# lostinc0de/sparsemat

Measured on AMD Instinct MI355X. Metric: csr_spmv_effective_hbm_GBps, higher is better.
Workload: dtype f32

## Files before the change

include/sparsemat_hip.h:

```cpp
#ifndef SPARSEMAT_HIP_H
#define SPARSEMAT_HIP_H

#include <stddef.h>
#include <stdint.h>

#ifdef __cplusplus
extern "C" {
#endif

#define SMH_ABI_VERSION 3

enum {
    SMH_OK = 0,
    SMH_ERR_DIM_MISMATCH = 1,
    SMH_ERR_NOT_SQUARE = 2,
    SMH_ERR_INDEX_RANGE = 3,
    SMH_ERR_INVALID = 4,
    SMH_ERR_HIP = 5,
    SMH_ERR_OOM = 6,
    SMH_ERR_NO_DEVICE = 7,
    SMH_ERR_CAPACITY = 8,
    SMH_ERR_COMM = 9
};

typedef enum { SMH_F32 = 0, SMH_F64 = 1 } smh_dtype;

typedef enum {
    SMH_SPMV_AUTO = 0,
    SMH_SPMV_VECTOR = 1,
    SMH_SPMV_MERGE = 2,
    SMH_SPMV_SEQ = 3,
    SMH_SPMV_STREAM = 4,
    SMH_SPMV_COLBLOCK = 5,
    SMH_SPMV_COLFUSED = 6,
    SMH_SPMV_COLSPLIT = 7,
    SMH_SPMV_TILED = 8
} smh_spmv_variant;

typedef enum { SMH_TRI_LOWER = 0, SMH_TRI_UPPER = 1 } smh_tri_uplo;
typedef enum { SMH_DIAG_NON_UNIT = 0, SMH_DIAG_UNIT = 1 } smh_tri_diag;

typedef struct smh_crs smh_crs;
typedef struct smh_vec smh_vec;
typedef struct smh_mvec smh_mvec;

int smh_abi_version(void);
const char *smh_last_error(void);
const char *smh_status_string(int status);
int smh_device_count(int *count_out);
int smh_set_device(int device);
int smh_device_synchronize(void);

int smh_crs_create(smh_dtype dtype, size_t n_rows, size_t n_cols, size_t nnz,
                   const uint32_t *offset_rows, const uint32_t *columns, const void *values,
                   int validate, smh_crs **out);
int smh_crs_create_dev(smh_dtype dtype, size_t n_rows, size_t n_cols, size_t nnz,
                       const uint32_t *offset_rows_dev, const uint32_t *columns_dev,
                       const void *values_dev, int validate, smh_crs **out);
int smh_crs_assemble(smh_dtype dtype, size_t n_ops, const uint32_t *rows, const uint32_t *cols,
                     const void *values, const uint8_t *ops, smh_crs **out);
int smh_crs_assemble_dev(smh_dtype dtype, size_t n_ops, const uint32_t *rows_dev,
                         const uint32_t *cols_dev, const void *values_dev, const uint8_t *ops_dev,
                         smh_crs **out);
int smh_crs_replay(smh_dtype dtype, size_t n_ops, const uint32_t *rows, const uint32_t *cols,
                   const void *values, const uint8_t *ops, smh_crs **out);
int smh_crs_replay_dev(smh_dtype dtype, size_t n_ops, const uint32_t *rows_dev,
                       const uint32_t *cols_dev, const void *values_dev, const uint8_t *ops_dev,
                       smh_crs **out);
int smh_crs_transpose(const smh_crs *a, smh_crs **out);
int smh_last_transpose_route(void);
int smh_crs_column_info(const smh_crs *m, uint32_t *rows, uint32_t *col_ptr, uint32_t *entries);
int smh_crs_column_info_dev(const smh_crs *m, uint32_t *rows_dev, uint32_t *col_ptr_dev,
                            uint32_t *entries_dev);
int smh_crs_prod(const smh_crs *a, const smh_crs *b, smh_crs **out);
int smh_crs_permute(const smh_crs *a, const uint32_t *row_perm, size_t n_row_perm, const uint32_t *col_perm, size_t n_col_perm, smh_crs **out);
int smh_crs_permute_dev(const smh_crs *a, const uint32_t *row_perm_dev, size_t n_row_perm, const uint32_t *col_perm_dev, size_t n_col_perm,
                        smh_crs **out);
int smh_crs_permute_symmetric(const smh_crs *a, const uint32_t *perm, size_t n_perm, smh_crs **out);
int smh_crs_permute_symmetric_dev(const smh_crs *a, const uint32_t *perm_dev, size_t n_perm, smh_crs **out);
int smh_crs_bandwidth(const smh_crs *m, uint32_t *lower_out, uint32_t *upper_out);
int smh_crs_span_fraction(smh_crs *m, double *out);
int smh_crs_rcm(const smh_crs *m, uint32_t *perm_out, size_t *n_components_out, size_t *n_levels_out);
int smh_crs_rcm_dev(const smh_crs *m, uint32_t *perm_out_dev, size_t *n_components_out, size_t *n_levels_out);
int smh_crs_color(const smh_crs *m, uint32_t seed, uint32_t *colors_out, uint32_t *perm_out, size_t *n_colors_out, size_t *n_rounds_out);
int smh_crs_color_dev(const smh_crs *m, uint32_t seed, uint32_t *colors_out_dev, uint32_t *perm_out_dev, size_t *n_colors_out, size_t *n_rounds_out);
int smh_crs_clone(const smh_crs *a, smh_crs **out);
int smh_crs_add(const smh_crs *a, const smh_crs *b, smh_crs **out);
int smh_crs_sub(const smh_crs *a, const smh_crs *b, smh_crs **out);
int smh_crs_add_assign(smh_crs *a, const smh_crs *b);
int smh_crs_sub_assign(smh_crs *a, const smh_crs *b);
int smh_last_add_route(void);
int smh_crs_get(const smh_crs *m, size_t i, size_t j, void *value_out);
int smh_crs_get_many(const smh_crs *m, size_t n, const uint32_t *rows, const uint32_t *cols, void *values_out);
int smh_crs_get_many_dev(const smh_crs *m, size_t n, const uint32_t *rows_dev, const uint32_t *cols_dev, void *values_out_dev);
int smh_crs_apply(smh_crs *m, size_t n_ops, const uint32_t *rows, const uint32_t *cols, const void *values, const uint8_t *ops);
int smh_crs_apply_dev(smh_crs *m, size_t n_ops, const uint32_t *rows_dev, const uint32_t *cols_dev, const void *values_dev,
                      const uint8_t *ops_dev);
int smh_last_apply_route(void);
typedef struct smh_update_plan smh_update_plan;
int smh_update_plan_create(const smh_crs *m, size_t n_ops, const uint32_t *rows, const uint32_t *cols, const uint8_t *ops,
                           smh_update_plan **out);
int smh_update_plan_create_dev(const smh_crs *m, size_t n_ops, const uint32_t *rows_dev, const uint32_t *cols_dev,
                               const uint8_t *ops_dev, smh_update_plan **out);
int smh_update_plan_execute(smh_update_plan *p, smh_crs *m, const void *values, int from_zero);
int smh_update_plan_execute_dev(smh_update_plan *p, smh_crs *m, const void *values_dev, int from_zero);
int smh_update_plan_stats(const smh_update_plan *p, size_t *n_ops, size_t *n_targets, size_t *n_live_ops, size_t *longest_run,
                          size_t *long_run_threshold, size_t *device_bytes);
int smh_update_plan_destroy(smh_update_plan *p);
int smh_crs_eye(smh_dtype dtype, size_t dim, smh_crs **out);
int smh_crs_is_symmetric(const smh_crs *m, int *out);
int smh_crs_is_sorted(const smh_crs *m, int *out);
int smh_crs_sort_rows(smh_crs *m);
int smh_crs_destroy(smh_crs *m);
int smh_crs_update_values(smh_crs *m, const void *values_host);
int smh_crs_download(const smh_crs *m, uint32_t *offset_rows, uint32_t *columns, void *values);
size_t smh_crs_n_rows(const smh_crs *m);
size_t smh_crs_n_cols(const smh_crs *m);
size_t smh_crs_nnz(const smh_crs *m);
size_t smh_crs_orphans(const smh_crs *m);
int smh_crs_dtype(const smh_crs *m);
int smh_crs_max_row_len(const smh_crs *m, uint32_t *out);
int smh_crs_col_range(const smh_crs *m, uint32_t *min_out, uint32_t *max_out);
int smh_crs_scale(smh_crs *m, double a);
int smh_crs_resolved_variant(const smh_crs *m, int *variant_out, int *lanes_out);
int smh_crs_set_vector_lanes(smh_crs *m, int lanes);
int smh_crs_set_stream_xs(smh_crs *m, int mode);
int smh_crs_stream_layout(smh_crs *m, int *coded_out, int *byte_lengths_out, int *small_tiles_out, int *xs_chunks_out);
int smh_crs_stream_value_dict(smh_crs *m, int *n_values_out, void *values_out);
int smh_crs_set_stream_value_dict(smh_crs *m, int mode);
int smh_crs_set_stream_direct(smh_crs *m, int mode);
int smh_crs_stream_direct(smh_crs *m, int *direct_out);
int smh_crs_set_vector_chunks(smh_crs *m, int chunks);
int smh_crs_set_ring(smh_crs *m, int mode);
int smh_crs_ring_entries(smh_crs *m, uint32_t *out);
int smh_crs_ring_column_form(smh_crs *m, int *form_out);
int smh_crs_ring_bands(smh_crs *m, uint32_t *bands_out, uint32_t *intervals_out);
int smh_crs_ring_plan(smh_crs *m, uint32_t *n_blocks_out, size_t *n_phases_out,
                      double *ring_fraction_out, int *active_out, uint32_t *phase_ptr_out,
                      uint32_t *phases_out);

int smh_crs_set_colblock_shift(smh_crs *m, uint32_t shift);
int smh_crs_colblock(smh_crs *m, uint32_t *shift_out, size_t *n_blocks_out, int *rows_per_thread_out,
                     double *span_fraction_out, uint32_t *offsets_out, uint32_t *columns_out,
                     void *values_out);

int smh_crs_colfused(smh_crs *m, int *fits_out, uint32_t *shift_out, size_t *n_blocks_out, uint32_t *rows_per_lane_out,
                     size_t *n_tiles_out, uint32_t *tile_rows_out, uint32_t *segments_out, uint8_t *counts_out,
                     uint32_t *columns_out, void *values_out);

int smh_crs_tiled_layout(smh_crs *m, uint32_t *n_slices_out, uint32_t *slice_columns_out, uint32_t *rows_per_block_out,
                         uint32_t *n_row_blocks_out, size_t *copy_entries_out);
int smh_crs_tiled_products(smh_crs *m, size_t *n_products_out);

int smh_crs_tiled_array(smh_crs *m, int which, void *out, size_t capacity_bytes, size_t *bytes_out);

int smh_crs_colsplit(smh_crs *m, int *split_out, uint32_t *min_long_out, size_t *n_long_out, uint32_t *long_rows_out,
                     smh_crs **long_out, smh_crs **short_out);

int smh_crs_spmv(smh_crs *m, const void *x_host, size_t x_len, void *y_host, int variant);
int smh_crs_prepare(smh_crs *m, int variant);
int smh_crs_prepare_stats(smh_crs *m, int variant, double *prepare_ms_out, size_t *derived_bytes_out);
int smh_crs_spmv_dev(smh_crs *m, const void *x_dev, size_t x_len, void *y_dev, int variant,
                     void *stream);
int smh_crs_inner_prod(smh_crs *m, const void *lhs_host, size_t lhs_len, const void *rhs_host,
                       size_t rhs_len, int variant, double *out);
size_t smh_crs_merge_tiles(const smh_crs *m);
size_t smh_crs_merge_tile_items(const smh_crs *m);
int smh_crs_merge_table(smh_crs *m, uint32_t *row_out, uint32_t *nnz_out);

int smh_vec_create(smh_dtype dtype, size_t n, smh_vec **out);
int smh_vec_from_host(smh_dtype dtype, size_t n, const void *host, smh_vec **out);
int smh_vec_wrap_dev(smh_dtype dtype, size_t n, void *dev_ptr, smh_vec **out);
int smh_vec_destroy(smh_vec *v);
int smh_vec_upload(smh_vec *v, const void *host);
int smh_vec_download(const smh_vec *v, void *host);
size_t smh_vec_dim(const smh_vec *v);
int smh_vec_dtype(const smh_vec *v);
void *smh_vec_data(const smh_vec *v);
int smh_vec_copy(smh_vec *dst, const smh_vec *src);
int smh_vec_permute(smh_vec *dst, const smh_vec *src, const uint32_t *perm, size_t n_perm, int inverse);
int smh_vec_permute_dev(smh_vec *dst, const smh_vec *src, const uint32_t *perm_dev, size_t n_perm, int inverse);
int smh_vec_add(smh_vec *x, const smh_vec *y);
int smh_vec_sub(smh_vec *x, const smh_vec *y);
int smh_vec_scale(smh_vec *x, double a);
int smh_vec_axpy(smh_vec *y, double a, const smh_vec *x);
int smh_vec_xpby(smh_vec *p, double b, const smh_vec *r);
int smh_vec_dot(const smh_vec *x, const smh_vec *y, double *out);
int smh_vec_norm_squared(const smh_vec *x, double *out);
int smh_vec_norm(const smh_vec *x, double *out);
int smh_blas_dot_dev(smh_dtype dtype, const void *x_dev, const void *y_dev, size_t n, void *result_dev,
                     void *scratch_dev, void *stream);
size_t smh_blas_dot_scratch_bytes(void);
int smh_blas_axpy_dev(smh_dtype dtype, void *y_dev, const void *a_dev, const void *x_dev, size_t n, void *stream);
int smh_blas_xpby_dev(smh_dtype dtype, void *p_dev, const void *b_dev, const void *r_dev, size_t n, void *stream);
int smh_crs_spmv_vec(smh_crs *m, const smh_vec *x, smh_vec *y, int variant);
int smh_crs_inner_prod_vec(smh_crs *m, const smh_vec *lhs, const smh_vec *rhs, int variant, double *out);

int smh_mvec_create(smh_dtype dtype, size_t n, size_t k, smh_mvec **out);
int smh_mvec_from_host(smh_dtype dtype, size_t n, size_t k, const void *host, smh_mvec **out);
int smh_mvec_upload(smh_mvec *mv, const void *host);
int smh_mvec_download(const smh_mvec *mv, void *host);
int smh_mvec_destroy(smh_mvec *mv);
size_t smh_mvec_dim(const smh_mvec *mv);
size_t smh_mvec_count(const smh_mvec *mv);
size_t smh_mvec_ld(const smh_mvec *mv);
int smh_mvec_dtype(const smh_mvec *mv);
void *smh_mvec_data(const smh_mvec *mv);
int smh_mvec_set_column(smh_mvec *mv, size_t c, const smh_vec *v);
int smh_mvec_get_column(const smh_mvec *mv, size_t c, smh_vec *v);
int smh_mvec_copy(smh_mvec *dst, const smh_mvec *src);
int smh_mvec_add(smh_mvec *x, const smh_mvec *y);
int smh_mvec_sub(smh_mvec *x, const smh_mvec *y);
int smh_mvec_scale(smh_mvec *x, const double *a);
int smh_mvec_dot(const smh_mvec *x, const smh_mvec *y, double *out);
int smh_mvec_norm_squared(const smh_mvec *x, double *out);

int smh_crs_spmv_many(smh_crs *m, const smh_mvec *x, smh_mvec *y);
int smh_crs_spmv_many_dev(smh_crs *m, const void *x_dev, size_t x_len, void *y_dev, size_t k, size_t ld, void *stream);
int smh_crs_spmv_many_host(smh_crs *m, const void *x_host, size_t x_len, size_t k, void *y_host);

int smh_cg_solve(smh_crs *m, const void *b_host, size_t b_len, void *x_host_inout, size_t x_len,
                 double tol, size_t iter_max, int variant, size_t *iters_out, double *rr_out);
int smh_cg_solve_vec(smh_crs *m, const smh_vec *b, smh_vec *x, double tol, size_t iter_max,
                     int variant, size_t check_every, size_t *iters_out, double *rr_out);
int smh_cg_solve_many(smh_crs *m, const smh_mvec *b, smh_mvec *x, double tol, size_t iter_max, size_t check_every,
                      size_t *iters_out, double *rr_out);
int smh_cg_solve_many_host(smh_crs *m, const void *b_host, size_t n, size_t k, void *x_host_inout, double tol,
                           size_t iter_max, size_t *iters_out, double *rr_out);

int smh_pcg_jacobi_solve(smh_crs *m, const void *b_host, size_t b_len, void *x_host_inout,
                         size_t x_len, double tol, size_t iter_max, int variant, size_t *iters_out,
                         double *rr_out);

int smh_crs_trisolve_levels(smh_crs *m, int uplo, size_t *n_levels_out, uint32_t *level_of_row_out, size_t *n_launches_out,
                            size_t *small_level_rows_out);
int smh_crs_trisolve(smh_crs *m, int uplo, int diag, const void *b_host, size_t b_len, void *x_host, size_t x_len);
int smh_crs_trisolve_vec(smh_crs *m, int uplo, int diag, const smh_vec *b, smh_vec *x);
int smh_crs_sgs_apply_vec(smh_crs *m, const smh_vec *r, smh_vec *z);
int smh_pcg_sgs_solve(smh_crs *m, const void *b_host, size_t b_len, void *x_host_inout, size_t x_len,
                      double tol, size_t iter_max, int variant, size_t *iters_out, double *rr_out);
int smh_pcg_sgs_solve_vec(smh_crs *m, const smh_vec *b, smh_vec *x, double tol, size_t iter_max,
                          int variant, size_t check_every, size_t *iters_out, double *rr_out);

int smh_crs_ilu0(const smh_crs *a, smh_crs **f_out, size_t *zero_pivot_out);
int smh_crs_ilu0_refactor(smh_crs *f, const smh_crs *a, size_t *zero_pivot_out);
int smh_crs_ilu_apply_vec(smh_crs *f, const smh_vec *r, smh_vec *z);
int smh_pcg_ilu_solve(smh_crs *a, smh_crs *f, const void *b_host, size_t b_len, void *x_host_inout, size_t x_len,
                      double tol, size_t iter_max, int variant, size_t *iters_out, double *rr_out);
int smh_pcg_ilu_solve_vec(smh_crs *a, smh_crs *f, const smh_vec *b, smh_vec *x, double tol, size_t iter_max,
                          int variant, size_t check_every, size_t *iters_out, double *rr_out);

int smh_bicgstab_solve(smh_crs *m, const void *b_host, size_t b_len, void *x_host_inout, size_t x_len,
                       double tol, size_t iter_max, int variant,
                       size_t *iters_out, double *rr_out, int *breakdown_out);
int smh_bicgstab_solve_vec(smh_crs *m, const smh_vec *b, smh_vec *x, double tol, size_t iter_max,
                           int variant, size_t check_every,
                           size_t *iters_out, double *rr_out, int *breakdown_out);

typedef struct smh_par smh_par;
typedef struct smh_par_vec smh_par_vec;
typedef struct smh_comm smh_comm;

enum { SMH_EXCHANGE_NONE = 0, SMH_EXCHANGE_ALLGATHER = 1, SMH_EXCHANGE_WINDOW = 2, SMH_EXCHANGE_AUTO = 3 };
enum { SMH_PAR_BACKEND_AUTO = 0, SMH_PAR_BACKEND_PEER = 1, SMH_PAR_BACKEND_RCCL = 2 };
#define SMH_COMM_ID_BYTES 128

int smh_comm_unique_id(void *id_out);
int smh_comm_create(const void *id, int n_ranks, int rank, smh_comm **out);
int smh_comm_destroy(smh_comm *c);
int smh_comm_size(const smh_comm *c);
int smh_comm_rank(const smh_comm *c);
int smh_comm_ranks_seen(const smh_comm *c, int *count_out, int *device_out);
int smh_rccl_version(int *version_out);
int smh_comm_barrier(smh_comm *c);
int smh_comm_max_f64(smh_comm *c, double *value_inout);

int smh_par_create(smh_dtype dtype, size_t n_blocks, const int *device_ids, size_t n_rows,
                   size_t n_cols, const uint32_t *offset_rows, const uint32_t *columns,
                   const void *values, int validate, smh_par **out);
enum { SMH_SPLIT_ROWS = 0, SMH_SPLIT_NNZ = 1 };
int smh_par_create_split(smh_dtype dtype, size_t n_blocks, const int *device_ids, size_t n_rows,
                         size_t n_cols, const uint32_t *offset_rows, const uint32_t *columns,
                         const void *values, int validate, int split_mode, smh_par **out);
int smh_par_adopt_split(size_t n_blocks, smh_crs *const *blocks, size_t n_rows, const size_t *split_rows, smh_par **out);
int smh_par_create_rank_split(smh_comm *comm, size_t n_rows, smh_crs *block, size_t row_begin, smh_par **out);
int smh_par_split(const smh_par *p, size_t *rows_out);
int smh_par_adopt(size_t n_blocks, smh_crs *const *blocks, size_t n_rows, smh_par **out);
int smh_par_create_rank(smh_comm *comm, size_t n_rows, smh_crs *block, smh_par **out);
int smh_par_destroy(smh_par *p);
size_t smh_par_n_blocks(const smh_par *p);
size_t smh_par_n_local_blocks(const smh_par *p);
size_t smh_par_n_rows(const smh_par *p);
// ... 72 lines not shown
```

rust/src/ffi.rs:

```rust
#![allow(non_camel_case_types)]
use std::os::raw::{c_char, c_double, c_int, c_void};

#[repr(C)] pub struct smh_crs { _private: [u8; 0] }
#[repr(C)] pub struct smh_vec { _private: [u8; 0] }
#[repr(C)] pub struct smh_update_plan { _private: [u8; 0] }
#[repr(C)] pub struct smh_par { _private: [u8; 0] }
#[repr(C)] pub struct smh_par_vec { _private: [u8; 0] }
#[repr(C)] pub struct smh_comm { _private: [u8; 0] }

pub const SMH_OK: c_int = 0;
pub const SMH_ERR_DIM_MISMATCH: c_int = 1;
pub const SMH_F32: c_int = 0;
pub const SMH_F64: c_int = 1;
pub const SMH_SPMV_AUTO: c_int = 0;
pub const SMH_TRI_LOWER: c_int = 0;
pub const SMH_TRI_UPPER: c_int = 1;
pub const SMH_DIAG_NON_UNIT: c_int = 0;
pub const SMH_DIAG_UNIT: c_int = 1;
pub const SMH_EXCHANGE_NONE: c_int = 0;
pub const SMH_EXCHANGE_ALLGATHER: c_int = 1;
pub const SMH_EXCHANGE_WINDOW: c_int = 2;
pub const SMH_EXCHANGE_AUTO: c_int = 3;
pub const SMH_COMM_ID_BYTES: usize = 128;
pub const SMH_SPLIT_ROWS: c_int = 0;
pub const SMH_SPLIT_NNZ: c_int = 1;

extern "C" {
    pub fn smh_abi_version() -> c_int;
    pub fn smh_last_error() -> *const c_char;
    pub fn smh_device_count(count_out: *mut c_int) -> c_int;
    pub fn smh_pool_trim() -> c_int;
    pub fn smh_pool_stats(kept_bytes_out: *mut usize, live_bytes_out: *mut usize) -> c_int;
    pub fn smh_crs_create(dtype: c_int, n_rows: usize, n_cols: usize, nnz: usize,
                          offset_rows: *const u32, columns: *const u32, values: *const c_void,
                          validate: c_int, out: *mut *mut smh_crs) -> c_int;
    pub fn smh_crs_destroy(m: *mut smh_crs) -> c_int;
    pub fn smh_crs_update_values(m: *mut smh_crs, values_host: *const c_void) -> c_int;
    pub fn smh_crs_spmv(m: *mut smh_crs, x_host: *const c_void, x_len: usize, y_host: *mut c_void,
                        variant: c_int) -> c_int;
    pub fn smh_cg_solve(m: *mut smh_crs, b_host: *const c_void, b_len: usize, x_host_inout: *mut c_void,
                        x_len: usize, tol: c_double, iter_max: usize, variant: c_int,
                        iters_out: *mut usize, rr_out: *mut c_double) -> c_int;
    pub fn smh_pcg_jacobi_solve(m: *mut smh_crs, b_host: *const c_void, b_len: usize, x_host_inout: *mut c_void,
                                x_len: usize, tol: c_double, iter_max: usize, variant: c_int,
                                iters_out: *mut usize, rr_out: *mut c_double) -> c_int;
    pub fn smh_bicgstab_solve(m: *mut smh_crs, b_host: *const c_void, b_len: usize, x_host_inout: *mut c_void,
                              x_len: usize, tol: c_double, iter_max: usize, variant: c_int,
                              iters_out: *mut usize, rr_out: *mut c_double, breakdown_out: *mut c_int) -> c_int;
    pub fn smh_bicgstab_solve_vec(m: *mut smh_crs, b: *const smh_vec, x: *mut smh_vec, tol: c_double, iter_max: usize,
                                  variant: c_int, check_every: usize,
                                  iters_out: *mut usize, rr_out: *mut c_double, breakdown_out: *mut c_int) -> c_int;
    pub fn smh_crs_trisolve_levels(m: *mut smh_crs, uplo: c_int, n_levels_out: *mut usize, level_of_row_out: *mut u32,
                                   n_launches_out: *mut usize, small_level_rows_out: *mut usize) -> c_int;
    pub fn smh_crs_trisolve(m: *mut smh_crs, uplo: c_int, diag: c_int, b_host: *const c_void, b_len: usize, x_host: *mut c_void,
                            x_len: usize) -> c_int;
    pub fn smh_crs_trisolve_vec(m: *mut smh_crs, uplo: c_int, diag: c_int, b: *const smh_vec, x: *mut smh_vec) -> c_int;
    pub fn smh_crs_sgs_apply_vec(m: *mut smh_crs, r: *const smh_vec, z: *mut smh_vec) -> c_int;
    pub fn smh_pcg_sgs_solve(m: *mut smh_crs, b_host: *const c_void, b_len: usize, x_host_inout: *mut c_void,
                             x_len: usize, tol: c_double, iter_max: usize, variant: c_int,
                             iters_out: *mut usize, rr_out: *mut c_double) -> c_int;
    pub fn smh_pcg_sgs_solve_vec(m: *mut smh_crs, b: *const smh_vec, x: *mut smh_vec, tol: c_double, iter_max: usize,
                                 variant: c_int, check_every: usize, iters_out: *mut usize, rr_out: *mut c_double) -> c_int;
    pub fn smh_crs_ilu0(a: *const smh_crs, f_out: *mut *mut smh_crs, zero_pivot_out: *mut usize) -> c_int;
    pub fn smh_crs_ilu0_refactor(f: *mut smh_crs, a: *const smh_crs, zero_pivot_out: *mut usize) -> c_int;
    pub fn smh_crs_ilu_apply_vec(f: *mut smh_crs, r: *const smh_vec, z: *mut smh_vec) -> c_int;
    pub fn smh_pcg_ilu_solve(a: *mut smh_crs, f: *mut smh_crs, b_host: *const c_void, b_len: usize, x_host_inout: *mut c_void,
                             x_len: usize, tol: c_double, iter_max: usize, variant: c_int,
                             iters_out: *mut usize, rr_out: *mut c_double) -> c_int;
    pub fn smh_pcg_ilu_solve_vec(a: *mut smh_crs, f: *mut smh_crs, b: *const smh_vec, x: *mut smh_vec, tol: c_double, iter_max: usize,
                                 variant: c_int, check_every: usize, iters_out: *mut usize, rr_out: *mut c_double) -> c_int;
    pub fn smh_crs_inner_prod(m: *mut smh_crs, lhs_host: *const c_void, lhs_len: usize, rhs_host: *const c_void,
                              rhs_len: usize, variant: c_int, out: *mut c_double) -> c_int;
    pub fn smh_crs_assemble(dtype: c_int, n_ops: usize, rows: *const u32, cols: *const u32, values: *const c_void,
                            ops: *const u8, out: *mut *mut smh_crs) -> c_int;
    pub fn smh_crs_replay(dtype: c_int, n_ops: usize, rows: *const u32, cols: *const u32, values: *const c_void,
                          ops: *const u8, out: *mut *mut smh_crs) -> c_int;
    pub fn smh_crs_transpose(a: *const smh_crs, out: *mut *mut smh_crs) -> c_int;
    pub fn smh_crs_set_stream_xs(m: *mut smh_crs, mode: c_int) -> c_int;
    pub fn smh_crs_set_stream_direct(m: *mut smh_crs, mode: c_int) -> c_int;
    pub fn smh_crs_stream_direct(m: *mut smh_crs, direct_out: *mut c_int) -> c_int;
    pub fn smh_crs_stream_layout(m: *mut smh_crs, coded_out: *mut c_int, byte_lengths_out: *mut c_int, small_tiles_out: *mut c_int, xs_chunks_out: *mut c_int) -> c_int;
    pub fn smh_last_transpose_route() -> c_int;
    pub fn smh_crs_orphans(m: *const smh_crs) -> usize;
    pub fn smh_crs_prod(a: *const smh_crs, b: *const smh_crs, out: *mut *mut smh_crs) -> c_int;
    pub fn smh_crs_clone(a: *const smh_crs, out: *mut *mut smh_crs) -> c_int;
    pub fn smh_crs_permute(a: *const smh_crs, row_perm: *const u32, n_row_perm: usize, col_perm: *const u32, n_col_perm: usize,
                           out: *mut *mut smh_crs) -> c_int;
    pub fn smh_crs_permute_dev(a: *const smh_crs, row_perm_dev: *const u32, n_row_perm: usize, col_perm_dev: *const u32,
                               n_col_perm: usize, out: *mut *mut smh_crs) -> c_int;
    pub fn smh_crs_permute_symmetric(a: *const smh_crs, perm: *const u32, n_perm: usize, out: *mut *mut smh_crs) -> c_int;
    pub fn smh_crs_permute_symmetric_dev(a: *const smh_crs, perm_dev: *const u32, n_perm: usize, out: *mut *mut smh_crs) -> c_int;
    pub fn smh_crs_bandwidth(m: *const smh_crs, lower_out: *mut u32, upper_out: *mut u32) -> c_int;
    pub fn smh_crs_span_fraction(m: *mut smh_crs, out: *mut f64) -> c_int;
    pub fn smh_crs_rcm(m: *const smh_crs, perm_out: *mut u32, n_components_out: *mut usize, n_levels_out: *mut usize) -> c_int;
    pub fn smh_crs_rcm_dev(m: *const smh_crs, perm_out_dev: *mut u32, n_components_out: *mut usize, n_levels_out: *mut usize) -> c_int;
    pub fn smh_crs_color(m: *const smh_crs, seed: u32, colors_out: *mut u32, perm_out: *mut u32, n_colors_out: *mut usize, n_rounds_out: *mut usize) -> c_int;
    pub fn smh_crs_color_dev(m: *const smh_crs, seed: u32, colors_out_dev: *mut u32, perm_out_dev: *mut u32, n_colors_out: *mut usize, n_rounds_out: *mut usize) -> c_int;
    pub fn smh_vec_permute(dst: *mut smh_vec, src: *const smh_vec, perm: *const u32, n_perm: usize, inverse: c_int) -> c_int;
    pub fn smh_vec_permute_dev(dst: *mut smh_vec, src: *const smh_vec, perm_dev: *const u32, n_perm: usize, inverse: c_int) -> c_int;
    pub fn smh_crs_add(a: *const smh_crs, b: *const smh_crs, out: *mut *mut smh_crs) -> c_int;
    pub fn smh_crs_sub(a: *const smh_crs, b: *const smh_crs, out: *mut *mut smh_crs) -> c_int;
    pub fn smh_crs_add_assign(a: *mut smh_crs, b: *const smh_crs) -> c_int;
    pub fn smh_crs_sub_assign(a: *mut smh_crs, b: *const smh_crs) -> c_int;
    pub fn smh_last_add_route() -> c_int;
    pub fn smh_crs_get(m: *const smh_crs, i: usize, j: usize, value_out: *mut c_void) -> c_int;
    pub fn smh_crs_get_many(m: *const smh_crs, n: usize, rows: *const u32, cols: *const u32, values_out: *mut c_void) -> c_int;
    pub fn smh_crs_get_many_dev(m: *const smh_crs, n: usize, rows_dev: *const u32, cols_dev: *const u32,
                                values_out_dev: *mut c_void) -> c_int;
    pub fn smh_crs_apply(m: *mut smh_crs, n_ops: usize, rows: *const u32, cols: *const u32, values: *const c_void,
                         ops: *const u8) -> c_int;
    pub fn smh_crs_apply_dev(m: *mut smh_crs, n_ops: usize, rows_dev: *const u32, cols_dev: *const u32,
                             values_dev: *const c_void, ops_dev: *const u8) -> c_int;
    pub fn smh_last_apply_route() -> c_int;
    pub fn smh_update_plan_create(m: *const smh_crs, n_ops: usize, rows: *const u32, cols: *const u32, ops: *const u8,
                                  out: *mut *mut smh_update_plan) -> c_int;
    pub fn smh_update_plan_create_dev(m: *const smh_crs, n_ops: usize, rows_dev: *const u32, cols_dev: *const u32,
                                      ops_dev: *const u8, out: *mut *mut smh_update_plan) -> c_int;
    pub fn smh_update_plan_execute(p: *mut smh_update_plan, m: *mut smh_crs, values: *const c_void, from_zero: c_int) -> c_int;
    pub fn smh_update_plan_execute_dev(p: *mut smh_update_plan, m: *mut smh_crs, values_dev: *const c_void, from_zero: c_int) -> c_int;
    pub fn smh_update_plan_stats(p: *const smh_update_plan, n_ops: *mut usize, n_targets: *mut usize, n_live_ops: *mut usize,
                                 longest_run: *mut usize, long_run_threshold: *mut usize, device_bytes: *mut usize) -> c_int;
    pub fn smh_update_plan_destroy(p: *mut smh_update_plan) -> c_int;
    pub fn smh_crs_eye(dtype: c_int, dim: usize, out: *mut *mut smh_crs) -> c_int;
    pub fn smh_crs_is_symmetric(m: *const smh_crs, out: *mut c_int) -> c_int;
    pub fn smh_crs_is_sorted(m: *const smh_crs, out: *mut c_int) -> c_int;
    pub fn smh_crs_column_info(m: *const smh_crs, rows: *mut u32, col_ptr: *mut u32, entries: *mut u32) -> c_int;
    pub fn smh_crs_sort_rows(m: *mut smh_crs) -> c_int;
    pub fn smh_par_create(dtype: c_int, n_blocks: usize, device_ids: *const c_int, n_rows: usize, n_cols: usize,
                          offset_rows: *const u32, columns: *const u32, values: *const c_void, validate: c_int,
                          out: *mut *mut smh_par) -> c_int;
    pub fn smh_par_create_split(dtype: c_int, n_blocks: usize, device_ids: *const c_int, n_rows: usize, n_cols: usize,
                                offset_rows: *const u32, columns: *const u32, values: *const c_void, validate: c_int,
                                split_mode: c_int, out: *mut *mut smh_par) -> c_int;
    pub fn smh_par_split(p: *const smh_par, rows_out: *mut usize) -> c_int;
    pub fn smh_par_set_overlap(p: *mut smh_par, on: c_int) -> c_int;
    pub fn smh_par_interior(p: *const smh_par, local_block: usize, variant: c_int, row_begin: *mut usize, row_end: *mut usize) -> c_int;
    pub fn smh_par_destroy(p: *mut smh_par) -> c_int;
    pub fn smh_par_spmv(p: *mut smh_par, x_host: *const c_void, x_len: usize, y_host: *mut c_void, variant: c_int) -> c_int;
    pub fn smh_par_cg_solve(p: *mut smh_par, b_host: *const c_void, b_len: usize, x_host_inout: *mut c_void, x_len: usize,
                            tol: c_double, iter_max: usize, variant: c_int, iters_out: *mut usize,
                            rr_out: *mut c_double) -> c_int;
    pub fn smh_par_vec_create(p: *mut smh_par, n: usize, out: *mut *mut smh_par_vec) -> c_int;
    pub fn smh_par_vec_destroy(v: *mut smh_par_vec) -> c_int;
    pub fn smh_par_vec_upload(v: *mut smh_par_vec, host: *const c_void) -> c_int;
    pub fn smh_par_vec_download(v: *const smh_par_vec, host: *mut c_void) -> c_int;
    pub fn smh_par_spmv_dev(p: *mut smh_par, x: *const smh_par_vec, y: *mut smh_par_vec, variant: c_int, exchange: c_int) -> c_int;
    pub fn smh_par_exchange(p: *mut smh_par, v: *mut smh_par_vec, mode: c_int) -> c_int;
    pub fn smh_par_synchronize(p: *mut smh_par) -> c_int;
    pub fn smh_par_cg_solve_vec(p: *mut smh_par, b: *const smh_par_vec, x: *mut smh_par_vec, tol: c_double, iter_max: usize,
                                variant: c_int, check_every: usize, iters_out: *mut usize, rr_out: *mut c_double) -> c_int;
    pub fn smh_comm_unique_id(id_out: *mut c_void) -> c_int;
    pub fn smh_comm_create(id: *const c_void, n_ranks: c_int, rank: c_int, out: *mut *mut smh_comm) -> c_int;
    pub fn smh_comm_destroy(c: *mut smh_comm) -> c_int;
    pub fn smh_par_create_rank(comm: *mut smh_comm, n_rows: usize, block: *mut smh_crs, out: *mut *mut smh_par) -> c_int;
    pub fn smh_par_create_rank_split(comm: *mut smh_comm, n_rows: usize, block: *mut smh_crs, row_begin: usize, out: *mut *mut smh_par) -> c_int;
    pub fn smh_crs_n_rows(m: *const smh_crs) -> usize;
    pub fn smh_crs_n_cols(m: *const smh_crs) -> usize;
    pub fn smh_crs_dtype(m: *const smh_crs) -> c_int;
    pub fn smh_crs_nnz(m: *const smh_crs) -> usize;
    pub fn smh_crs_download(m: *const smh_crs, offset_rows: *mut u32, columns: *mut u32, values: *mut c_void) -> c_int;
}
```

sparsemat_amd/_lib.py:

```python
import ctypes as C
import os

_HERE = os.path.dirname(os.path.abspath(__file__))
LIB_PATH = os.environ.get("SPARSEMAT_HIP_LIB") or os.path.join(_HERE, "libsparsemat_hip.so")

SMH_OK = 0
SMH_ERR_DIM_MISMATCH, SMH_ERR_NOT_SQUARE, SMH_ERR_INDEX_RANGE, SMH_ERR_INVALID = 1, 2, 3, 4
SMH_ERR_HIP, SMH_ERR_OOM, SMH_ERR_NO_DEVICE, SMH_ERR_CAPACITY, SMH_ERR_COMM = 5, 6, 7, 8, 9
SMH_F32, SMH_F64 = 0, 1
SMH_TRI_LOWER, SMH_TRI_UPPER = 0, 1
SMH_DIAG_NON_UNIT, SMH_DIAG_UNIT = 0, 1
UPLO = {"lower": SMH_TRI_LOWER, "upper": SMH_TRI_UPPER}
EXCHANGE_NONE, EXCHANGE_ALLGATHER, EXCHANGE_WINDOW, EXCHANGE_AUTO = 0, 1, 2, 3
EXCHANGES = {"none": EXCHANGE_NONE, "allgather": EXCHANGE_ALLGATHER, "window": EXCHANGE_WINDOW, "halo": EXCHANGE_WINDOW, "auto": EXCHANGE_AUTO}
EXCHANGE_NAMES = {EXCHANGE_NONE: "none", EXCHANGE_ALLGATHER: "allgather", EXCHANGE_WINDOW: "window", EXCHANGE_AUTO: "auto"}
PAR_BACKEND_AUTO, PAR_BACKEND_PEER, PAR_BACKEND_RCCL = 0, 1, 2
PAR_BACKENDS = {"auto": PAR_BACKEND_AUTO, "peer": PAR_BACKEND_PEER, "rccl": PAR_BACKEND_RCCL}
COMM_ID_BYTES = 128
SPMV_AUTO, SPMV_VECTOR, SPMV_MERGE, SPMV_SEQ, SPMV_STREAM, SPMV_COLBLOCK, SPMV_COLFUSED, SPMV_COLSPLIT, SPMV_TILED = 0, 1, 2, 3, 4, 5, 6, 7, 8
VARIANTS = {"auto": SPMV_AUTO, "vector": SPMV_VECTOR, "merge": SPMV_MERGE, "seq": SPMV_SEQ, "stream": SPMV_STREAM,
            "colblock": SPMV_COLBLOCK, "colfused": SPMV_COLFUSED, "colsplit": SPMV_COLSPLIT, "tiled": SPMV_TILED}

_sz = C.c_size_t
_vp = C.c_void_p
_u32p = C.POINTER(C.c_uint32)
_int = C.c_int

SIGNATURES = {
    "smh_abi_version": (_int, []),
    "smh_last_error": (C.c_char_p, []),
    "smh_status_string": (C.c_char_p, [_int]),
    "smh_device_count": (_int, [C.POINTER(_int)]),
    "smh_set_device": (_int, [_int]),
    "smh_device_synchronize": (_int, []),
    "smh_crs_create": (_int, [_int, _sz, _sz, _sz, _vp, _vp, _vp, _int, C.POINTER(_vp)]),
    "smh_crs_create_dev": (_int, [_int, _sz, _sz, _sz, _vp, _vp, _vp, _int, C.POINTER(_vp)]),
    "smh_crs_assemble": (_int, [_int, _sz, _vp, _vp, _vp, _vp, C.POINTER(_vp)]),
    "smh_crs_assemble_dev": (_int, [_int, _sz, _vp, _vp, _vp, _vp, C.POINTER(_vp)]),
    "smh_crs_replay": (_int, [_int, _sz, _vp, _vp, _vp, _vp, C.POINTER(_vp)]),
    "smh_crs_replay_dev": (_int, [_int, _sz, _vp, _vp, _vp, _vp, C.POINTER(_vp)]),
    "smh_crs_transpose": (_int, [_vp, C.POINTER(_vp)]),
    "smh_crs_column_info": (_int, [_vp, _vp, _vp, _vp]),
    "smh_crs_column_info_dev": (_int, [_vp, _vp, _vp, _vp]),
    "smh_crs_prod": (_int, [_vp, _vp, C.POINTER(_vp)]),
    "smh_crs_permute": (_int, [_vp, _vp, _sz, _vp, _sz, C.POINTER(_vp)]),
    "smh_crs_permute_dev": (_int, [_vp, _vp, _sz, _vp, _sz, C.POINTER(_vp)]),
    "smh_crs_permute_symmetric": (_int, [_vp, _vp, _sz, C.POINTER(_vp)]),
    "smh_crs_permute_symmetric_dev": (_int, [_vp, _vp, _sz, C.POINTER(_vp)]),
    "smh_crs_bandwidth": (_int, [_vp, _u32p, _u32p]),
    "smh_crs_span_fraction": (_int, [_vp, C.POINTER(C.c_double)]),
    "smh_crs_rcm": (_int, [_vp, _vp, C.POINTER(_sz), C.POINTER(_sz)]),
    "smh_crs_rcm_dev": (_int, [_vp, _vp, C.POINTER(_sz), C.POINTER(_sz)]),
    "smh_crs_color": (_int, [_vp, C.c_uint32, _vp, _vp, C.POINTER(_sz), C.POINTER(_sz)]),
    "smh_crs_color_dev": (_int, [_vp, C.c_uint32, _vp, _vp, C.POINTER(_sz), C.POINTER(_sz)]),
    "smh_vec_permute": (_int, [_vp, _vp, _vp, _sz, _int]),
    "smh_vec_permute_dev": (_int, [_vp, _vp, _vp, _sz, _int]),
    "smh_crs_clone": (_int, [_vp, C.POINTER(_vp)]),
    "smh_crs_add": (_int, [_vp, _vp, C.POINTER(_vp)]),
    "smh_crs_sub": (_int, [_vp, _vp, C.POINTER(_vp)]),
    "smh_crs_add_assign": (_int, [_vp, _vp]),
    "smh_crs_sub_assign": (_int, [_vp, _vp]),
    "smh_last_add_route": (_int, []),
    "smh_crs_get": (_int, [_vp, _sz, _sz, _vp]),
    "smh_crs_get_many": (_int, [_vp, _sz, _vp, _vp, _vp]),
    "smh_crs_get_many_dev": (_int, [_vp, _sz, _vp, _vp, _vp]),
    "smh_crs_apply": (_int, [_vp, _sz, _vp, _vp, _vp, _vp]),
    "smh_crs_apply_dev": (_int, [_vp, _sz, _vp, _vp, _vp, _vp]),
    "smh_last_apply_route": (_int, []),
    "smh_update_plan_create": (_int, [_vp, _sz, _vp, _vp, _vp, _vp]),
    "smh_update_plan_create_dev": (_int, [_vp, _sz, _vp, _vp, _vp, _vp]),
    "smh_update_plan_execute": (_int, [_vp, _vp, _vp, _int]),
    "smh_update_plan_execute_dev": (_int, [_vp, _vp, _vp, _int]),
    "smh_update_plan_stats": (_int, [_vp, _vp, _vp, _vp, _vp, _vp, _vp]),
    "smh_update_plan_destroy": (_int, [_vp]),
    "smh_crs_eye": (_int, [_int, _sz, C.POINTER(_vp)]),
    "smh_crs_is_symmetric": (_int, [_vp, C.POINTER(_int)]),
    "smh_crs_is_sorted": (_int, [_vp, C.POINTER(_int)]),
    "smh_crs_sort_rows": (_int, [_vp]),
    "smh_crs_destroy": (_int, [_vp]),
    "smh_crs_update_values": (_int, [_vp, _vp]),
    "smh_crs_download": (_int, [_vp, _vp, _vp, _vp]),
    "smh_crs_n_rows": (_sz, [_vp]),
    "smh_crs_n_cols": (_sz, [_vp]),
    "smh_crs_nnz": (_sz, [_vp]),
    "smh_crs_orphans": (_sz, [_vp]),
    "smh_crs_dtype": (_int, [_vp]),
    "smh_crs_max_row_len": (_int, [_vp, _u32p]),
    "smh_crs_col_range": (_int, [_vp, _u32p, _u32p]),
    "smh_crs_scale": (_int, [_vp, C.c_double]),
    "smh_crs_resolved_variant": (_int, [_vp, C.POINTER(_int), C.POINTER(_int)]),
    "smh_crs_set_vector_lanes": (_int, [_vp, _int]),
    "smh_crs_set_vector_chunks": (_int, [_vp, _int]),
    "smh_crs_set_ring": (_int, [_vp, _int]),
    "smh_crs_ring_entries": (_int, [_vp, _u32p]),
    "smh_crs_ring_column_form": (_int, [_vp, C.POINTER(_int)]),
    "smh_crs_ring_bands": (_int, [_vp, _u32p, _vp]),
    "smh_crs_ring_plan": (_int, [_vp, _u32p, C.POINTER(_sz), C.POINTER(C.c_double), C.POINTER(_int), _vp, _vp]),
    "smh_crs_set_colblock_shift": (_int, [_vp, C.c_uint32]),
    "smh_crs_tiled_layout": (_int, [_vp, _u32p, _u32p, _u32p, _u32p, C.POINTER(_sz)]),
    "smh_crs_tiled_products": (_int, [_vp, C.POINTER(_sz)]),
    "smh_crs_prepare_stats": (_int, [_vp, _int, C.POINTER(C.c_double), C.POINTER(_sz)]),
    "smh_crs_tiled_array": (_int, [_vp, _int, _vp, _sz, C.POINTER(_sz)]),
    "smh_crs_colblock": (_int, [_vp, _u32p, C.POINTER(_sz), C.POINTER(_int), C.POINTER(C.c_double), _vp, _vp, _vp]),
    "smh_crs_colfused": (_int, [_vp, C.POINTER(_int), _u32p, C.POINTER(_sz), _u32p, C.POINTER(_sz), _vp, _vp, _vp, _vp, _vp]),
    "smh_crs_colsplit": (_int, [_vp, C.POINTER(_int), _u32p, C.POINTER(_sz), _vp, C.POINTER(_vp), C.POINTER(_vp)]),
    "smh_crs_spmv": (_int, [_vp, _vp, _sz, _vp, _int]),
    "smh_crs_spmv_dev": (_int, [_vp, _vp, _sz, _vp, _int, _vp]),
    "smh_crs_prepare": (_int, [_vp, _int]),
    "smh_crs_merge_tiles": (_sz, [_vp]),
    "smh_crs_merge_tile_items": (_sz, [_vp]),
    "smh_crs_merge_table": (_int, [_vp, _vp, _vp]),
    "smh_vec_create": (_int, [_int, _sz, C.POINTER(_vp)]),
    "smh_vec_from_host": (_int, [_int, _sz, _vp, C.POINTER(_vp)]),
    "smh_vec_wrap_dev": (_int, [_int, _sz, _vp, C.POINTER(_vp)]),
    "smh_vec_destroy": (_int, [_vp]),
    "smh_vec_upload": (_int, [_vp, _vp]),
    "smh_vec_download": (_int, [_vp, _vp]),
    "smh_vec_dim": (_sz, [_vp]),
    "smh_vec_dtype": (_int, [_vp]),
    "smh_vec_data": (_vp, [_vp]),
    "smh_vec_copy": (_int, [_vp, _vp]),
    "smh_vec_add": (_int, [_vp, _vp]),
    "smh_vec_sub": (_int, [_vp, _vp]),
    "smh_vec_scale": (_int, [_vp, C.c_double]),
    "smh_vec_axpy": (_int, [_vp, C.c_double, _vp]),
    "smh_vec_xpby": (_int, [_vp, C.c_double, _vp]),
    "smh_vec_dot": (_int, [_vp, _vp, C.POINTER(C.c_double)]),
    "smh_vec_norm_squared": (_int, [_vp, C.POINTER(C.c_double)]),
    "smh_vec_norm": (_int, [_vp, C.POINTER(C.c_double)]),
    "smh_blas_dot_dev": (_int, [_int, _vp, _vp, _sz, _vp, _vp, _vp]),
    "smh_blas_dot_scratch_bytes": (_sz, []),
    "smh_blas_axpy_dev": (_int, [_int, _vp, _vp, _vp, _sz, _vp]),
    "smh_blas_xpby_dev": (_int, [_int, _vp, _vp, _vp, _sz, _vp]),
    "smh_crs_spmv_vec": (_int, [_vp, _vp, _vp, _int]),
    "smh_crs_inner_prod": (_int, [_vp, _vp, _sz, _vp, _sz, _int, C.POINTER(C.c_double)]),
    "smh_crs_inner_prod_vec": (_int, [_vp, _vp, _vp, _int, C.POINTER(C.c_double)]),
    "smh_mvec_create": (_int, [_int, _sz, _sz, C.POINTER(_vp)]),
    "smh_mvec_from_host": (_int, [_int, _sz, _sz, _vp, C.POINTER(_vp)]),
    "smh_mvec_upload": (_int, [_vp, _vp]),
    "smh_mvec_download": (_int, [_vp, _vp]),
    "smh_mvec_destroy": (_int, [_vp]),
    "smh_mvec_dim": (_sz, [_vp]),
    "smh_mvec_count": (_sz, [_vp]),
    "smh_mvec_ld": (_sz, [_vp]),
    "smh_mvec_dtype": (_int, [_vp]),
    "smh_mvec_data": (_vp, [_vp]),
    "smh_mvec_set_column": (_int, [_vp, _sz, _vp]),
    "smh_mvec_get_column": (_int, [_vp, _sz, _vp]),
    "smh_mvec_copy": (_int, [_vp, _vp]),
    "smh_mvec_add": (_int, [_vp, _vp]),
    "smh_mvec_sub": (_int, [_vp, _vp]),
    "smh_mvec_scale": (_int, [_vp, C.POINTER(C.c_double)]),
    "smh_mvec_dot": (_int, [_vp, _vp, C.POINTER(C.c_double)]),
    "smh_mvec_norm_squared": (_int, [_vp, C.POINTER(C.c_double)]),
    "smh_crs_spmv_many": (_int, [_vp, _vp, _vp]),
    "smh_crs_spmv_many_dev": (_int, [_vp, _vp, _sz, _vp, _sz, _sz, _vp]),
    "smh_crs_spmv_many_host": (_int, [_vp, _vp, _sz, _sz, _vp]),
    "smh_cg_solve": (_int, [_vp, _vp, _sz, _vp, _sz, C.c_double, _sz, _int, C.POINTER(_sz),
                            C.POINTER(C.c_double)]),
    "smh_cg_solve_vec": (_int, [_vp, _vp, _vp, C.c_double, _sz, _int, _sz, C.POINTER(_sz),
                                C.POINTER(C.c_double)]),
    "smh_cg_solve_many": (_int, [_vp, _vp, _vp, C.c_double, _sz, _sz, C.POINTER(_sz), C.POINTER(C.c_double)]),
    "smh_cg_solve_many_host": (_int, [_vp, _vp, _sz, _sz, _vp, C.c_double, _sz, C.POINTER(_sz), C.POINTER(C.c_double)]),
    "smh_pcg_jacobi_solve": (_int, [_vp, _vp, _sz, _vp, _sz, C.c_double, _sz, _int, C.POINTER(_sz),
                                    C.POINTER(C.c_double)]),
    "smh_crs_trisolve_levels": (_int, [_vp, _int, C.POINTER(_sz), _vp, C.POINTER(_sz), C.POINTER(_sz)]),
    "smh_crs_trisolve": (_int, [_vp, _int, _int, _vp, _sz, _vp, _sz]),
    "smh_crs_trisolve_vec": (_int, [_vp, _int, _int, _vp, _vp]),
    "smh_crs_sgs_apply_vec": (_int, [_vp, _vp, _vp]),
    "smh_pcg_sgs_solve": (_int, [_vp, _vp, _sz, _vp, _sz, C.c_double, _sz, _int, C.POINTER(_sz),
                                 C.POINTER(C.c_double)]),
    "smh_pcg_sgs_solve_vec": (_int, [_vp, _vp, _vp, C.c_double, _sz, _int, _sz, C.POINTER(_sz),
                                     C.POINTER(C.c_double)]),
    "smh_crs_ilu0": (_int, [_vp, C.POINTER(_vp), C.POINTER(_sz)]),
    "smh_crs_ilu0_refactor": (_int, [_vp, _vp, C.POINTER(_sz)]),
    "smh_crs_ilu_apply_vec": (_int, [_vp, _vp, _vp]),
    "smh_pcg_ilu_solve": (_int, [_vp, _vp, _vp, _sz, _vp, _sz, C.c_double, _sz, _int, C.POINTER(_sz),
                                 C.POINTER(C.c_double)]),
    "smh_pcg_ilu_solve_vec": (_int, [_vp, _vp, _vp, _vp, C.c_double, _sz, _int, _sz, C.POINTER(_sz),
                                     C.POINTER(C.c_double)]),
    "smh_bicgstab_solve": (_int, [_vp, _vp, _sz, _vp, _sz, C.c_double, _sz, _int, C.POINTER(_sz),
                                  C.POINTER(C.c_double), C.POINTER(_int)]),
    "smh_bicgstab_solve_vec": (_int, [_vp, _vp, _vp, C.c_double, _sz, _int, _sz, C.POINTER(_sz),
                                      C.POINTER(C.c_double), C.POINTER(_int)]),
    "smh_comm_unique_id": (_int, [_vp]),
    "smh_comm_create": (_int, [_vp, _int, _int, C.POINTER(_vp)]),
    "smh_comm_destroy": (_int, [_vp]),
    "smh_comm_size": (_int, [_vp]),
    "smh_comm_rank": (_int, [_vp]),
    "smh_comm_ranks_seen": (_int, [_vp, C.POINTER(C.c_int), C.POINTER(C.c_int)]),
    "smh_rccl_version": (_int, [C.POINTER(C.c_int)]),
    "smh_comm_barrier": (_int, [_vp]),
    "smh_comm_max_f64": (_int, [_vp, C.POINTER(C.c_double)]),
    "smh_par_create": (_int, [_int, _sz, _vp, _sz, _sz, _vp, _vp, _vp, _int, C.POINTER(_vp)]),
    "smh_par_create_split": (_int, [_int, _sz, _vp, _sz, _sz, _vp, _vp, _vp, _int, _int, C.POINTER(_vp)]),
    "smh_par_adopt_split": (_int, [_sz, C.POINTER(_vp), _sz, _vp, C.POINTER(_vp)]),
    "smh_par_create_rank_split": (_int, [_vp, _sz, _vp, _sz, C.POINTER(_vp)]),
    "smh_par_split": (_int, [_vp, _vp]),
    "smh_par_plan_split": (_int, [_sz, _sz, _vp, _vp, _vp, _vp, _sz, _vp, _vp, _vp, _vp, C.POINTER(_int), C.POINTER(_sz)]),
    "smh_par_adopt": (_int, [_sz, C.POINTER(_vp), _sz, C.POINTER(_vp)]),
    "smh_par_create_rank": (_int, [_vp, _sz, _vp, C.POINTER(_vp)]),
    "smh_par_n_local_blocks": (_sz, [_vp]),
    "smh_par_set_backend": (_int, [_vp, _int]),
    "smh_par_backend": (_int, [_vp]),
    "smh_par_set_overlap": (_int, [_vp, _int]),
    "smh_par_set_threads": (_int, [_vp, _int]),
    "smh_par_interior": (_int, [_vp, _sz, _int, C.POINTER(_sz), C.POINTER(_sz)]),
    "smh_par_exchange_mode": (_int, [_vp, _int, C.POINTER(_int), C.POINTER(_sz)]),
    "smh_par_plan": (_int, [_sz, _sz, _vp, _vp, _vp, _sz, _vp, _vp, _vp, _vp, C.POINTER(_int), C.POINTER(_sz)]),
    "smh_par_vec_create": (_int, [_vp, _sz, C.POINTER(_vp)]),
    "smh_par_vec_destroy": (_int, [_vp]),
    "smh_par_vec_dim": (_sz, [_vp]),
    "smh_par_vec_upload": (_int, [_vp, _vp]),
    "smh_par_vec_download": (_int, [_vp, _vp]),
    "smh_par_vec_download_block": (_int, [_vp, _sz, _vp]),
    "smh_par_vec_ptr": (_int, [_vp, _sz, C.POINTER(_vp)]),
    "smh_par_spmv_dev": (_int, [_vp, _vp, _vp, _int, _int]),
    "smh_par_exchange": (_int, [_vp, _vp, _int]),
    "smh_par_synchronize": (_int, [_vp]),
    "smh_par_cg_solve_vec": (_int, [_vp, _vp, _vp, C.c_double, _sz, _int, _sz, C.POINTER(_sz), C.POINTER(C.c_double)]),
    "smh_par_destroy": (_int, [_vp]),
    "smh_par_n_blocks": (_sz, [_vp]),
    "smh_par_n_rows": (_sz, [_vp]),
    "smh_par_n_cols": (_sz, [_vp]),
    "smh_par_nnz": (_sz, [_vp]),
    "smh_par_rows_per_block": (_sz, [_vp]),
    "smh_par_block": (_int, [_vp, _sz, C.POINTER(_vp), C.POINTER(_sz), C.POINTER(_sz), C.POINTER(_int)]),
    "smh_par_block_stream": (_int, [_vp, _sz, C.POINTER(_vp)]),
    "smh_par_get_block_and_row_id": (_int, [_vp, _sz, C.POINTER(_sz), C.POINTER(_sz)]),
    "smh_par_scale": (_int, [_vp, C.c_double]),
    "smh_par_spmv": (_int, [_vp, _vp, _sz, _vp, _int]),
    "smh_par_cg_solve": (_int, [_vp, _vp, _sz, _vp, _sz, C.c_double, _sz, _int, C.POINTER(_sz),
                                C.POINTER(C.c_double)]),
    "smh_synth_x": (_int, [_int, C.c_uint64, _sz, _sz, _vp, _vp]),
    "smh_synth_fixed": (_int, [_int, C.c_uint64, _int, _sz, C.c_uint32, _sz, _sz, _vp, _vp, _vp, _vp]),
    "smh_synth_powerlaw_cdf": (_int, [C.c_uint32, C.c_double, _vp]),
    "smh_synth_powerlaw_lengths": (_int, [C.c_uint64, _sz, _sz, C.c_uint32, _vp, _vp]),
    "smh_synth_fill": (_int, [_int, C.c_uint64, _sz, _sz, _sz, _vp, _vp, _vp, _vp]),
    "smh_synth_laplace3d": (_int, [_int, _sz, _sz, _sz, _sz, _sz, _vp, _vp, _vp, C.POINTER(_sz), _vp]),
    "smh_crs_set_stream_xs": (_int, [_vp, _int]),
    "smh_crs_set_stream_direct": (_int, [_vp, _int]),
    "smh_crs_stream_direct": (_int, [_vp, C.POINTER(_int)]),
    "smh_crs_stream_layout": (_int, [_vp, C.POINTER(_int), C.POINTER(_int), C.POINTER(_int), C.POINTER(_int)]),
    "smh_crs_stream_value_dict": (_int, [_vp, C.POINTER(C.c_int), _vp]),
    "smh_crs_set_stream_value_dict": (_int, [_vp, _int]),
    "smh_last_transpose_route": (_int, []),
    "smh_pool_trim": (_int, []),
    "smh_pool_stats": (_int, [C.POINTER(_sz), C.POINTER(_sz)]),
    "smh_dev_alloc": (_int, [_sz, C.POINTER(_vp)]),
# ... 68 lines not shown
```

sparsemat_amd/csrc/capi.hip:

```cpp
#include <atomic>
#include <chrono>
#include <cmath>
#include <cstdarg>
#include <cstdlib>
#include <cstring>
#include <new>
#include <vector>

#include "crs_forms.hpp"

namespace smh {

static thread_local char g_err[512] = "";

void set_error(const char *fmt, ...) {
    va_list ap;
    va_start(ap, fmt);
    vsnprintf(g_err, sizeof g_err, fmt, ap);
    va_end(ap);
}

void clear_error() { g_err[0] = 0; }

int fail(int status, const char *fmt, ...) {
// ... 1049 lines not shown
    return tiled_array(m, which, out, capacity_bytes, bytes_out);
}

int smh_crs_set_colblock_shift(smh_crs *m, uint32_t shift) {
    if (!m) return fail(SMH_ERR_INVALID, "NULL handle");
    if (shift > 31) return fail(SMH_ERR_INVALID, "column block shift must be 0 (automatic) or 1..31");
    if (shift != m->knobs.cb_forced_shift) invalidate(m, Changed::BlockWidth);
    m->knobs.cb_forced_shift = shift;
    return SMH_OK;
}

int smh_crs_colblock(smh_crs *m, uint32_t *shift_out, size_t *n_blocks_out, int *rows_per_thread_out,
                     double *span_fraction_out, uint32_t *offsets_out, uint32_t *columns_out, void *values_out) {
    if (!m) return fail(SMH_ERR_INVALID, "NULL handle");
    SMH_TRY(ensure_ring_plan(m, false));
    SMH_TRY(ensure_colblock(m));
    if (shift_out) *shift_out = m->cb.shift;
    if (n_blocks_out) *n_blocks_out = m->cb.blocks;
    if (rows_per_thread_out) *rows_per_thread_out = m->cb.rpt;
    if (span_fraction_out) *span_fraction_out = m->span_fraction;
    if (offsets_out)
        SMH_HIP(hipMemcpy(offsets_out, m->cb.off.get(), m->cb.blocks * (m->n_rows + 1) * sizeof(uint32_t), hipMemcpyDeviceToHost));
    if (columns_out && m->nnz) SMH_HIP(hipMemcpy(columns_out, m->cb.col.get(), m->nnz * sizeof(uint32_t), hipMemcpyDeviceToHost));
    if (values_out && m->nnz) SMH_HIP(hipMemcpy(values_out, m->cb.val.get(), m->nnz * dtype_size(m->dtype), hipMemcpyDeviceToHost));
    return SMH_OK;
}

int smh_crs_colfused(smh_crs *m, int *fits_out, uint32_t *shift_out, size_t *n_blocks_out, uint32_t *rows_per_lane_out,
                     size_t *n_tiles_out, uint32_t *tile_rows_out, uint32_t *segments_out, uint8_t *counts_out, uint32_t *columns_out,
                     void *values_out) {
    if (!m) return fail(SMH_ERR_INVALID, "NULL handle");
    SMH_TRY(ensure_colfused(m));
    const size_t tile_rows = (size_t)64 * m->cf.rt, n_tiles = (m->cf.state == Form::Ready) ? m->cf.tiles : 0;
    if (fits_out) *fits_out = (m->cf.state == Form::Ready) ? 1 : 0;
    if (shift_out) *shift_out = m->cf.shift;
    if (n_blocks_out) *n_blocks_out = m->cf.blocks;
    if (rows_per_lane_out) *rows_per_lane_out = m->cf.rt;
    if (n_tiles_out) *n_tiles_out = n_tiles;
    if (m->cf.state != Form::Ready) return SMH_OK;
    SMH_HIP(hipStreamSynchronize(m->stream));
    if (tile_rows_out) SMH_HIP(hipMemcpy(tile_rows_out, m->cf.tile_row.get(), (n_tiles + 1) * sizeof(uint32_t), hipMemcpyDeviceToHost));
    if (segments_out) SMH_HIP(hipMemcpy(segments_out, m->cf.seg.get(), (n_tiles * m->cf.blocks + 1) * sizeof(uint32_t), hipMemcpyDeviceToHost));
    if (counts_out && n_tiles) SMH_HIP(hipMemcpy(counts_out, m->cf.cnt.get(), n_tiles * m->cf.blocks * tile_rows, hipMemcpyDeviceToHost));
    if (columns_out && m->nnz) SMH_HIP(hipMemcpy(columns_out, m->cf.col.get(), m->nnz * sizeof(uint32_t), hipMemcpyDeviceToHost));
    if (values_out && m->nnz) SMH_HIP(hipMemcpy(values_out, m->cf.val.get(), m->nnz * dtype_size(m->dtype), hipMemcpyDeviceToHost));
    return SMH_OK;
}

int smh_crs_colsplit(smh_crs *m, int *split_out, uint32_t *min_long_out, size_t *n_long_out, uint32_t *long_rows_out, smh_crs **long_out,
                     smh_crs **short_out) {
    if (!m) return fail(SMH_ERR_INVALID, "NULL handle");
    SMH_TRY(ensure_split(m));
    const bool split = m->split.state == Form::Ready;
    if (split_out) *split_out = split ? 1 : 0;
    if (min_long_out) *min_long_out = kSplitMinLong;
    if (n_long_out) *n_long_out = split ? m->split.n_long : 0;
    if (long_out) *long_out = split ? m->split.long_part : nullptr;
    if (short_out) *short_out = split ? m->split.short_part : nullptr;
    if (long_rows_out && split && m->split.n_long)
        SMH_HIP(hipMemcpy(long_rows_out, m->split.rows.get(), m->split.n_long * sizeof(uint32_t), hipMemcpyDeviceToHost));
    return SMH_OK;
}

int smh_crs_resolved_variant(const smh_crs *m, int *variant_out, int *lanes_out) {
    if (!m) return fail(SMH_ERR_INVALID, "NULL handle");
    if (variant_out) *variant_out = resolve_variant(m, SMH_SPMV_AUTO);
    if (lanes_out) *lanes_out = auto_lanes(m);
    return SMH_OK;
}

int smh_crs_set_stream_xs(smh_crs *m, int mode) {
    if (!m) return fail(SMH_ERR_INVALID, "NULL handle");
    if (mode < -1 || mode > 1) return fail(SMH_ERR_INVALID, "mode must be -1 (automatic), 0 (never) or 1 (whenever the tiles allow)");
    m->knobs.use_stream_xs = mode;
    return recode_stream(m);
}

int smh_crs_set_stream_direct(smh_crs *m, int mode) {
    if (!m) return fail(SMH_ERR_INVALID, "NULL handle");
    if (mode < -1 || mode > 1) return fail(SMH_ERR_INVALID, "mode must be -1 (automatic), 0 (never) or 1 (whenever x is staged)");
    m->knobs.use_stream_direct = mode;
    return recode_stream(m);
}

int smh_crs_stream_direct(smh_crs *m, int *direct_out) {
    if (!m || !direct_out) return fail(SMH_ERR_INVALID, "NULL argument");
    StreamCfg c;
    SMH_TRY(stream_cfg(m, &c));
    *direct_out = c.direct && c.xs != 0;
    return SMH_OK;
}

int smh_crs_stream_value_dict(smh_crs *m, int *n_values_out, void *values_out) {
    if (!m || !n_values_out) return fail(SMH_ERR_INVALID, "NULL argument");
    StreamCfg c;
    SMH_TRY(stream_cfg(m, &c));
    *n_values_out = c.dict ? (int)m->dict.n : 0;
    if (c.dict && values_out) {
        SMH_HIP(hipMemcpyAsync(values_out, m->dict.values.get(), (size_t)m->dict.n * dtype_size(m->dtype), hipMemcpyDeviceToHost, m->stream));
        SMH_HIP(hipStreamSynchronize(m->stream));
    }
    return SMH_OK;
}

int smh_crs_set_stream_value_dict(smh_crs *m, int mode) {
    if (!m) return fail(SMH_ERR_INVALID, "NULL handle");
    if (mode < -1 || mode > 0) return fail(SMH_ERR_INVALID, "mode must be -1 (automatic: whenever the values allow) or 0 (never)");
    m->knobs.use_stream_vdict = mode;
    return recode_stream(m);
}

int smh_crs_stream_layout(smh_crs *m, int *coded_out, int *byte_lengths_out, int *small_tiles_out, int *xs_chunks_out) {
    if (!m) return fail(SMH_ERR_INVALID, "NULL handle");
    StreamCfg c;
    SMH_TRY(stream_cfg(m, &c));
    if (coded_out) *coded_out = c.code && c.cwin;
    if (byte_lengths_out) *byte_lengths_out = c.len8 && c.tbase;
    if (small_tiles_out) *small_tiles_out = c.small;
    if (xs_chunks_out) *xs_chunks_out = c.xs;
    return SMH_OK;
}

int smh_crs_set_vector_chunks(smh_crs *m, int chunks) {
    if (!m) return fail(SMH_ERR_INVALID, "NULL handle");
    if (chunks < 0 || chunks > 3) return fail(SMH_ERR_INVALID, "chunks per lane must be 0 (automatic), 1, 2 or 3");
    m->knobs.forced_chunks = chunks;
    return SMH_OK;
}

int smh_crs_set_ring(smh_crs *m, int mode) {
    if (!m) return fail(SMH_ERR_INVALID, "NULL handle");
    if (mode < -1 || mode > 1) return fail(SMH_ERR_INVALID, "ring mode must be -1 (auto), 0 (plain K1) or 1 (K1r)");
    m->knobs.use_ring = mode;
    return SMH_OK;
}

int smh_crs_ring_plan(smh_crs *m, uint32_t *n_blocks_out, size_t *n_phases_out, double *ring_fraction_out,
                      int *active_out, uint32_t *phase_ptr_out, uint32_t *phases_out) {
    if (!m) return fail(SMH_ERR_INVALID, "NULL handle");
    SMH_TRY(ensure_ring_plan(m));
    bool ring = false;
    SMH_TRY(vector_uses_ring(m, &ring));
    if (n_blocks_out) *n_blocks_out = m->ring.blocks;
    if (n_phases_out) *n_phases_out = m->ring.n_phases;
    if (ring_fraction_out) *ring_fraction_out = m->ring.fraction;
    if (active_out) *active_out = ring ? 1 : 0;
    if (phase_ptr_out)
        SMH_HIP(hipMemcpy(phase_ptr_out, m->ring.phase_ptr.get(), (m->ring.blocks + 1) * sizeof(uint32_t), hipMemcpyDeviceToHost));
    if (phases_out && m->ring.n_phases)
        SMH_HIP(hipMemcpy(phases_out, m->ring.phases.get(), m->ring.n_phases * sizeof(RingPhase), hipMemcpyDeviceToHost));
    return SMH_OK;
}

int smh_crs_ring_column_form(smh_crs *m, int *form_out) {
    if (!m || !form_out) return fail(SMH_ERR_INVALID, "NULL argument");
    bool ring = false;
    SMH_TRY(vector_uses_ring(m, &ring));
    *form_out = !ring ? 0 : m->ring.lo8.get() ? 2 : m->ring.col16.get() ? 1 : 0;
    return SMH_OK;
}

int smh_crs_ring_entries(smh_crs *m, uint32_t *out) {
    if (!m || !out) return fail(SMH_ERR_INVALID, "NULL argument");
    SMH_TRY(ensure_ring_plan(m));
    *out = m->ring.entries;
    return SMH_OK;
}

int smh_crs_ring_bands(smh_crs *m, uint32_t *bands_out, uint32_t *intervals_out) {
    if (!m || !bands_out) return fail(SMH_ERR_INVALID, "NULL argument");
    SMH_TRY(ensure_ring_plan(m));
    *bands_out = m->ring.bands;
    if (intervals_out && m->ring.bands == 4 && m->ring.win.get())
        SMH_HIP(hipMemcpy(intervals_out, m->ring.win.get(), ((m->n_rows + 63) / 64) * 8 * sizeof(uint32_t), hipMemcpyDeviceToHost));
    return SMH_OK;
}

int smh_crs_set_vector_lanes(smh_crs *m, int lanes) {
    if (!m) return fail(SMH_ERR_INVALID, "NULL handle");
    if (lanes != 0 && (lanes < 1 || lanes > 64 || (lanes & (lanes - 1))))
        return fail(SMH_ERR_INVALID, "lanes per row must be 0 or a power of two in 1..64");
    m->knobs.forced_lanes = lanes;
    return SMH_OK;
}

int smh_crs_prepare(smh_crs *m, int variant) {
    if (!m) return fail(SMH_ERR_INVALID, "NULL handle");
    const auto t0 = std::chrono::steady_clock::now();
    const long long b0 = pool_thread_net_bytes();
    int rc = prepare_forms(m, variant);
    if (rc == SMH_OK && m->stream) {
        const hipError_t e = hipStreamSynchronize(m->stream);
        if (e != hipSuccess) rc = hip_fail(e, "hipStreamSynchronize", __FILE__, __LINE__);
    }
    m->prepare_ms += std::chrono::duration<double, std::milli>(std::chrono::steady_clock::now() - t0).count();
    m->prepare_bytes += pool_thread_net_bytes() - b0;
    return rc;
}

int smh_crs_prepare_stats(smh_crs *m, int variant, double *prepare_ms_out, size_t *derived_bytes_out) {
    if (!m) return fail(SMH_ERR_INVALID, "NULL handle");
    SMH_TRY(smh_crs_prepare(m, variant));
    if (prepare_ms_out) *prepare_ms_out = m->create_ms + m->prepare_ms;
    if (derived_bytes_out) *derived_bytes_out = (size_t)(m->prepare_bytes + m->create_bytes > 0 ? m->prepare_bytes + m->create_bytes : 0);
    return SMH_OK;
}

int smh_crs_spmv_dev(smh_crs *m, const void *x_dev, size_t x_len, void *y_dev, int variant, void *stream) {
    if (!m) return fail(SMH_ERR_INVALID, "NULL handle");
    if (m->n_rows && (!y_dev || (m->nnz && !x_dev))) return fail(SMH_ERR_INVALID, "NULL device vector");
    return spmv_enqueue(m, x_dev, x_len, y_dev, variant, (hipStream_t)stream);
}

int smh_crs_spmv(smh_crs *m, const void *x_host, size_t x_len, void *y_host, int variant) {
    if (!m) return fail(SMH_ERR_INVALID, "NULL handle");
    if (m->n_rows == 0) return SMH_OK;
    if (!y_host || (x_len && !x_host)) return fail(SMH_ERR_INVALID, "NULL host vector");
    const size_t vs = dtype_size(m->dtype);
    SMH_TRY(m->stage_x.ensure_cap(x_len * vs));
    SMH_TRY(m->stage_y.ensure_cap(m->n_rows * vs));
    if (x_len) SMH_HIP(hipMemcpyAsync(m->stage_x.d.get(), x_host, x_len * vs, hipMemcpyHostToDevice, m->stream));
    SMH_TRY(spmv_enqueue(m, m->stage_x.d.get(), x_len, m->stage_y.d.get(), variant, m->stream));
    SMH_HIP(hipMemcpyAsync(y_host, m->stage_y.d.get(), m->n_rows * vs, hipMemcpyDeviceToHost, m->stream));
    SMH_HIP(hipStreamSynchronize(m->stream));
    return SMH_OK;
}

size_t smh_crs_merge_tiles(const smh_crs *m) {
    if (!m) return 0;
    return (size_t)(((uint64_t)m->n_rows + m->nnz + kMergeTile - 1) / kMergeTile);
}

size_t smh_crs_merge_tile_items(const smh_crs *) { return kMergeTile; }

int smh_crs_merge_table(smh_crs *m, uint32_t *row_out, uint32_t *nnz_out) {
    if (!m || !row_out || !nnz_out) return fail(SMH_ERR_INVALID, "NULL argument");
    SMH_TRY(ensure_merge_ws(m));
    if (m->merge.n_tiles == 0) { row_out[0] = 0; nnz_out[0] = 0; return SMH_OK; }
    SMH_HIP(hipMemcpy(row_out, m->merge.tile_row.get(), (m->merge.n_tiles + 1) * sizeof(uint32_t), hipMemcpyDeviceToHost));
    SMH_HIP(hipMemcpy(nnz_out, m->merge.tile_nz.get(), (m->merge.n_tiles + 1) * sizeof(uint32_t), hipMemcpyDeviceToHost));
    return SMH_OK;
}

int smh_vec_create(smh_dtype dtype, size_t n, smh_vec **out) {
    if (!out) return fail(SMH_ERR_INVALID, "out is NULL");
    *out = nullptr;
    if (!valid_dtype(dtype)) return fail(SMH_ERR_INVALID, "dtype must be SMH_F32 or SMH_F64");
    SMH_TRY(require_device());
    smh_vec *v = new (std::nothrow) smh_vec();
    if (!v) return fail(SMH_ERR_OOM, "host allocation failed");
    v->dtype = dtype; v->n = n; v->owns = true; v->device = current_device();
    const size_t bytes = (n ? n : 1) * dtype_size(dtype);
    hipError_t e = hipMalloc(&v->d, bytes);
    if (e == hipSuccess) e = hipMemset(v->d, 0, bytes);
    if (e != hipSuccess) { delete v; return hip_fail(e, "smh_vec_create", __FILE__, __LINE__); }
    *out = v;
    return SMH_OK;
}

int smh_vec_from_host(smh_dtype dtype, size_t n, const void *host, smh_vec **out) {
    SMH_TRY(smh_vec_create(dtype, n, out));
    if (n) {
        int rc = smh_vec_upload(*out, host);
        if (rc != SMH_OK) { smh_vec_destroy(*out); *out = nullptr; return rc; }
    }
    return SMH_OK;
}

int smh_vec_wrap_dev(smh_dtype dtype, size_t n, void *dev_ptr, smh_vec **out) {
    if (!out) return fail(SMH_ERR_INVALID, "out is NULL");
    *out = nullptr;
    if (!valid_dtype(dtype)) return fail(SMH_ERR_INVALID, "dtype must be SMH_F32 or SMH_F64");
    if (n && !dev_ptr) return fail(SMH_ERR_INVALID, "dev_ptr is NULL");
    SMH_TRY(require_device());
    smh_vec *v = new (std::nothrow) smh_vec();
    if (!v) return fail(SMH_ERR_OOM, "host allocation failed");
    v->dtype = dtype; v->n = n; v->d = dev_ptr; v->owns = false; v->device = current_device();
    *out = v;
    return SMH_OK;
}

int smh_vec_destroy(smh_vec *v) {
    if (!v) return SMH_OK;
    if (v->owns) { (void)hipFree(v->d); (void)hipGetLastError(); }
    delete v;
    return SMH_OK;
}

int smh_vec_upload(smh_vec *v, const void *host) {
    if (!v || (v->n && !host)) return fail(SMH_ERR_INVALID, "NULL argument");
    if (v->n) SMH_HIP(hipMemcpy(v->d, host, v->n * dtype_size(v->dtype), hipMemcpyHostToDevice));
    return SMH_OK;
}

int smh_vec_download(const smh_vec *v, void *host) {
    if (!v || (v->n && !host)) return fail(SMH_ERR_INVALID, "NULL argument");
    if (v->n) SMH_HIP(hipMemcpy(host, v->d, v->n * dtype_size(v->dtype), hipMemcpyDeviceToHost));
    return SMH_OK;
}

size_t smh_vec_dim(const smh_vec *v) { return v ? v->n : 0; }
int smh_vec_dtype(const smh_vec *v) { return v ? v->dtype : -1; }
void *smh_vec_data(const smh_vec *v) { return v ? v->d : nullptr; }

int smh_vec_copy(smh_vec *dst, const smh_vec *src) {
    SMH_TRY(vec_check_pair(dst, src));
// ... 310 lines not shown
```

sparsemat_amd/csrc/crs_forms.hip:

```cpp
#include <cstdlib>
#include <cstring>
#include <vector>

#include "crs_forms.hpp"

namespace smh {

void build_ring_plan(size_t n_rows, size_t ring_entries, const uint32_t *cmin, const uint32_t *cmax, size_t n_blocks,
                     uint32_t noring_mode, std::vector<uint32_t> &phase_ptr, std::vector<RingPhase> &phases,
                     double *ring_row_fraction);
void build_ring_plan_banded(size_t n_rows, size_t ring_entries, const uint32_t *win, size_t n_blocks, uint32_t noring_mode,
                            std::vector<uint32_t> &phase_ptr, std::vector<RingPhase> &phases, double *ring_row_fraction);

int ensure_merge_ws(smh_crs *m) {
    if (m->merge.state == Form::Ready) return SMH_OK;
    MergeTable t;
    const uint64_t items = (uint64_t)m->n_rows + (uint64_t)m->nnz;
    t.n_tiles = (size_t)((items + kMergeTile - 1) / kMergeTile);
    if (t.n_tiles) {
        SMH_TRY(t.tile_row.alloc(t.n_tiles + 1));
        SMH_TRY(t.tile_nz.alloc(t.n_tiles + 1));
        SMH_TRY(t.carry_row.alloc(t.n_tiles));
        SMH_TRY(t.carry_val.alloc(t.n_tiles * dtype_size(m->dtype)));
        SMH_TRY(launch_merge_table(m->d_off, m->n_rows, m->nnz, t.n_tiles, t.tile_row.get(), t.tile_nz.get(), m->stream));
        SMH_HIP(hipStreamSynchronize(m->stream));
    }
    t.state = Form::Ready;
    m->merge = std::move(t);
    return SMH_OK;
}

int ensure_ring_plan(smh_crs *m, bool with_bands) {
    if (m->ring.state == Form::Ready && (!with_bands || m->ring.bands_tried)) return SMH_OK;
    m->ring = RingPlan();
    RingPlan p;
    p.bands_tried = with_bands;
    const size_t n_tiles = (m->n_rows + 63) / 64;
    int cus = 256;
    hipDeviceProp_t prop;
    if (hipGetDeviceProperties(&prop, m->device) == hipSuccess && prop.multiProcessorCount > 0) cus = prop.multiProcessorCount;
    unsigned per_cu = 6;
    if (const char *e = getenv("SMH_RING_BLOCKS_PER_CU")) {
        const int v = atoi(e);
        if (v >= 1 && v <= 64) per_cu = (unsigned)v;
    }
    unsigned blocks = per_cu * (unsigned)cus;
    blocks = (blocks + 7u) & ~7u;
    std::vector<uint32_t> cmin(n_tiles), cmax(n_tiles);
    if (n_tiles) {
        Scratch scr;
        uint32_t *d_min = nullptr, *d_max = nullptr;
        SMH_TRY(scr.alloc(&d_min, n_tiles));
        SMH_TRY(scr.alloc(&d_max, n_tiles));
        SMH_TRY(read_back(d_min, cmin.data(), n_tiles, m->stream, [&](uint32_t *) -> int {
            SMH_TRY(launch_tile_span(m->d_off, m->d_col, m->n_rows, n_tiles, d_min, d_max, m->stream));
            SMH_HIP(hipMemcpyAsync(cmax.data(), d_max, n_tiles * sizeof(uint32_t), hipMemcpyDeviceToHost, m->stream));
            return SMH_OK;
        }));
    }
    double span_fraction = 0.0;
    {
        double acc = 0.0;
        size_t used = 0;
        for (size_t t = 0; t < n_tiles; ++t)
            if (cmin[t] <= cmax[t]) { acc += (double)(cmax[t] - cmin[t]) + 1.0; ++used; }
        span_fraction = used && m->n_cols ? acc / (double)used / (double)m->n_cols : 0.0;
    }
    std::vector<uint32_t> phase_ptr;
    std::vector<RingPhase> phases;
    uint32_t noring_mode = 0;
    if (const char *e = getenv("SMH_GATHER_NT")) noring_mode = atoi(e) ? 2u : 0u;
    build_ring_plan(m->n_rows, kRingEntries, cmin.data(), cmax.data(), blocks, noring_mode, phase_ptr, phases,
                    &p.fraction);
    p.entries = kRingEntries;
    const char *wide_env = getenv("SMH_RING_WIDE");
    if (m->dtype == SMH_F32 && p.fraction < 0.5 && !(wide_env && atoi(wide_env) == 0)) {
        std::vector<uint32_t> phase_ptr_w;
        std::vector<RingPhase> phases_w;
        double frac_w = 0.0;
        const unsigned blocks_w = ((blocks / 2) + 7u) & ~7u;
        build_ring_plan(m->n_rows, kRingEntriesWide, cmin.data(), cmax.data(), blocks_w, noring_mode, phase_ptr_w, phases_w, &frac_w);
        if (frac_w >= 0.5) {
            phase_ptr.swap(phase_ptr_w);
            phases.swap(phases_w);
            p.fraction = frac_w;
            p.entries = kRingEntriesWide;
            blocks = blocks_w;
        }
    }
    const char *band_env = getenv("SMH_RING_BANDS");
    if (with_bands && p.fraction < 0.5 && n_tiles && m->nnz && !(band_env && atoi(band_env) == 0)) {
        const unsigned sizes[2] = {(unsigned)kRingEntries, (unsigned)kRingEntriesWide};
        const int n_sizes = m->dtype == SMH_F32 && !(wide_env && atoi(wide_env) == 0) ? 2 : 1;
        std::vector<uint32_t> h_win(n_tiles * 8);
        Scratch scr;
        uint32_t *d_count = nullptr;
        SMH_TRY(p.win.alloc(n_tiles * 8));
        SMH_TRY(scr.alloc(&d_count, 1));
        for (int si = 0; si < n_sizes && p.bands == 1; ++si) {
            const unsigned ring = sizes[si];
            SMH_TRY(read_back(p.win.get(), h_win.data(), n_tiles * 8, m->stream, [&](uint32_t *d_win) {
                return launch_tile_intervals(m->d_off, m->d_col, m->n_rows, 64, ring / 4, d_win, d_count, m->stream);
            }));
            std::vector<uint32_t> phase_ptr_b;
            std::vector<RingPhase> phases_b;
            double frac_b = 0.0;
            const unsigned blocks_b = ring == (unsigned)kRingEntries || m->dtype == SMH_F64 ? blocks : ((blocks / 2) + 7u) & ~7u;
            build_ring_plan_banded(m->n_rows, ring, h_win.data(), blocks_b, noring_mode, phase_ptr_b, phases_b, &frac_b);
            if (frac_b >= 0.5 && frac_b > p.fraction) {
                phase_ptr.swap(phase_ptr_b);
                phases.swap(phases_b);
                p.fraction = frac_b;
                p.entries = ring;
                p.bands = 4;
                blocks = blocks_b;
            }
        }
        if (p.bands != 4) p.win.reset();
    }
    SMH_TRY(p.phase_ptr.alloc(phase_ptr.size()));
    SMH_TRY(p.phases.alloc(phases.size() + 1));
    SMH_HIP(hipMemcpy(p.phase_ptr.get(), phase_ptr.data(), phase_ptr.size() * sizeof(uint32_t), hipMemcpyHostToDevice));
    if (!phases.empty())
        SMH_HIP(hipMemcpy(p.phases.get(), phases.data(), phases.size() * sizeof(RingPhase), hipMemcpyHostToDevice));
    p.blocks = blocks;
    p.n_phases = phases.size();
    p.state = Form::Ready;
    m->ring = std::move(p);
    m->span_fraction = span_fraction;
    return SMH_OK;
}

int columns_within_n_cols(const smh_crs *m, const char *what) {
    if (m->nnz && (size_t)m->max_col >= m->n_cols)
        return fail(SMH_ERR_INDEX_RANGE, "%s: column index %u >= n_cols %zu", what, m->max_col, m->n_cols);
    return SMH_OK;
}

int ensure_colblock(smh_crs *m) {
    if (m->cb.state == Form::Ready) return SMH_OK;
    SMH_TRY(columns_within_n_cols(m, "column-blocked variant"));
    const size_t blocks = blocks_for(m->n_cols, cb_shift_for(m));
    if (blocks == 0 || blocks > 128)
        return fail(SMH_ERR_INVALID, "column-blocked variant: %zu column blocks (supported: 1..128)", blocks);
    if ((uint64_t)blocks * (m->n_rows + 1) >= (1ull << 34)) return fail(SMH_ERR_OOM, "column-blocked offsets too large");
    ColBlock c;
    c.shift = cb_shift_for(m);
    uint32_t *off2 = nullptr, *col2 = nullptr;
    void *val2 = nullptr;
    SMH_TRY(build_colblock(m->dtype, m->d_off, m->d_col, m->d_val, m->n_rows, m->nnz, c.shift, blocks, &off2, &col2, &val2, m->stream));
    c.off.reset(off2);
    c.col.reset(col2);
    c.val.reset((char *)val2);
    c.blocks = blocks;
    Scratch scr;
    uint32_t *d_max = nullptr;
    SMH_TRY(scr.alloc(&d_max, 1));
    int rpt = 8;
    uint32_t worst = 0;
    for (; rpt >= 1; rpt >>= 1) {
        worst = 0;
        for (size_t b = 0; b < blocks; ++b) {
            uint32_t h = 0;
            SMH_TRY(read_back(d_max, &h, 1, m->stream, [&](uint32_t *d) {
                return launch_stream_max_tile(c.off.get() + b * (m->n_rows + 1), m->n_rows, (size_t)kStreamRows * rpt, d, m->stream);
            }));
            worst = h > worst ? h : worst;
        }
        if (worst <= (uint32_t)kStreamCap || rpt == 1) break;
    }
    c.rpt = rpt < 1 ? 1 : rpt;
    c.single_pass = worst <= (uint32_t)kStreamCap;
    c.state = Form::Ready;
    m->cb = std::move(c);
    return SMH_OK;
}

int ensure_colfused(smh_crs *m) {
    if (m->cf.state != Form::NotTried) return SMH_OK;
    SMH_TRY(columns_within_n_cols(m, "fused column-blocked variant"));
    const size_t blocks = blocks_for(m->n_cols, cf_shift_for(m));
    if (blocks > 255) return fail(SMH_ERR_INVALID, "fused column-blocked variant: %zu column blocks (supported: 1..255)", blocks);
    uint32_t rt = 16;
    if (const char *e = getenv("SMH_COLFUSED_RT")) {
        if (atoi(e) == 8) rt = 8;
    }
    ColFused c;
    bool fits = false;
    uint32_t *tile_row = nullptr, *seg = nullptr, *col2 = nullptr;
    uint8_t *cnt = nullptr;
    void *val2 = nullptr;
    SMH_TRY(build_colfused(m->dtype, m->d_off, m->d_col, m->d_val, m->n_rows, m->nnz, cf_shift_for(m), blocks, rt, &c.tiles,
                           &tile_row, &seg, &cnt, &col2, &val2, &fits, m->stream));
    c.tile_row.reset(tile_row);
    c.seg.reset(seg);
    c.cnt.reset(cnt);
    c.col.reset(col2);
    c.val.reset((char *)val2);
    c.shift = cf_shift_for(m);
    c.blocks = blocks;
    c.rt = rt;
    c.state = fits ? Form::Ready : Form::Refused;
    m->cf = std::move(c);
    return SMH_OK;
}

const uint32_t kSplitMinLong = 64;
int ensure_split(smh_crs *m) {
    if (m->split.state != Form::NotTried) return SMH_OK;
    SMH_TRY(columns_within_n_cols(m, "row-length split"));
    m->split.state = Form::Refused;
    if (m->no_split || m->n_rows == 0 || m->nnz == 0) return SMH_OK;
    RowSplit sp;
    size_t nnz_long = 0;
    uint32_t *rows = nullptr;
    CrsArrays long_part, short_part;
    SMH_TRY(build_colsplit(m->dtype, m->d_off, m->d_col, m->d_val, m->n_rows, m->nnz, kSplitMinLong, &sp.n_long, &nnz_long, &rows, &long_part.off,
                           &long_part.col, &long_part.val, &short_part.off, &short_part.col, &short_part.val, m->stream));
    sp.rows.reset(rows);
    const bool worth = sp.n_long > 0 && sp.n_long * 4 <= m->n_rows && nnz_long * 4 >= m->nnz;
    if (!worth) return SMH_OK;
    auto part = [&](size_t n_rows, size_t nnz, CrsArrays &arrays, uint32_t shift, smh_crs **out) -> int {
        SMH_TRY(wrap_arrays(m->dtype, nullptr, n_rows, m->n_cols, nnz, arrays, 0, out));
        (*out)->no_split = true;
        (*out)->knobs.cb_forced_shift = shift;
        return SMH_OK;
    };
    SMH_TRY(part(sp.n_long, nnz_long, long_part, 18u, &sp.long_part));
    SMH_TRY(part(m->n_rows, m->nnz - nnz_long, short_part, 19u, &sp.short_part));
    SMH_TRY(sp.y.alloc(sp.n_long * dtype_size(m->dtype)));
    SMH_HIP(hipStreamCreateWithFlags(&sp.side, hipStreamNonBlocking));
    SMH_HIP(hipEventCreateWithFlags(&sp.fork, hipEventDisableTiming));
    SMH_HIP(hipEventCreateWithFlags(&sp.join, hipEventDisableTiming));
    sp.state = Form::Ready;
    m->split = std::move(sp);
    return SMH_OK;
}
RowSplit::~RowSplit() {
    (void)smh_crs_destroy(long_part);
    (void)smh_crs_destroy(short_part);
    rows.reset();
    y.reset();
    if (side) { (void)hipStreamSynchronize(side); (void)hipStreamDestroy(side); }
    if (fork) (void)hipEventDestroy(fork);
    if (join) (void)hipEventDestroy(join);
}

static int ensure_stream_codes(smh_crs *m) {
    if (m->codes.state != Form::NotTried) return SMH_OK;
    StreamCodes c;
    c.state = Form::Refused;
    const size_t n_tiles = (m->n_rows + kStreamRows - 1) / kStreamRows;
    if (n_tiles && m->nnz) {
        uint32_t h_count = 0;
        SMH_TRY(c.cwin.alloc(n_tiles * 8));
        SMH_TRY(read_back(&h_count, 1, m->stream, [&](uint32_t *d_count) {
            return launch_stream_windows(m->d_off, m->d_col, m->n_rows, c.cwin.get(), d_count, m->stream);
        }));
        if ((size_t)h_count == n_tiles) c.state = Form::Ready;
        else c.cwin.reset();
    }
    if (c.state == Form::Ready) {
        const size_t n_out = ((m->nnz + 3) & ~size_t(3)) + 4;
        SMH_TRY(c.code.alloc(n_out));
        SMH_HIP(hipMemsetAsync(c.code.get(), 0, n_out * sizeof(uint16_t), m->stream));
        SMH_TRY(launch_stream_codes(m->d_off, m->d_col, c.cwin.get(), m->n_rows, c.code.get(), m->stream));
        if (m->max_row_len <= 255u) {
            SMH_TRY(c.len8.alloc(n_tiles * kStreamRows));
            SMH_TRY(c.tbase.alloc(n_tiles + 1));
            SMH_TRY(launch_stream_len8(m->d_off, m->n_rows, c.len8.get(), c.tbase.get(), m->stream));
            uint32_t h_xs[2] = {0xFFFFFFFFu, 0};
            SMH_TRY(read_back(h_xs, 2, m->stream, [&](uint32_t *d_xs) { return launch_stream_xs_stats(c.cwin.get(), n_tiles, d_xs, m->stream); }));
            c.xs_chunks = h_xs[0];
            c.xs_end = h_xs[1];
            unsigned long long h_odd = 0;
            SMH_TRY(read_back(&h_odd, 1, m->stream, [&](unsigned long long *d_odd) {
                return launch_stream_odd_rows(c.len8.get(), n_tiles * kStreamRows, d_odd, m->stream);
// ... 168 lines not shown
```

sparsemat_amd/csrc/internal.hpp:

```cpp
#pragma once
#include <hip/hip_runtime.h>

#include <cstddef>
#include <cstdint>
#include <cstdio>
#include <cstring>
#include <string>
#include <utility>
#include <vector>

#include "../../include/sparsemat_hip.h"

namespace smh {

void set_error(const char *fmt, ...);
int fail(int status, const char *fmt, ...);
int hip_fail(hipError_t e, const char *what, const char *file, int line);

#define SMH_HIP(call)                                                     \
    do {                                                                  \
        hipError_t e__ = (call);                                          \
        if (e__ != hipSuccess) return ::smh::hip_fail(e__, #call, __FILE__, __LINE__); \
    } while (0)

// ... 269 lines not shown
constexpr int kRingEntriesWide = 32768;
constexpr int kStreamRows = kBlock;
constexpr int kStreamCap = 4096;
constexpr int kStreamCapSmall = 2045;
constexpr int kStreamCodeWidth = 16384;
constexpr int kManyCap = 2048;

int device_exclusive_scan_u32(uint32_t *data, uint64_t n, hipStream_t s, uint64_t *total_out);
int launch_spmv_vector(int dtype, int lanes, const uint32_t *off, const uint32_t *col, const void *val,
                       const void *x, void *y, size_t n_rows, size_t nnz, hipStream_t s);
int launch_spmv_seq(int dtype, const uint32_t *off, const uint32_t *col, const void *val, const void *x,
                    void *y, size_t n_rows, hipStream_t s);
int launch_merge_table(const uint32_t *off, size_t n_rows, size_t nnz, size_t n_tiles, uint32_t *tile_row,
                       uint32_t *tile_nz, hipStream_t s);
int launch_spmv_merge(int dtype, const uint32_t *off, const uint32_t *col, const void *val, const void *x,
                      void *y, size_t n_rows, size_t nnz, size_t n_tiles, const uint32_t *tile_row,
                      const uint32_t *tile_nz, uint32_t *carry_row, void *carry_val, hipStream_t s);
int launch_spmv_stream(int dtype, const uint32_t *off, const uint32_t *col, const void *val, const void *x, void *y,
                       size_t n_rows, size_t nnz, bool padded, int rows_per_thread,
                       bool single_pass ,
                       void *dot_partials ,
                       const uint16_t *code, const uint32_t *cwin ,
                       const uint8_t *len8, const uint32_t *tbase ,
                       const void *dot_lhs ,
                       hipStream_t s, bool small_tiles = false ,
                       int xs = 0 ,
                       uint64_t tile_begin = 0, uint64_t tile_end = ~uint64_t(0) );
int launch_stream_xs_stats(const uint32_t *win, size_t n_tiles, uint32_t *d_out2, hipStream_t s);
int launch_stream_len8(const uint32_t *off, size_t n_rows, uint8_t *len8, uint32_t *tbase, hipStream_t s);
size_t stream_tiles(size_t n_rows, int rows_per_thread);
int launch_stream_windows(const uint32_t *off, const uint32_t *col, size_t n_rows, uint32_t *win,
                          uint32_t *d_count, hipStream_t s);
int launch_stream_codes(const uint32_t *off, const uint32_t *col, const uint32_t *win, size_t n_rows, uint16_t *code,
                        hipStream_t s);
int launch_spmv_many(int dtype, const uint32_t *off, const uint32_t *col, const void *val, const void *x, void *y, size_t n_rows, size_t nnz,
                     bool padded, size_t k, size_t ld, hipStream_t s);
int launch_spmv_stream_xd(int dtype, const void *val, const void *x, void *y, size_t n_rows, void *dot_partials, const uint16_t *scode,
                          const uint32_t *cwin, const uint8_t *len8, const uint32_t *tbase, const void *dot_lhs, hipStream_t s, int xs,
                          uint64_t tile_begin = 0, uint64_t tile_end = ~uint64_t(0), const void *dict = nullptr ,
                          bool dict_high = false );
bool stream_value_dict_high(int dtype, uint32_t n, int xs);
int stream_value_dict(int dtype, const void *val, size_t nnz, void *dict_out, uint32_t *count_out, hipStream_t s);
int launch_stream_value_codes(int dtype, const void *val, size_t nnz, const void *dict, uint32_t n, int xs, uint16_t *code, hipStream_t s);
uint32_t stream_value_dict_capacity(int xs);
int launch_stream_stage_codes(const uint32_t *off, const uint32_t *col, const uint32_t *win, size_t n_rows, uint32_t elem_bytes,
                              uint16_t *code, hipStream_t s);
int launch_stream_odd_rows(const uint8_t *len8, size_t n_padded, unsigned long long *d_out, hipStream_t s);
int launch_stream_max_tile(const uint32_t *off, size_t n_rows, size_t tile_rows, uint32_t *d_out, hipStream_t s);
int launch_spmv_stream_block(int dtype, const uint32_t *off, const uint32_t *col, const void *val, const void *x, void *y,
                             size_t n_rows, size_t nnz_total, int rows_per_thread, bool single_pass, bool accumulate,
                             hipStream_t s);
int build_colblock(int dtype, const uint32_t *off, const uint32_t *col, const void *val, size_t n_rows, size_t nnz,
                   uint32_t shift, size_t n_blocks, uint32_t **off2_out, uint32_t **col2_out, void **val2_out,
                   hipStream_t s);
int build_colfused(int dtype, const uint32_t *off, const uint32_t *col, const void *val, size_t n_rows, size_t nnz, uint32_t shift,
                   size_t n_blocks, uint32_t rt, size_t *n_tiles_out, uint32_t **tile_row_out, uint32_t **seg_out, uint8_t **cnt_out,
                   uint32_t **col2_out, void **val2_out, bool *fits_out, hipStream_t s);
int launch_spmv_colfused(int dtype, uint32_t rt, const uint32_t *tile_row, size_t n_tiles, const uint32_t *seg, const uint8_t *cnt,
                         const uint32_t *col, const void *val, const void *x, void *y, size_t n_rows, size_t nnz, uint32_t n_blocks,
                         int device, hipStream_t s);
int build_colsplit(int dtype, const uint32_t *off, const uint32_t *col, const void *val, size_t n_rows, size_t nnz, uint32_t min_long,
                   size_t *n_long_out, size_t *nnz_long_out, uint32_t **long_rows_out, uint32_t **off_l_out, uint32_t **col_l_out, void **val_l_out,
                   uint32_t **off_s_out, uint32_t **col_s_out, void **val_s_out, hipStream_t s);
int launch_split_scatter(int dtype, const uint32_t *long_rows, const void *y_long, size_t n_long, void *y, hipStream_t s);
int assemble_triplets(int dtype, size_t n, const uint32_t *rows, const uint32_t *cols, const void *vals, const uint8_t *ops,
                      bool reverse_rows, bool all_set, bool repeats_adjacent, size_t *n_rows_out, size_t *n_cols_out, size_t *nnz_out,
                      uint32_t **off_out, uint32_t **col_out, void **val_out, hipStream_t s);
int expand_rows(const uint32_t *off, size_t n_rows, uint32_t *rows_out, hipStream_t s);
int column_lists_bucketed(const uint32_t *off, const uint32_t *col, size_t n_rows, size_t n_cols, size_t nnz, uint32_t max_col, uint32_t *col_ptr,
                          uint32_t *entries, bool *done, hipStream_t s);
int transpose_bucketed(int dtype, const uint32_t *off, const uint32_t *col, const void *val, size_t n_rows, size_t nnz, uint32_t max_col,
                       uint32_t **off_out, uint32_t **col_out, void **val_out, size_t *n_rows_out, size_t *n_cols_out, bool *done, hipStream_t s);
int append_to_row(int dtype, uint32_t *off, uint32_t **col, void **val, size_t n_rows, size_t *nnz, size_t row, uint32_t column,
                  const void *value_host, hipStream_t s);
int column_info(const uint32_t *off, const uint32_t *col, size_t n_rows, size_t n_cols, size_t nnz, uint32_t max_col, uint32_t *rows,
                uint32_t *col_ptr, uint32_t *entries, hipStream_t s);
int sort_rows(int dtype, const uint32_t *off, uint32_t *col, void *val, size_t n_rows, size_t nnz, uint32_t max_col,
              hipStream_t s);
int crs_is_sorted(const uint32_t *off, const uint32_t *col, size_t n_rows, int *out, hipStream_t s);
int crs_is_symmetric(int dtype, const uint32_t *off, const uint32_t *col, const void *val, size_t n_rows, int *out, hipStream_t s);
int prod_crs(int dtype, const uint32_t *a_off, const uint32_t *a_col, const void *a_val, size_t a_rows, size_t a_nnz, uint32_t a_max_col,
             const uint32_t *b_off, const uint32_t *b_col, const void *b_val, size_t b_rows, size_t *n_rows_out, size_t *n_cols_out,
             size_t *nnz_out, uint32_t **off_out, uint32_t **col_out, void **val_out, hipStream_t s);
struct AddOperand {
    const uint32_t *off = nullptr, *col = nullptr;
    const void *val = nullptr;
    size_t n_rows = 0, n_cols = 0, nnz = 0, orphans = 0;
    uint32_t max_row_len = 0, max_col = 0;
};
struct AddResult {
    size_t n_rows = 0, n_cols = 0, nnz = 0;
    CrsArrays arrays;
    int route = 0;
    bool values_only = false;
};
int add_crs(int dtype, bool subtract, const AddOperand &a, const AddOperand &b, bool in_place, bool alias, bool force_general, AddResult *res,
            hipStream_t s);
struct UpdMatrix {
    const uint32_t *off = nullptr, *col = nullptr;
    void *val = nullptr;
    size_t n_rows = 0, n_cols = 0, nnz = 0, orphans = 0;
    uint32_t max_row_len = 0;
};
struct UpdResult {
    size_t n_rows = 0, n_cols = 0, nnz = 0;
    CrsArrays arrays;
    int route = 0;
    bool values_only = false;
};
int crs_get_many(int dtype, const UpdMatrix &m, size_t n, const uint32_t *rows, const uint32_t *cols, void *values_out, hipStream_t s);
int crs_apply(int dtype, const UpdMatrix &m, size_t n, const uint32_t *rows, const uint32_t *cols, const void *vals, const uint8_t *ops,
              bool force_general, UpdResult *res, hipStream_t s);
int build_eye(int dtype, size_t dim, uint32_t *off, uint32_t *col, void *val, hipStream_t s);
int validate_permutation(const uint32_t *perm, size_t n, uint32_t *first, const char *what, hipStream_t s);
int permute_crs(int dtype, const uint32_t *a_off, const uint32_t *a_col, const void *a_val, size_t n_rows, size_t nnz, const uint32_t *row_perm,
                const uint32_t *col_inv, CrsArrays *out, hipStream_t s);
int launch_vec_permute(int dtype, void *dst, const void *src, const uint32_t *perm, size_t n, bool inverse, hipStream_t s);
int launch_bandwidth(const uint32_t *off, const uint32_t *col, size_t n_rows, uint32_t *d_out2, hipStream_t s);
int rcm_order(const uint32_t *off, const uint32_t *col, size_t n, size_t nnz, uint32_t *perm_out, size_t *n_components, size_t *n_levels, hipStream_t s);
int symmetrised_pattern(const uint32_t *off, const uint32_t *col, size_t n, size_t nnz, Scratch &scr, uint32_t **adj_off_out, uint32_t **adj_col_out,
                        hipStream_t s);
int color_order(const uint32_t *off, const uint32_t *col, size_t n, size_t nnz, uint32_t seed, uint32_t *colors_out, uint32_t *perm_out, size_t *n_colors,
                size_t *n_rounds, hipStream_t s);
constexpr uint32_t kPlanLongRun = 64;
struct UpdPlan {
    size_t n_ops = 0, n_targets = 0, n_live = 0, longest_run = 0, n_short = 0, device_bytes = 0;
    DevArray<uint32_t> pos;
    DevArray<uint32_t> off;
    DevArray<uint32_t> tgt;
    DevArray<uint32_t> setbits;
};
int crs_plan_targets(const UpdMatrix &m, size_t n, const uint32_t *rows, const uint32_t *cols, uint32_t *key_out, uint32_t *src_out,
                     uint64_t *n_absent_out, hipStream_t s);
int plan_build(size_t n, const uint32_t *key, const uint32_t *src, const uint8_t *ops, UpdPlan *plan, hipStream_t s);
int plan_execute(int dtype, const UpdPlan &plan, const void *values, void *m_val, bool from_zero, hipStream_t s);
struct RingPhase {
    uint32_t row_begin, row_end;
    uint32_t load_lo, load_hi;
    uint32_t use_ring;
    uint32_t band_lo[3], band_hi[3];
};
constexpr int kRingPhaseWords = 11;
int launch_tile_span(const uint32_t *off, const uint32_t *col, size_t n_rows, size_t n_tiles, uint32_t *cmin,
                     uint32_t *cmax, hipStream_t s);
struct RingCol12 {
    const uint8_t *lo8 = nullptr;
    const uint16_t *hdr = nullptr;
    const uint32_t *escapes = nullptr;
};
int launch_spmv_ring2(int dtype, int lanes, int chunks, const uint32_t *off, const uint32_t *col, const uint16_t *col16, const RingCol12 &c12,
                      const void *val, const void *x, void *y, size_t n_rows, size_t nnz, bool padded, unsigned n_blocks,
                      const uint32_t *phase_ptr, const RingPhase *phases, unsigned ring_entries, unsigned bands,
                      hipStream_t s, void *dot_partials = nullptr ,
                      unsigned block_begin = 0, unsigned block_end = ~0u );
int launch_tile_intervals(const uint32_t *off, const uint32_t *col, size_t n_rows, size_t tile_rows, size_t max_width,
                          uint32_t *win, uint32_t *d_count, hipStream_t s);
int launch_ring_band_codes(const uint32_t *off, const uint32_t *col, const uint32_t *win, size_t n_rows, uint32_t S,
                           uint16_t *code, hipStream_t s);
int launch_narrow_columns(const uint32_t *col, size_t nnz, uint16_t *col16, size_t n_out, hipStream_t s);
int launch_col12_count(const uint32_t *off, const uint32_t *col, size_t nnz, const RingPhase *phases, size_t n_phases, uint32_t *jobs,
                       unsigned long long *counts, hipStream_t s);
int launch_col12_encode(const uint32_t *col, size_t nnz, const uint32_t *jobs, size_t n_phases, size_t n_chunks_out, uint8_t *lo8,
                        uint16_t *hdr, uint32_t *escapes, unsigned long long *counts, hipStream_t s);
struct CrsStats {
    uint32_t max_row_len;
    uint32_t max_col;
    uint32_t min_col_inv;
    uint32_t bad;
};
int launch_crs_stats(const uint32_t *off, const uint32_t *col, size_t n_rows, size_t nnz, CrsStats *d_stats,
                     hipStream_t s);
void tiled_geometry(size_t n_rows, size_t n_cols, size_t nnz, int dtype, uint32_t *n_cb, uint32_t *rows_per_block, uint32_t *n_rb);
int tiled_build(::smh_crs *m);
uint32_t tiled_slice_columns(int dtype);
int columns_within_n_cols(const ::smh_crs *m, const char *what);
int tiled_array(::smh_crs *m, int which, void *out, size_t capacity_bytes, size_t *bytes_out);
int launch_spmv_tiled(::smh_crs *m, const void *x, size_t x_len, void *y, hipStream_t s);
size_t spmv_fused_dot_partials(::smh_crs *m, size_t x_len, int variant, bool any_lhs = false);
int spmv_enqueue(::smh_crs *m, const void *x, size_t x_len, void *y, int variant, hipStream_t s, void *dot_partials = nullptr,
                 const void *dot_lhs = nullptr);
int spmv_rows_granularity(::smh_crs *m, int variant, size_t *gran_out);
int spmv_enqueue_rows(::smh_crs *m, const void *x, size_t x_len, void *y, int variant, hipStream_t s, size_t row0, size_t row1,
                      void *dot_partials = nullptr, const void *dot_lhs = nullptr);
int spmv_enqueue_rows_short(::smh_crs *m, const void *x, size_t x_len, void *y, int variant, hipStream_t s, size_t row0, size_t row1);
enum class Ew { Add, Sub, Scale, Axpy, Xpby, RSubInto };
int launch_ew(int dtype, Ew op, void *x, const void *y, size_t n, double a, const void *a_dev, hipStream_t s);
int launch_dot(int dtype, const void *x, const void *y, size_t n, void *partials, void *result_dev,
               hipStream_t s);
int launch_fold2(int dtype, const void *in, size_t count, void *partials, void *result_dev, hipStream_t s);
int launch_scale_values(int dtype, void *v, size_t n, double a, hipStream_t s);
int ensure_tri_schedule(::smh_crs *m, int uplo);
int tri_lanes(const ::smh_crs *m);
int trisolve_enqueue(::smh_crs *m, int uplo, int diag, bool scale_rhs, const void *b, void *x, const uint32_t *active, hipStream_t s);

template <typename T>
struct CgScalars {
    T rr, rr_prev, pap, alpha, beta;
    uint32_t converged;
    uint32_t active;
    uint32_t entered;
    uint32_t pad_;
    uint64_t iters;
    uint64_t iter_max;
    double tol;
};
size_t cg_scalars_bytes(int dtype);
void cg_read_scalars(int dtype, const void *host_copy, int *converged, uint64_t *iters, double *rr);

template <typename Body>
int solve_in_batches(int dtype, hipStream_t s, size_t iter_max, size_t check_every, Body &&body, const void *d_sc, void *h_sc, int *converged,
                     size_t *iters, double *rr, bool capture = true) {
    Graph graph;
    GraphExec exec;
    if (capture && iter_max > check_every && hipStreamBeginCapture(s, hipStreamCaptureModeThreadLocal) == hipSuccess) {
        int crc = SMH_OK;
        for (size_t i = 0; i < check_every && crc == SMH_OK; ++i) crc = body();
        const hipError_t ce = graph.end_capture(s);
        if (crc != SMH_OK || ce != hipSuccess || !graph.get() || exec.instantiate(graph.get()) != hipSuccess)
            (void)hipGetLastError();
    } else {
        (void)hipGetLastError();
    }
    auto poll = [&]() -> int {
        SMH_HIP(hipMemcpyAsync(h_sc, d_sc, cg_scalars_bytes(dtype), hipMemcpyDeviceToHost, s));
        SMH_HIP(hipStreamSynchronize(s));
        uint64_t it64 = 0;
        cg_read_scalars(dtype, h_sc, converged, &it64, rr);
        *iters = (size_t)it64;
        return SMH_OK;
    };
    auto run = [&]() -> int {
        size_t launched = 0;
        while (launched < iter_max) {
            size_t batch = iter_max - launched < check_every ? iter_max - launched : check_every;
            if (exec.get()) {
                SMH_HIP(hipGraphLaunch(exec.get(), s));
                batch = check_every;
            } else {
                for (size_t i = 0; i < batch; ++i) SMH_TRY(body());
            }
            launched += batch;
            SMH_TRY(poll());
            if (*converged) break;
        }
        if (iter_max == 0) SMH_TRY(poll());
        return SMH_OK;
    };
    const int rc = run();
    if (rc != SMH_OK) (void)hipStreamSynchronize(s);
    return rc;
}

enum class Form {
    NotTried,
    Ready,
    Refused,
};
struct MergeTable {
    Form state = Form::NotTried;
    size_t n_tiles = 0;
    DevArray<uint32_t> tile_row, tile_nz, carry_row;
    DevArray<char> carry_val;
};
struct RingPlan {
    Form state = Form::NotTried;
    bool bands_tried = false;
    unsigned blocks = 0;
    double fraction = 0.0;
    unsigned entries = kRingEntries;
    unsigned bands = 1;
    size_t n_phases = 0;
    DevArray<uint32_t> phase_ptr;
    DevArray<RingPhase> phases;
    DevArray<uint32_t> win;
    DevArray<uint16_t> col16;
    Form c12 = Form::NotTried;
    uint64_t c12_chunks = 0, c12_escapes = 0;
    DevArray<uint8_t> lo8;
    DevArray<uint16_t> hdr;
    DevArray<uint32_t> escapes;
};
struct StreamCodes {
    Form state = Form::NotTried;
    DevArray<uint32_t> cwin;
    DevArray<uint16_t> code;
    DevArray<uint8_t> len8;
    DevArray<uint32_t> tbase;
    uint32_t xs_chunks = 0xFFFFFFFFu, xs_end = 0;
    uint64_t odd_rows = 0;
    bool direct = false;
    bool vdict = false;
    int vdict_xs = 0;
};
struct StreamDict {
    Form state = Form::NotTried;
    uint32_t n = 0;
    DevArray<char> values;
};
struct ColBlock {
    Form state = Form::NotTried;
    uint32_t shift = 0;
    size_t blocks = 0;
    int rpt = 1;
    bool single_pass = false;
    DevArray<uint32_t> off, col;
    DevArray<char> val;
};
struct ColFused {
    Form state = Form::NotTried;
    uint32_t shift = 0, rt = 0;
    size_t blocks = 0, tiles = 0;
    DevArray<uint32_t> seg, col, tile_row;
    DevArray<uint8_t> cnt;
    DevArray<char> val;
};
struct RowSplit {
    Form state = Form::NotTried;
    ::smh_crs *long_part = nullptr, *short_part = nullptr;
    DevArray<uint32_t> rows;
    DevArray<char> y;
    size_t n_long = 0;
    hipStream_t side = nullptr;
    hipEvent_t fork = nullptr, join = nullptr;
    RowSplit() = default;
    RowSplit(RowSplit &&o) noexcept { swap(o); }
    RowSplit &operator=(RowSplit &&o) noexcept {
        RowSplit old(std::move(*this));
        swap(o);
        return *this;
    }
    ~RowSplit();
    void swap(RowSplit &o) noexcept {
        std::swap(state, o.state); std::swap(long_part, o.long_part); std::swap(short_part, o.short_part);
        std::swap(rows, o.rows); std::swap(y, o.y); std::swap(n_long, o.n_long);
        std::swap(side, o.side); std::swap(fork, o.fork); std::swap(join, o.join);
    }
};
struct Tiled {
    Form state = Form::NotTried;
    uint32_t n_cb = 0, n_rb = 0, R = 0;
    uint64_t tot = 0;
    DevArray<char> val, prod;
    DevArray<uint16_t> code, row;
    DevArray<uint32_t> tstart;
    DevArray<uint32_t> rbstart;
    DevArray<uint32_t> cptr;
    DevArray<char> chunk;
    uint32_t n_chunks = 0, max_slice_chunks = 0;
    bool dups = false;
    uint64_t n_prod = 0;
};
struct TriSchedule {
    Form state = Form::NotTried;
    size_t n_levels = 0;
    uint64_t first_no_diag = ~0ull;
    DevArray<uint32_t> rows;
    DevArray<uint32_t> level_ptr;
    DevArray<uint32_t> level;
    DevArray<uint32_t> diagpos;
    struct Launch { uint32_t level_begin, level_end, row_begin, row_end; bool small; };
    std::vector<Launch> launches;
};
constexpr uint32_t kTriSmallRows = 128;
constexpr uint32_t kTriSmallBlock = 1024;
struct StageBuf {
    DevArray<char> d;
    size_t cap = 0;
    int ensure_cap(size_t bytes) {
        if (cap >= bytes && d.get()) return SMH_OK;
        cap = 0;
        const size_t want = bytes < 256 ? 256 : bytes;
        SMH_TRY(d.alloc(want));
        cap = want;
        return SMH_OK;
    }
};
struct Knobs {
    int forced_lanes = 0;
    int forced_chunks = 0;
    int stream_rows_per_thread = 0;
    uint32_t cb_forced_shift = 0;
    int use_ring = -1;
    int use_stream_xs = -1;
    int use_stream_direct = -1;
    int use_stream_vdict = -1;
    int use_col16 = -1;
    int use_col12 = -1;
};

}

namespace smh {
uint64_t next_crs_id();
}
struct smh_crs {
    uint64_t id = smh::next_crs_id();
    uint64_t epoch = 0;
    int dtype = SMH_F32;
    int device = 0;
    size_t n_rows = 0, n_cols = 0, nnz = 0;
    size_t orphans = 0;
    bool has_first_op = false;
    uint32_t first_row = 0, first_col = 0;
    uint64_t first_val_bits = 0;
    uint32_t *d_off = nullptr;
    uint32_t *d_col = nullptr;
    void *d_val = nullptr;
    bool owns = true;
    bool no_split = false;
    hipStream_t stream = nullptr;
    uint32_t max_row_len = 0;
    uint32_t max_col = 0;
    uint32_t min_col = 0;
    uint32_t max_tile_entries = 0;
    uint32_t max_tile512_entries = 0;
    bool have_stats = false;
    double span_fraction = 0.0;
    smh::Knobs knobs;
    smh::MergeTable merge;
    smh::RingPlan ring;
    smh::StreamCodes codes;
    smh::StreamDict dict;
    smh::ColBlock cb;
    smh::ColFused cf;
    smh::RowSplit split;
    smh::Tiled tiled;
// ... 31 lines not shown
```

sparsemat_amd/csrc/spmv_dispatch.hip:

```cpp
#include <cstdlib>

#include "crs_forms.hpp"

namespace smh {

static double mean_row(const smh_crs *m) { return m->n_rows ? (double)m->nnz / (double)m->n_rows : 0.0; }

static int mean_lanes(const smh_crs *m) {
    const double mean = mean_row(m);
    const double need = mean < 16.0 ? mean + 3.0 : mean;
    int lanes = 1;
    while (lanes < 64 && 4.0 * lanes < need) lanes <<= 1;
    return lanes;
}

int auto_lanes(const smh_crs *m) {
    if (m->knobs.forced_lanes) return m->knobs.forced_lanes;
    const double mean = mean_row(m);
    int lanes = mean_lanes(m);
    if (m->knobs.use_ring != 0) {
        if (mean >= 128.0) lanes = 16;
        else if (lanes > 32) lanes = 32;
        if (mean > 32.0 && m->ring.state == Form::Ready && m->ring.fraction < 0.5) lanes = 8;
    }
    return lanes;
}

static int auto_chunks(const smh_crs *m) {
    const int lanes = auto_lanes(m);
    if (m->knobs.forced_chunks) {
        if (lanes == 1) return m->knobs.forced_chunks;
        if (lanes == 2) return m->knobs.forced_chunks > 2 ? 2 : m->knobs.forced_chunks;
        return 1;
    }
    return 1;
}

uint32_t cb_shift_for(const smh_crs *m) { return m->knobs.cb_forced_shift ? m->knobs.cb_forced_shift : 19u; }
uint32_t cf_shift_for(const smh_crs *m) { return m->knobs.cb_forced_shift ? m->knobs.cb_forced_shift : 18u; }
size_t blocks_for(size_t n_cols, uint32_t shift) {
    const uint64_t w = 1ull << shift;
    const uint64_t b = ((uint64_t)n_cols + w - 1) / w;
    return (size_t)(b ? b : 1);
}
const size_t kColblockMinXBytes = 4u << 20;
static bool wants_colblock(const smh_crs *m) {
    const size_t b = blocks_for(m->n_cols, cb_shift_for(m));
    return m->n_cols * dtype_size(m->dtype) >= kColblockMinXBytes && m->span_fraction > 0.25 && b >= 2 && b <= 128;
}

static bool tiled_fits(const smh_crs *m, double min_tile = 32.0) {
    static const bool tiled_off = getenv("SMH_TILED") && atoi(getenv("SMH_TILED")) == 0;
    if (tiled_off || m->tiled.state == Form::Refused) return false;
    uint32_t n_cb = 0, R = 0, n_rb = 0;
    tiled_geometry(m->n_rows, m->n_cols, m->nnz, m->dtype, &n_cb, &R, &n_rb);
    const double tile = (double)m->nnz / (double)n_cb / (double)n_rb;
    return tile >= min_tile && (double)(n_rb + 1) * (double)n_cb * 4.0 <= (double)(1u << 30);
}

int resolve_variant(const smh_crs *m, int variant) {
    if (variant != SMH_SPMV_AUTO) return variant;
    if (wants_colblock(m)) {
        static const bool fused_off = getenv("SMH_COLBLOCK_FUSED") && atoi(getenv("SMH_COLBLOCK_FUSED")) == 0;
        if (fused_off || m->cf.state == Form::Refused || blocks_for(m->n_cols, cf_shift_for(m)) > 255) return SMH_SPMV_COLBLOCK;
        const double mean = mean_row(m);
        const double similar = 2.0 * mean + 8.0 > 128.0 ? 2.0 * mean + 8.0 : 128.0;
        if ((double)m->max_row_len <= similar) {
            const size_t blocks = blocks_for(m->n_cols, cf_shift_for(m));
            const bool pays = m->dtype == SMH_F32 ? tiled_fits(m)
                              : m->no_split       ? false
                                                  : tiled_fits(m, blocks >= 24 ? 12.0 : 32.0);
            if (pays) return SMH_SPMV_TILED;
            return SMH_SPMV_COLFUSED;
        }
        if (!m->no_split && tiled_fits(m, m->dtype == SMH_F64 && blocks_for(m->n_cols, cf_shift_for(m)) >= 24 ? 12.0 : 32.0)) return SMH_SPMV_TILED;
        static const bool split_off = getenv("SMH_COLBLOCK_SPLIT") && atoi(getenv("SMH_COLBLOCK_SPLIT")) == 0;
        const double vs = (double)dtype_size(m->dtype);
        const double sweeps = (double)blocks_for(m->n_cols, cb_shift_for(m)) * (double)m->n_rows * (4.0 + 2.0 * vs), entries = (double)m->nnz * (4.0 + vs);
        if (!split_off && !m->no_split && m->split.state != Form::Refused && sweeps >= 0.6 * entries) return SMH_SPMV_COLSPLIT;
        return SMH_SPMV_COLBLOCK;
    }
    const int lanes = mean_lanes(m);
    const double mean = mean_row(m);
    const bool short_ring_rows = mean > 8.0 && m->ring.state == Form::Ready && m->ring.fraction >= 0.5 && m->knobs.use_ring != 0;
    if (mean <= 12.0 && m->max_row_len <= 64 && !short_ring_rows) return SMH_SPMV_STREAM;
    if ((uint64_t)m->max_row_len >= 8ull * 4ull * (uint64_t)lanes && m->max_row_len > 64) return SMH_SPMV_MERGE;
    if (mean > 32.0 && mean <= 128.0 && m->ring.state == Form::Ready && m->ring.fraction < 0.5) return SMH_SPMV_STREAM;
    return SMH_SPMV_VECTOR;
}

static int launch_colblock(const smh_crs *m, const void *x, void *y, hipStream_t s) {
    for (size_t b = 0; b < m->cb.blocks; ++b)
        SMH_TRY(launch_spmv_stream_block(m->dtype, m->cb.off.get() + b * (m->n_rows + 1), m->cb.col.get(), m->cb.val.get(), x, y,
                                         m->n_rows, m->nnz, m->cb.rpt, m->cb.single_pass, b > 0, s));
    return SMH_OK;
}

static int stream_launch(smh_crs *m, const StreamCfg &c, const void *x, size_t x_len, void *y, hipStream_t s, void *dot_partials,
                         const void *dot_lhs, uint64_t t0, uint64_t t1) {
    const bool xs_ok = ((m->dtype == SMH_F64 ? x_len + 1 : ((x_len + 3) & ~(size_t)3)) >= (size_t)m->codes.xs_end) &&
                       (reinterpret_cast<uintptr_t>(x) & 15u) == 0;
    if (c.direct) {
        if (xs_ok && c.xs)
            return launch_spmv_stream_xd(m->dtype, m->d_val, x, y, m->n_rows, dot_partials, c.code, c.cwin, c.len8, c.tbase, dot_lhs, s,
                                         c.xs, t0, t1, c.dict, c.dict_high);
        return launch_spmv_stream(m->dtype, m->d_off, m->d_col, m->d_val, x, y, m->n_rows, m->nnz, m->owns, c.rpt, c.single_pass,
                                  dot_partials, nullptr, nullptr, nullptr, nullptr, dot_lhs, s, false, 0, t0, t1);
    }
    return launch_spmv_stream(m->dtype, m->d_off, m->d_col, m->d_val, x, y, m->n_rows, m->nnz, m->owns, c.rpt, c.single_pass,
                              dot_partials, c.code, c.cwin, c.len8, c.tbase, dot_lhs, s, c.small, xs_ok ? c.xs : 0, t0, t1);
}

static int launch_ring(smh_crs *m, const void *x, void *y, hipStream_t s, void *dot_partials = nullptr, unsigned b0 = 0, unsigned b1 = ~0u) {
    return launch_spmv_ring2(m->dtype, auto_lanes(m), auto_chunks(m), m->d_off, m->d_col, m->ring.col16.get(),
                             RingCol12{m->ring.lo8.get(), m->ring.hdr.get(), m->ring.escapes.get()}, m->d_val, x, y, m->n_rows, m->nnz,
                             m->owns || m->nnz % 4 == 0, m->ring.blocks, m->ring.phase_ptr.get(), m->ring.phases.get(), m->ring.entries,
                             m->ring.bands, s, dot_partials, b0, b1);
}

size_t spmv_fused_dot_partials(smh_crs *m, size_t x_len, int variant, bool any_lhs) {
    if (const char *e = getenv("SMH_CG_FUSED_DOT")) {
        if (atoi(e) == 0) return 0;
    }
    if (resolve_variant(m, variant) != SMH_SPMV_STREAM) return 0;
    if (!any_lhs && (m->n_rows != m->n_cols || x_len < m->n_rows)) return 0;
    StreamCfg c;
    if (stream_cfg(m, &c) != SMH_OK) return 0;
    return stream_tiles(m->n_rows, c.rpt);
}

static int x_covers_columns(const smh_crs *m, size_t x_len) {
    if (m->nnz > 0 && (size_t)m->max_col >= x_len)
        return fail(SMH_ERR_INDEX_RANGE, "index out of bounds: the len is %zu but the index is %u", x_len, m->max_col);
    return SMH_OK;
}

struct Resolved {
    int v = SMH_SPMV_AUTO;
    bool ring = false;
    StreamCfg stream;
};

static int build_forms(smh_crs *m, Resolved *r, bool eager) {
    switch (r->v) {
        case SMH_SPMV_VECTOR: return vector_uses_ring(m, &r->ring);
        case SMH_SPMV_SEQ: return SMH_OK;
        case SMH_SPMV_STREAM: return stream_cfg(m, &r->stream, eager);
        case SMH_SPMV_COLSPLIT:
            SMH_TRY(ensure_split(m));
            if (m->split.state != Form::Ready) return ensure_colblock(m);
            if (eager) {
                SMH_TRY(smh_crs_prepare(m->split.short_part, SMH_SPMV_AUTO));
                return smh_crs_prepare(m->split.long_part, SMH_SPMV_AUTO);
            }
            return SMH_OK;
        case SMH_SPMV_COLFUSED:
            SMH_TRY(ensure_colfused(m));
            return (m->cf.state == Form::Ready) ? SMH_OK : ensure_colblock(m);
        case SMH_SPMV_COLBLOCK: return ensure_colblock(m);
        case SMH_SPMV_TILED: return tiled_build(m);
        case SMH_SPMV_MERGE: return ensure_merge_ws(m);
        default: return fail(SMH_ERR_INVALID, "unknown SpMV variant %d", r->v);
    }
}

static int resolve_and_build(smh_crs *m, int variant, bool eager, Resolved *r) {
    for (;;) {
        r->v = resolve_variant(m, variant);
        const int rc = build_forms(m, r, eager);
        if (rc == SMH_OK || variant != SMH_SPMV_AUTO || rc == SMH_ERR_INDEX_RANGE || resolve_variant(m, variant) == r->v) return rc;
        clear_error();
    }
}

int prepare_forms(smh_crs *m, int variant) {
    Resolved r;
    return resolve_and_build(m, variant, true, &r);
}

int spmv_enqueue(smh_crs *m, const void *x, size_t x_len, void *y, int variant, hipStream_t s, void *dot_partials, const void *dot_lhs) {
    SMH_TRY(x_covers_columns(m, x_len));
    Resolved r;
    SMH_TRY(resolve_and_build(m, variant, false, &r));
    switch (r.v) {
        case SMH_SPMV_VECTOR:
            if (r.ring) return launch_ring(m, x, y, s);
            return launch_spmv_vector(m->dtype, auto_lanes(m), m->d_off, m->d_col, m->d_val, x, y, m->n_rows, m->nnz, s);
        case SMH_SPMV_SEQ:
            return launch_spmv_seq(m->dtype, m->d_off, m->d_col, m->d_val, x, y, m->n_rows, s);
        case SMH_SPMV_STREAM:
            return stream_launch(m, r.stream, x, x_len, y, s, dot_partials, dot_lhs, 0, ~uint64_t(0));
        case SMH_SPMV_COLSPLIT:
            if (m->split.state == Form::Ready) {
                static const bool overlap = getenv("SMH_COLSPLIT_OVERLAP") && atoi(getenv("SMH_COLSPLIT_OVERLAP")) != 0;
                hipStream_t sl = overlap ? m->split.side : s;
                if (overlap) {
                    SMH_HIP(hipEventRecord(m->split.fork, s));
                    SMH_HIP(hipStreamWaitEvent(sl, m->split.fork, 0));
                }
                SMH_TRY(spmv_enqueue(m->split.long_part, x, x_len, m->split.y.get(), SMH_SPMV_AUTO, sl));
                if (overlap) SMH_HIP(hipEventRecord(m->split.join, sl));
                SMH_TRY(spmv_enqueue(m->split.short_part, x, x_len, y, SMH_SPMV_AUTO, s));
                if (overlap) SMH_HIP(hipStreamWaitEvent(s, m->split.join, 0));
                return launch_split_scatter(m->dtype, m->split.rows.get(), m->split.y.get(), m->split.n_long, y, s);
            }
            return launch_colblock(m, x, y, s);
        case SMH_SPMV_COLFUSED:
            if (m->cf.state == Form::Ready)
                return launch_spmv_colfused(m->dtype, m->cf.rt, m->cf.tile_row.get(), m->cf.tiles, m->cf.seg.get(), m->cf.cnt.get(), m->cf.col.get(), m->cf.val.get(),
                                            x, y, m->n_rows, m->nnz, (uint32_t)m->cf.blocks, m->device, s);
            [[fallthrough]];
        case SMH_SPMV_COLBLOCK:
            return launch_colblock(m, x, y, s);
        case SMH_SPMV_TILED:
            return launch_spmv_tiled(m, x, x_len, y, s);
        case SMH_SPMV_MERGE:
            return launch_spmv_merge(m->dtype, m->d_off, m->d_col, m->d_val, x, y, m->n_rows, m->nnz, m->merge.n_tiles,
                                     m->merge.tile_row.get(), m->merge.tile_nz.get(), m->merge.carry_row.get(), m->merge.carry_val.get(), s);
        default:
            return fail(SMH_ERR_INVALID, "unknown SpMV variant %d", variant);
    }
}

static int resolve_rows(smh_crs *m, int variant, Resolved *r, size_t *gran_out) {
    *gran_out = 0;
    if (m->n_rows == 0) return SMH_OK;
    r->v = resolve_variant(m, variant);
    if (r->v == SMH_SPMV_STREAM) {
        SMH_TRY(stream_cfg(m, &r->stream));
        *gran_out = (size_t)kStreamRows * (size_t)r->stream.rpt;
    } else if (r->v == SMH_SPMV_VECTOR) {
        SMH_TRY(vector_uses_ring(m, &r->ring));
        if (r->ring && m->ring.blocks) {
            const size_t n_tiles = (m->n_rows + 63) / 64;
            *gran_out = ((n_tiles + m->ring.blocks - 1) / m->ring.blocks) * 64;
        }
    }
    return SMH_OK;
}
int spmv_rows_granularity(smh_crs *m, int variant, size_t *gran_out) {
    Resolved r;
    return resolve_rows(m, variant, &r, gran_out);
}

int spmv_enqueue_rows(smh_crs *m, const void *x, size_t x_len, void *y, int variant, hipStream_t s, size_t row0, size_t row1,
                      void *dot_partials, const void *dot_lhs) {
    SMH_TRY(x_covers_columns(m, x_len));
    if (row1 > m->n_rows) row1 = m->n_rows;
    if (row0 >= row1) return SMH_OK;
    Resolved r;
    size_t gran = 0;
    SMH_TRY(resolve_rows(m, variant, &r, &gran));
    if (gran == 0 || row0 % gran || (row1 % gran && row1 != m->n_rows))
        return fail(SMH_ERR_INVALID, "rows [%zu, %zu) cannot be launched on their own (granularity %zu)", row0, row1, gran);
    if (r.v == SMH_SPMV_STREAM)
        return stream_launch(m, r.stream, x, x_len, y, s, dot_partials, dot_lhs, row0 / gran, (row1 + gran - 1) / gran);
    if (dot_partials) return fail(SMH_ERR_INVALID, "a product by parts with the dot epilogue needs the CSR-stream kernel");
    return launch_ring(m, x, y, s, nullptr, (unsigned)(row0 / gran), (unsigned)((row1 + gran - 1) / gran));
}

int spmv_enqueue_rows_short(smh_crs *m, const void *x, size_t x_len, void *y, int variant, hipStream_t s, size_t row0, size_t row1) {
    static const bool off = getenv("SMH_PAR_BOUNDARY_K1") && atoi(getenv("SMH_PAR_BOUNDARY_K1")) == 0;
    if (row1 > m->n_rows) row1 = m->n_rows;
    if (row0 >= row1) return SMH_OK;
    if (!off && resolve_variant(m, variant) == SMH_SPMV_VECTOR && auto_lanes(m) >= 4 && row1 - row0 <= (size_t)1 << 20) {
        bool ring = false;
        SMH_TRY(vector_uses_ring(m, &ring));
        if (ring) {
            SMH_TRY(x_covers_columns(m, x_len));
            return launch_spmv_vector(m->dtype, auto_lanes(m), m->d_off + row0, m->d_col, m->d_val, x, (char *)y + row0 * dtype_size(m->dtype), row1 - row0,
// ... 30 lines not shown
```

sparsemat_amd/csrc/spmv_ring2.hip:

```cpp
#include "internal.hpp"
#include "ring_col12.hpp"

#include <atomic>
#include <type_traits>

namespace smh {

typedef uint32_t u32x4 __attribute__((ext_vector_type(4)));
typedef uint32_t u32x2 __attribute__((ext_vector_type(2)));
typedef float f32x4 __attribute__((ext_vector_type(4)));
typedef double f64x2 __attribute__((ext_vector_type(2)));

#ifndef SMH_RING2_THREADS64
#define SMH_RING2_THREADS64 1024
#endif
template <typename T, int RING> struct Ring2Cfg {
    static constexpr bool kBig = (size_t)RING * sizeof(T) > 65536;
    static constexpr int kThreads = kBig ? (sizeof(T) == 8 ? SMH_RING2_THREADS64 : 1024) : 512;
    static constexpr int kWavesPerSimd = (kBig ? 1 : 2) * (kThreads / 64) / 4;
};
#ifndef SMH_RING2_SB
#define SMH_RING2_SB 2
#endif
constexpr int kRing2SB = SMH_RING2_SB;
#ifndef SMH_RING2_SB64
#define SMH_RING2_SB64 1
#endif
#ifndef SMH_RING2_SADDR
#define SMH_RING2_SADDR 0
#endif
#if SMH_RING2_SADDR
#define SMH_R2_OFF(rel, size) ((size_t)((rel) * (size)))
#else
#define SMH_R2_OFF(rel, size) ((size_t)(rel) * (size))
#endif

template <typename T, int NCH>
struct Unit {
    uint32_t o0, o1;
    uint32_t c[NCH][4];
    T v[NCH][4];
};

template <typename T, int LANES>
__device__ __forceinline__ uint32_t lane_pos(uint32_t j, int q) {
    if constexpr (sizeof(T) == 8) return q < 2 ? 2u * j + (uint32_t)q : 2u * LANES + 2u * j + (uint32_t)(q - 2);
    else return 4u * j + (uint32_t)q;
}

enum : int { kColU32 = 0, kCol16 = 1, kCol12 = 2 };
struct ColStream {
    const void *colp;
    const uint16_t *hdrp;
    const uint16_t *table;
    const u32x2 *escapes;
};
template <typename T, int CF, int LANES>
__device__ __forceinline__ void load_chunk_nb(const ColStream &cs, const T *__restrict__ valp, uint32_t pass_rel, uint32_t j,
                                              uint32_t last_rel, uint32_t (&c)[4], T (&v)[4]) {
    const void *colp = cs.colp;
    if constexpr (sizeof(T) == 4) {
        uint32_t rel = pass_rel + 4u * j;
        rel = rel < last_rel ? rel : last_rel;
        if constexpr (CF == kCol12) {
            c[0] = __builtin_nontemporal_load(reinterpret_cast<const uint32_t *>(reinterpret_cast<const char *>(colp) + SMH_R2_OFF(rel, 1u)));
            c[1] = __builtin_nontemporal_load(reinterpret_cast<const uint16_t *>(reinterpret_cast<const char *>(cs.hdrp) + (SMH_R2_OFF(rel, 1u) >> 1)));
        } else if constexpr (CF == kCol16) {
            const u32x2 cc = __builtin_nontemporal_load(reinterpret_cast<const u32x2 *>(
                reinterpret_cast<const char *>(colp) + SMH_R2_OFF(rel, 2u)));
            c[0] = cc.x; c[1] = cc.y;
        } else {
            const u32x4 cc = __builtin_nontemporal_load(reinterpret_cast<const u32x4 *>(
                reinterpret_cast<const char *>(colp) + SMH_R2_OFF(rel, 4u)));
            c[0] = cc.x; c[1] = cc.y; c[2] = cc.z; c[3] = cc.w;
        }
        const f32x4 a = __builtin_nontemporal_load(reinterpret_cast<const f32x4 *>(
            reinterpret_cast<const char *>(valp) + SMH_R2_OFF(rel, 4u)));
        v[0] = a.x; v[1] = a.y; v[2] = a.z; v[3] = a.w;
    } else {
        uint32_t e0 = pass_rel + 2u * j, e1 = pass_rel + 2u * LANES + 2u * j;
        e0 = e0 < last_rel + 2u ? e0 : last_rel + 2u;
        e1 = e1 < last_rel + 2u ? e1 : last_rel + 2u;
        static_assert(CF != kCol12, "the compact column form is an f32 form");
        if constexpr (CF == kCol16) {
            c[0] = __builtin_nontemporal_load(reinterpret_cast<const uint32_t *>(reinterpret_cast<const char *>(colp) + SMH_R2_OFF(e0, 2u)));
            c[1] = __builtin_nontemporal_load(reinterpret_cast<const uint32_t *>(reinterpret_cast<const char *>(colp) + SMH_R2_OFF(e1, 2u)));
        } else {
            const u32x2 c0 = __builtin_nontemporal_load(reinterpret_cast<const u32x2 *>(reinterpret_cast<const char *>(colp) + SMH_R2_OFF(e0, 4u)));
            const u32x2 c1 = __builtin_nontemporal_load(reinterpret_cast<const u32x2 *>(reinterpret_cast<const char *>(colp) + SMH_R2_OFF(e1, 4u)));
            c[0] = c0.x; c[1] = c0.y; c[2] = c1.x; c[3] = c1.y;
        }
        const f64x2 a = __builtin_nontemporal_load(reinterpret_cast<const f64x2 *>(reinterpret_cast<const char *>(valp) + SMH_R2_OFF(e0, 8u)));
        const f64x2 b = __builtin_nontemporal_load(reinterpret_cast<const f64x2 *>(reinterpret_cast<const char *>(valp) + SMH_R2_OFF(e1, 8u)));
        v[0] = a.x; v[1] = a.y; v[2] = b.x; v[3] = b.y;
    }
}

template <int CF, int RING>
__device__ __forceinline__ void chunk_slots(const uint32_t (&c)[4], const ColStream &cs, uint32_t (&slot)[4]) {
    constexpr uint32_t MASK = RING - 1;
    if constexpr (CF == kCol12) {
        static_assert(RING == (int)col12::kSlots, "the compact column form holds slots of the 16384-slot ring");
        col12::decode_chunk(c[1], c[0], cs.table, slot);
        const bool escaped = col12::is_escape(c[1]);
        if (__builtin_amdgcn_ballot_w64(escaped) != 0) {
            if (escaped) {
                const u32x2 e = cs.escapes[c[0]];
                col12::unpack_escape(e.x, e.y, slot);
            }
        }
    } else {
#pragma unroll
        for (int q = 0; q < 4; ++q) {
            if constexpr (CF == kCol16) slot[q] = (q & 1) ? ((c[q >> 1] >> 16) & MASK) : (c[q >> 1] & MASK);
            else slot[q] = c[q] & MASK;
        }
    }
}

__device__ __forceinline__ float r2_fma(float a, float b, float c) { return __builtin_fmaf(a, b, c); }
__device__ __forceinline__ double r2_fma(double a, double b, double c) { return __builtin_fma(a, b, c); }

template <typename T, int NCH>
__device__ __forceinline__ void load_offsets(Unit<T, NCH> &u, const uint32_t *__restrict__ off, uint64_t base,
                                             uint64_t row_end, uint32_t lane) {
    uint64_t r0 = base + lane, r1 = base + lane + 1;
    r0 = r0 < row_end ? r0 : row_end;
    r1 = r1 < row_end ? r1 : row_end;
    u.o0 = off[r0];
    u.o1 = off[r1];
}

template <int LANES>
__device__ __forceinline__ void row_bounds(uint32_t o0, uint32_t o1, int t, uint32_t lane, uint32_t nnz_lim,
                                           uint32_t &s, uint32_t &e) {
    if constexpr (LANES == 1) {
        s = o0;
        e = o1;
    } else {
        constexpr int RPS = kWave / LANES;
        const int src = t * RPS + (int)(lane / LANES);
        s = (uint32_t)__shfl((int)o0, src, kWave);
        e = (uint32_t)__shfl((int)o1, src, kWave);
    }
    s = s < nnz_lim ? s : nnz_lim;
    e = e < nnz_lim ? e : nnz_lim;
}

template <typename T, int LANES, int CH, int SB, int CF>
__device__ __forceinline__ void issue_unit(Unit<T, SB * CH> &u, const ColStream &cs,
                                           const T *__restrict__ valp, uint32_t kb, uint32_t nnz_lim, uint32_t last_rel,
                                           uint32_t lane) {
    const uint32_t j = lane % LANES;
#pragma unroll
    for (int t = 0; t < SB; ++t) {
        uint32_t s, e;
        row_bounds<LANES>(u.o0, u.o1, t, lane, nnz_lim, s, e);
        s = s > kb ? s : kb;
#pragma unroll
        for (int ch = 0; ch < CH; ++ch) {
            load_chunk_nb<T, CF, LANES>(cs, valp, (s & ~3u) - kb + 4u * (uint32_t)(ch * LANES), j, last_rel, u.c[t * CH + ch], u.v[t * CH + ch]);
        }
    }
}

template <typename T, int LANES, int CH, int SB, int GM, int CF, int RING, bool DOT = false>
__device__ __forceinline__ void consume_unit(const Unit<T, SB * CH> &u, uint64_t base, uint64_t row_end,
                                             const ColStream &cs, const T *__restrict__ valp,
                                             const T *__restrict__ x, const T *ring, T *__restrict__ y, uint32_t kb,
                                             uint32_t nnz_lim, uint32_t last_rel, uint32_t lane, T *dacc = nullptr) {
    constexpr int RPS = kWave / LANES;
    const uint32_t j = lane % LANES;
    T out = T(0);
#pragma unroll
    for (int t = 0; t < SB; ++t) {
        uint32_t s, e;
        row_bounds<LANES>(u.o0, u.o1, t, lane, nnz_lim, s, e);
        s = s > kb ? s : kb;
        e = e > s ? e : s;
        const uint32_t sa = s & ~3u;
        const uint32_t lo = s - sa;
        const uint32_t len = e - sa;
        T sum = T(0);
#pragma unroll
        for (int ch = 0; ch < CH; ++ch) {
            uint32_t slot[4];
            if constexpr (GM == 1) chunk_slots<CF, RING>(u.c[t * CH + ch], cs, slot);
#pragma unroll
            for (int q = 0; q < 4; ++q) {
                const uint32_t rel = 4u * (uint32_t)(ch * LANES) + lane_pos<T, LANES>(j, q);
                const bool in = rel >= lo && rel < len;
                T xv;
                if constexpr (GM == 1) xv = ring[slot[q]];
                else if constexpr (GM == 2) xv = __builtin_nontemporal_load(&x[in ? u.c[t * CH + ch][q] : 0u]);
                else xv = x[in ? u.c[t * CH + ch][q] : 0u];
                const T f = r2_fma(u.v[t * CH + ch][q], xv, sum);
                sum = in ? f : sum;
            }
        }
        for (uint32_t pass = 4u * (uint32_t)(CH * LANES); pass + lane_pos<T, LANES>(j, 0) < len; pass += 4u * LANES) {
            uint32_t cc[4];
            T vv[4];
            load_chunk_nb<T, CF, LANES>(cs, valp, sa - kb + pass, j, last_rel, cc, vv);
            uint32_t slot[4];
            if constexpr (GM == 1) chunk_slots<CF, RING>(cc, cs, slot);
#pragma unroll
            for (int q = 0; q < 4; ++q) {
                const bool in = pass + lane_pos<T, LANES>(j, q) < len;
                T xv;
                if constexpr (GM == 1) xv = ring[slot[q]];
                else if constexpr (GM == 2) xv = __builtin_nontemporal_load(&x[in ? cc[q] : 0u]);
                else xv = x[in ? cc[q] : 0u];
                const T f = r2_fma(vv[q], xv, sum);
                sum = in ? f : sum;
            }
        }
        if constexpr (LANES == 1) {
            out = sum;
        } else {
#pragma unroll
            for (int o = LANES / 2; o > 0; o >>= 1) sum += __shfl_xor(sum, o, kWave);
            const T got = __shfl(sum, (int)((lane % RPS) * LANES), kWave);
            out = ((int)(lane / RPS) == t) ? got : out;
        }
    }
    const uint64_t row = base + lane;
    if constexpr (DOT) {
        if (lane < (uint32_t)(SB * RPS) && row < row_end) *dacc = r2_fma(y[row], out, *dacc);
    } else {
        if (lane < (uint32_t)(SB * RPS) && row < row_end) y[row] = out;
    }
}

template <typename T, int LANES, int CH, int GM, int CF, int RING, bool DOT = false>
__device__ __forceinline__ void phase_rows(const uint32_t *__restrict__ off, const ColStream &cols,
                                           const T *__restrict__ val, const T *__restrict__ x, const T *ring,
                                           T *__restrict__ y, uint64_t rb, uint64_t re, uint32_t nnz_lim,
                                           uint64_t last_chunk, uint32_t wave, uint32_t lane, T *dacc = nullptr) {
    constexpr int STEPS = LANES;
    constexpr int SBMAX = sizeof(T) == 8 ? SMH_RING2_SB64 : kRing2SB;
    constexpr int SB = STEPS < SBMAX ? STEPS : SBMAX;
    constexpr int RU = SB * (kWave / LANES);
    constexpr uint64_t STRIDE = (uint64_t)(Ring2Cfg<T, RING>::kThreads / kWave) * RU;
    uint64_t base = rb + (uint64_t)wave * RU;
    if (base >= re) return;
    uint32_t kb = __builtin_amdgcn_readfirstlane(off[rb]) & ~3u;
    kb = kb < (uint32_t)last_chunk ? kb : (uint32_t)last_chunk;
    const uint32_t last_rel = (uint32_t)last_chunk - kb;
    ColStream cs = cols;
    cs.colp = reinterpret_cast<const char *>(cols.colp) + (size_t)kb * (CF == kCol12 ? 1u : CF == kCol16 ? 2u : 4u);
    if constexpr (CF == kCol12) cs.hdrp = cols.hdrp + (kb >> 2);
    const T *valp = val + kb;
    Unit<T, SB * CH> A, B, N;
    load_offsets(A, off, base, re, lane);
    load_offsets(B, off, base + STRIDE, re, lane);
    issue_unit<T, LANES, CH, SB, CF>(A, cs, valp, kb, nnz_lim, last_rel, lane);
    for (;;) {
        if (base + STRIDE >= re) {
            consume_unit<T, LANES, CH, SB, GM, CF, RING, DOT>(A, base, re, cs, valp, x, ring, y, kb, nnz_lim, last_rel, lane, dacc);
            break;
        }
        load_offsets(N, off, base + 2 * STRIDE, re, lane);
        issue_unit<T, LANES, CH, SB, CF>(B, cs, valp, kb, nnz_lim, last_rel, lane);
        consume_unit<T, LANES, CH, SB, GM, CF, RING, DOT>(A, base, re, cs, valp, x, ring, y, kb, nnz_lim, last_rel, lane, dacc);
        A.o0 = N.o0; A.o1 = N.o1;
        base += STRIDE;
        if (base + STRIDE >= re) {
            consume_unit<T, LANES, CH, SB, GM, CF, RING, DOT>(B, base, re, cs, valp, x, ring, y, kb, nnz_lim, last_rel, lane, dacc);
            break;
        }
        load_offsets(N, off, base + 2 * STRIDE, re, lane);
        issue_unit<T, LANES, CH, SB, CF>(A, cs, valp, kb, nnz_lim, last_rel, lane);
        consume_unit<T, LANES, CH, SB, GM, CF, RING, DOT>(B, base, re, cs, valp, x, ring, y, kb, nnz_lim, last_rel, lane, dacc);
        B.o0 = N.o0; B.o1 = N.o1;
        base += STRIDE;
    }
}

__device__ const col12::Table k_col12_table = col12::make_table();

template <typename T, int LANES, int CH, int CF, int RING, bool DOT = false>
__global__ void __launch_bounds__((Ring2Cfg<T, RING>::kThreads), (Ring2Cfg<T, RING>::kWavesPerSimd))
k_spmv_ring2(const uint32_t *__restrict__ off, const uint32_t *__restrict__ col, const uint16_t *__restrict__ col16, RingCol12 c12,
             const T *__restrict__ val, const T *__restrict__ x, T *__restrict__ y, uint32_t nnz_lim, uint64_t last_chunk,
             const uint32_t *__restrict__ phase_ptr, const RingPhase *__restrict__ phases, uint32_t bands,
             T *__restrict__ dot_partials, uint32_t lb0, uint32_t lb_n) {
    T dacc_v = T(0);
    T *dacc = DOT ? &dacc_v : nullptr;
    extern __shared__ __attribute__((aligned(16))) unsigned char ring_raw[];
    T *ring = reinterpret_cast<T *>(ring_raw);
    const uint32_t MASK = (bands == 4u ? (uint32_t)RING / 4u : (uint32_t)RING) - 1u;
    constexpr int kRing2Threads = Ring2Cfg<T, RING>::kThreads;
    const uint32_t per_xcd = gridDim.x >> 3;
    const uint32_t lb_rel = (blockIdx.x & 7u) * per_xcd + (blockIdx.x >> 3);
    if (lb_rel >= lb_n) return;
    const uint32_t lb = lb0 + lb_rel;
    const uint32_t wave = __builtin_amdgcn_readfirstlane(threadIdx.x / kWave);
    const uint32_t lane = threadIdx.x & (kWave - 1);
    const uint32_t p0 = phase_ptr[lb], p1 = phase_ptr[lb + 1];
    ColStream ring_cols = {CF == kCol16 ? (const void *)col16 : (const void *)col, nullptr, nullptr, nullptr};
    const ColStream wide_cols = {col, nullptr, nullptr, nullptr};
    if constexpr (CF == kCol12) {
        static_assert(kRing2Threads * sizeof(uint32_t) == sizeof(col12::Table), "one dword of the table per thread");
        uint16_t *table = reinterpret_cast<uint16_t *>(ring_raw + (size_t)RING * sizeof(T));
        reinterpret_cast<uint32_t *>(table)[threadIdx.x] = reinterpret_cast<const uint32_t *>(k_col12_table.e)[threadIdx.x];
        __syncthreads();
        ring_cols = {c12.lo8, c12.hdr, table, reinterpret_cast<const u32x2 *>(c12.escapes)};
    }
    for (uint32_t p = p0; p < p1; ++p) {
        const RingPhase ph = phases[p];
        const bool more = bands == 4u && (ph.band_hi[0] > ph.band_lo[0] || ph.band_hi[1] > ph.band_lo[1] || ph.band_hi[2] > ph.band_lo[2]);
        if (ph.load_hi > ph.load_lo || more) {
            __syncthreads();
            for (uint64_t cidx = (uint64_t)ph.load_lo + threadIdx.x; cidx < ph.load_hi; cidx += kRing2Threads)
                ring[cidx & MASK] = x[cidx];
            if (more) {
#pragma unroll
                for (uint32_t k = 0; k < 3; ++k)
                    for (uint64_t cidx = (uint64_t)ph.band_lo[k] + threadIdx.x; cidx < ph.band_hi[k]; cidx += kRing2Threads)
                        ring[(k + 1u) * (MASK + 1u) + (cidx & MASK)] = x[cidx];
            }
            __syncthreads();
        }
        if (ph.use_ring == 1)
            phase_rows<T, LANES, CH, 1, CF, RING, DOT>(off, ring_cols, val, x, ring, y, ph.row_begin, ph.row_end, nnz_lim, last_chunk, wave,
                                                       lane, dacc);
        else if (ph.use_ring == 2)
            phase_rows<T, LANES, CH, 2, kColU32, RING, DOT>(off, wide_cols, val, x, ring, y, ph.row_begin, ph.row_end, nnz_lim, last_chunk, wave,
                                                          lane, dacc);
        else
            phase_rows<T, LANES, CH, 0, kColU32, RING, DOT>(off, wide_cols, val, x, ring, y, ph.row_begin, ph.row_end, nnz_lim, last_chunk, wave,
                                                          lane, dacc);
    }
    if constexpr (DOT) {
        __shared__ T s_dot[kRing2Threads / kWave];
        T d = dacc_v;
#pragma unroll
        for (int o = kWave / 2; o > 0; o >>= 1) d += __shfl_down(d, o, kWave);
        if (lane == 0) s_dot[wave] = d;
        __syncthreads();
        if (threadIdx.x == 0) {
            T t = T(0);
            for (int w = 0; w < kRing2Threads / kWave; ++w) t += s_dot[w];
            dot_partials[blockIdx.x] = t;
        }
    }
}

template <typename T>
__global__ void k_ring2_tail(const uint32_t *__restrict__ off, const uint32_t *__restrict__ col,
                             const T *__restrict__ val, const T *__restrict__ x, T *__restrict__ y, uint64_t n_rows,
                             uint64_t k_begin, uint64_t nnz) {
    if (blockIdx.x != 0 || threadIdx.x != 0) return;
    uint64_t r = n_rows - 1;
    while (r > 0 && (uint64_t)off[r] > k_begin) --r;
    for (uint64_t k = k_begin; k < nnz; ++k) {
        while ((uint64_t)off[r + 1] <= k) ++r;
        y[r] = r2_fma(val[k], x[col[k]], y[r]);
    }
}

template <typename T>
__global__ void k_ring2_tail_dot(const uint32_t *__restrict__ off, const uint32_t *__restrict__ col, const T *__restrict__ val,
                                 const T *__restrict__ x, const T *__restrict__ lhs, T *__restrict__ out, uint64_t n_rows, uint64_t k_begin,
                                 uint64_t nnz) {
    if (blockIdx.x != 0 || threadIdx.x != 0) return;
    uint64_t r = n_rows - 1;
    while (r > 0 && (uint64_t)off[r] > k_begin) --r;
    T acc = T(0);
    for (uint64_t k = k_begin; k < nnz; ++k) {
        while ((uint64_t)off[r + 1] <= k) ++r;
        acc = r2_fma(lhs[r], val[k] * x[col[k]], acc);
    }
    *out = acc;
}

__global__ void __launch_bounds__(kBlock)
k_narrow_columns(const uint32_t *__restrict__ col, uint64_t nnz, uint64_t n_out, uint16_t *__restrict__ col16) {
    for (uint64_t k = (uint64_t)blockIdx.x * blockDim.x + threadIdx.x; k < n_out; k += (uint64_t)gridDim.x * blockDim.x)
        col16[k] = k < nnz ? (uint16_t)col[k] : (uint16_t)0;
}

int launch_narrow_columns(const uint32_t *col, size_t nnz, uint16_t *col16, size_t n_out, hipStream_t s) {
    if (n_out == 0) return SMH_OK;
    uint64_t blocks = (n_out + kBlock - 1) / kBlock;
    if (blocks > 8192) blocks = 8192;
    hipLaunchKernelGGL(k_narrow_columns, dim3((unsigned)blocks), dim3(kBlock), 0, s, col, (uint64_t)nnz, (uint64_t)n_out, col16);
    SMH_HIP(hipGetLastError());
    return SMH_OK;
}

__global__ void __launch_bounds__(kBlock)
k_col12_jobs(const uint32_t *__restrict__ off, const RingPhase *__restrict__ phases, uint32_t n_phases, u32x2 *__restrict__ jobs,
             unsigned long long *__restrict__ counts) {
    const uint32_t p = blockIdx.x * blockDim.x + threadIdx.x;
    if (p >= n_phases) return;
    const uint32_t e0 = off[phases[p].row_begin], e1 = off[phases[p].row_end];
    uint32_t cb = e0 >> 2, ce = (uint32_t)(((uint64_t)e1 + 3u) >> 2);
    if (phases[p].use_ring != 1u || e1 <= e0) {
        cb = ce = 0;
    } else if (e0 & 3u) {
        uint32_t q = p;
        while (q > 0 && off[phases[q - 1].row_begin] == e0) --q;
        if (q > 0 && phases[q - 1].use_ring == 1u) ++cb;
    }
    jobs[p] = u32x2{cb, ce > cb ? ce : cb};
    if (ce > cb) atomicAdd(&counts[0], (unsigned long long)(ce - cb));
}

template <bool COUNT>
__global__ void __launch_bounds__(kBlock)
k_col12_encode(const uint32_t *__restrict__ col, uint64_t nnz, const u32x2 *__restrict__ jobs, uint32_t n_jobs, uint32_t *__restrict__ lo,
               uint16_t *__restrict__ hdr, u32x2 *__restrict__ escapes, unsigned long long *__restrict__ counts) {
    unsigned long long mine = 0;
    for (uint32_t job = blockIdx.x; job < n_jobs; job += gridDim.x) {
        const u32x2 range = jobs[job];
        for (uint64_t c = (uint64_t)range.x + threadIdx.x; c < range.y; c += kBlock) {
            uint32_t slot[4];
#pragma unroll
            for (int q = 0; q < 4; ++q) slot[q] = (4u * c + q < nnz ? col[4u * c + q] : 0u) & (col12::kSlots - 1u);
            uint16_t h = 0;
            uint32_t l = 0;
            const bool ok = col12::encode_chunk(slot, &h, &l);
            if constexpr (COUNT) {
                mine += ok ? 0u : 1u;
            } else {
                if (!ok) {
                    l = (uint32_t)atomicAdd(&counts[1], 1ull);
                    h = (uint16_t)col12::kEscape;
                    uint32_t pair[2];
                    col12::pack_escape(slot, pair);
                    escapes[l] = u32x2{pair[0], pair[1]};
                }
                lo[c] = l;
                hdr[c] = h;
            }
        }
    }
    if constexpr (COUNT) {
        if (mine) atomicAdd(&counts[1], mine);
    }
}

int launch_col12_count(const uint32_t *off, const uint32_t *col, size_t nnz, const RingPhase *phases, size_t n_phases, uint32_t *jobs,
                       unsigned long long *counts, hipStream_t s) {
    SMH_HIP(hipMemsetAsync(counts, 0, 2 * sizeof(unsigned long long), s));
    if (n_phases == 0) return SMH_OK;
    hipLaunchKernelGGL(k_col12_jobs, dim3((unsigned)((n_phases + kBlock - 1) / kBlock)), dim3(kBlock), 0, s, off, phases, (uint32_t)n_phases,
                       reinterpret_cast<u32x2 *>(jobs), counts);
    SMH_HIP(hipGetLastError());
    hipLaunchKernelGGL(k_col12_encode<true>, dim3((unsigned)(n_phases < 8192 ? n_phases : 8192)), dim3(kBlock), 0, s, col, (uint64_t)nnz,
                       reinterpret_cast<const u32x2 *>(jobs), (uint32_t)n_phases, (uint32_t *)nullptr, (uint16_t *)nullptr, (u32x2 *)nullptr, counts);
    SMH_HIP(hipGetLastError());
    return SMH_OK;
}

int launch_col12_encode(const uint32_t *col, size_t nnz, const uint32_t *jobs, size_t n_phases, size_t n_chunks_out, uint8_t *lo8,
                        uint16_t *hdr, uint32_t *escapes, unsigned long long *counts, hipStream_t s) {
    SMH_HIP(hipMemsetAsync(lo8, 0, n_chunks_out * 4, s));
    SMH_HIP(hipMemsetAsync(hdr, 0, n_chunks_out * sizeof(uint16_t), s));
    SMH_HIP(hipMemsetAsync(counts + 1, 0, sizeof(unsigned long long), s));
    if (n_phases == 0) return SMH_OK;
    hipLaunchKernelGGL(k_col12_encode<false>, dim3((unsigned)(n_phases < 8192 ? n_phases : 8192)), dim3(kBlock), 0, s, col, (uint64_t)nnz,
                       reinterpret_cast<const u32x2 *>(jobs), (uint32_t)n_phases, reinterpret_cast<uint32_t *>(lo8), hdr,
                       reinterpret_cast<u32x2 *>(escapes), counts);
    SMH_HIP(hipGetLastError());
    return SMH_OK;
}

template <typename T, int RING>
static int launch_ring2_t(int lanes, int chunks, const uint32_t *off, const uint32_t *col, const uint16_t *col16, const RingCol12 &c12, const T *val,
                          const T *x, T *y, size_t n_rows, size_t nnz, bool padded, unsigned n_blocks,
                          const uint32_t *phase_ptr, const RingPhase *phases, uint32_t bands, T *dot_partials, hipStream_t s,
                          unsigned block_begin, unsigned block_end) {
    if (bands == 4u && !col16) return fail(SMH_ERR_INVALID, "banded ring plan without the 16-bit slot array");
    constexpr bool kHasCol12 = std::is_same<T, float>::value && RING == (int)col12::kSlots;
    if (c12.lo8 && (!kHasCol12 || bands != 1u || !c12.hdr || !c12.escapes))
        return fail(SMH_ERR_INVALID, "ring kernel: the compact column form is for f32 on the single-window ring of 16384 columns");
    const unsigned lb0 = block_begin < n_blocks ? block_begin : n_blocks, lb1 = block_end < n_blocks ? block_end : n_blocks;
    const bool whole = lb0 == 0 && lb1 == n_blocks;
    if (!whole && dot_partials) return fail(SMH_ERR_INVALID, "ring kernel: the DOT form takes the whole plan");
    if (lb1 <= lb0) return SMH_OK;
    const uint64_t nnz_lim = padded ? nnz : (nnz & ~uint64_t(3));
    if (dot_partials) SMH_HIP(hipMemsetAsync(dot_partials, 0, ((size_t)n_blocks + 1) * sizeof(T), s));
    if (nnz_lim == 0) {
        if (!dot_partials && lb1 == n_blocks) SMH_HIP(hipMemsetAsync(y, 0, n_rows * sizeof(T), s));
    } else {
        const uint64_t last_chunk = (nnz_lim - 1) & ~uint64_t(3);
        dim3 grid(((lb1 - lb0) + 7u) & ~7u), block(Ring2Cfg<T, RING>::kThreads);
        constexpr size_t ring_bytes = (size_t)RING * sizeof(T);
#define SMH_R2_LAUNCH2(L, C, N, D)                                                                                       \
    do {                                                                                                                 \
        constexpr size_t lds_bytes = ring_bytes + ((N) == kCol12 ? sizeof(col12::Table) : 0);                            \
                  \
        static std::atomic<uint64_t> attr_mask{0};                                                                       \
        const uint64_t dev_bit = 1ull << (unsigned)(current_device() & 63);                                              \
        if (!(attr_mask.load(std::memory_order_acquire) & dev_bit)) {                                                    \
            SMH_HIP(hipFuncSetAttribute(reinterpret_cast<const void *>(&k_spmv_ring2<T, L, C, N, RING, D>),               \
                                        hipFuncAttributeMaxDynamicSharedMemorySize, (int)lds_bytes));                    \
            attr_mask.fetch_or(dev_bit, std::memory_order_release);                                                      \
        }                                                                                                                \
        hipLaunchKernelGGL((k_spmv_ring2<T, L, C, N, RING, D>), grid, block, lds_bytes, s, off, col, col16, c12, val, x, y, \
                           (uint32_t)nnz_lim, last_chunk, phase_ptr, phases, bands, dot_partials, (uint32_t)lb0,         \
                           (uint32_t)(lb1 - lb0));                                                                       \
    } while (0)
#define SMH_R2_LAUNCH1(L, C, N)                                                            \
    do {                                                                                   \
        if (dot_partials) SMH_R2_LAUNCH2(L, C, N, true); else SMH_R2_LAUNCH2(L, C, N, false); \
    } while (0)
#define SMH_R2_LAUNCH(L, C)                                                   \
    do {                                                                      \
        if (c12.lo8) {                                                        \
            if constexpr (kHasCol12) SMH_R2_LAUNCH1(L, C, kCol12);            \
        } else if (col16) SMH_R2_LAUNCH1(L, C, kCol16);                       \
        else SMH_R2_LAUNCH1(L, C, kColU32);                                   \
    } while (0)
        switch (lanes * 16 + chunks) {
            case 1 * 16 + 1: SMH_R2_LAUNCH(1, 1); break;
            case 1 * 16 + 2: SMH_R2_LAUNCH(1, 2); break;
            case 1 * 16 + 3: SMH_R2_LAUNCH(1, 3); break;
            case 2 * 16 + 1: SMH_R2_LAUNCH(2, 1); break;
            case 2 * 16 + 2: SMH_R2_LAUNCH(2, 2); break;
            case 4 * 16 + 1: SMH_R2_LAUNCH(4, 1); break;
            case 8 * 16 + 1: SMH_R2_LAUNCH(8, 1); break;
            case 16 * 16 + 1: SMH_R2_LAUNCH(16, 1); break;
            case 32 * 16 + 1: SMH_R2_LAUNCH(32, 1); break;
            case 64 * 16 + 1: SMH_R2_LAUNCH(64, 1); break;
            default:
                return fail(SMH_ERR_INVALID, "ring kernel: unsupported (lanes per row, chunks per lane) = (%d, %d)", lanes, chunks);
        }
#undef SMH_R2_LAUNCH
#undef SMH_R2_LAUNCH1
#undef SMH_R2_LAUNCH2
        SMH_HIP(hipGetLastError());
    }
    if (nnz_lim != nnz && lb1 == n_blocks) {
        if (dot_partials)
            hipLaunchKernelGGL(k_ring2_tail_dot<T>, dim3(1), dim3(64), 0, s, off, col, val, x, (const T *)y, dot_partials + n_blocks,
                               (uint64_t)n_rows, nnz_lim, (uint64_t)nnz);
        else
            hipLaunchKernelGGL(k_ring2_tail<T>, dim3(1), dim3(64), 0, s, off, col, val, x, y, (uint64_t)n_rows, nnz_lim, (uint64_t)nnz);
        SMH_HIP(hipGetLastError());
    }
    return SMH_OK;
}

int launch_spmv_ring2(int dtype, int lanes, int chunks, const uint32_t *off, const uint32_t *col, const uint16_t *col16, const RingCol12 &c12,
                      const void *val, const void *x, void *y, size_t n_rows, size_t nnz, bool padded, unsigned n_blocks,
                      const uint32_t *phase_ptr, const RingPhase *phases, unsigned ring_entries, unsigned bands,
                      hipStream_t s, void *dot_partials, unsigned block_begin, unsigned block_end) {
    if (n_rows == 0) return SMH_OK;
    if (bands != 1u && bands != 4u) return fail(SMH_ERR_INVALID, "ring kernel: %u bands", bands);
    if (dtype == SMH_F64) {
        if (ring_entries != (unsigned)kRingEntries) return fail(SMH_ERR_INVALID, "f64 ring kernel: ring of %u columns", ring_entries);
        return launch_ring2_t<double, kRingEntries>(lanes, chunks, off, col, col16, c12, (const double *)val, (const double *)x,
                                                    (double *)y, n_rows, nnz, padded, n_blocks, phase_ptr, phases, bands,
                                                    (double *)dot_partials, s, block_begin, block_end);
    }
    if (ring_entries == (unsigned)kRingEntriesWide)
        return launch_ring2_t<float, kRingEntriesWide>(lanes, chunks, off, col, col16, c12, (const float *)val, (const float *)x,
                                                       (float *)y, n_rows, nnz, padded, n_blocks, phase_ptr, phases, bands,
                                                       (float *)dot_partials, s, block_begin, block_end);
    if (ring_entries != (unsigned)kRingEntries) return fail(SMH_ERR_INVALID, "ring kernel: ring of %u columns", ring_entries);
    return launch_ring2_t<float, kRingEntries>(lanes, chunks, off, col, col16, c12, (const float *)val, (const float *)x, (float *)y,
                                               n_rows, nnz, padded, n_blocks, phase_ptr, phases, bands, (float *)dot_partials, s, block_begin, block_end);
}

}
```

sparsemat_amd/sparsemat_crs.py:

```python
import ctypes as C
import numbers

import numpy as np

from . import _lib
from ._lib import check, lib
from .densevec import DenseVec
from .multivec import MultiVec, pack_host


def _index(i):
    i = int(i)
    if not 0 <= i <= 0xFFFFFFFF:
        raise _lib.SparseMatPanic(_lib.SMH_ERR_INVALID, "index %d does not fit the u32 index type" % i)
    return i


class SparseMatCRS:
    def __init__(self, handle, dtype, keep=None):
        self._h = handle
        self._dtype = np.dtype(dtype)
        self._keep = keep

    @classmethod
# ... 364 lines not shown
        check(lib().smh_crs_scale(self._h, float(a)))

    def update_values(self, values):
        values = np.ascontiguousarray(values, dtype=self._dtype)
        assert len(values) == self.n_non_zero_entries()
        check(lib().smh_crs_update_values(self._h, values.ctypes.data))

    def resolved_variant(self):
        v, lanes = C.c_int(), C.c_int()
        check(lib().smh_crs_resolved_variant(self._h, C.byref(v), C.byref(lanes)))
        return {1: "vector", 2: "merge", 3: "seq", 4: "stream", 5: "colblock", 6: "colfused", 7: "colsplit", 8: "tiled"}[v.value], lanes.value

    def set_colblock_shift(self, shift):
        check(lib().smh_crs_set_colblock_shift(self._h, shift))

    def tiled_layout(self, arrays=False):
        a, b, c, d, e, f = C.c_uint32(), C.c_uint32(), C.c_uint32(), C.c_uint32(), C.c_size_t(), C.c_size_t()
        check(lib().smh_crs_tiled_layout(self._h, C.byref(a), C.byref(b), C.byref(c), C.byref(d), C.byref(e)))
        check(lib().smh_crs_tiled_products(self._h, C.byref(f)))
        out = {"n_slices": a.value, "slice_columns": b.value, "rows_per_block": c.value, "n_row_blocks": d.value, "copy_entries": e.value,
               "n_products": f.value}
        if arrays:
            kinds = (("slice_chunks", np.uint32), ("chunks", np.uint32), ("codes", np.uint16), ("values", self.dtype), ("product_rows", np.uint16),
                     ("row_block_start", np.uint32), ("tile_start", np.uint32), ("products", self.dtype))
            for which, (name, dt) in enumerate(kinds):
                n = C.c_size_t()
                check(lib().smh_crs_tiled_array(self._h, which, None, 0, C.byref(n)))
                buf = np.empty(n.value // np.dtype(dt).itemsize, dtype=dt)
                check(lib().smh_crs_tiled_array(self._h, which, buf.ctypes.data, buf.nbytes, None))
                out[name] = buf
            out["chunks"] = out["chunks"].reshape(-1, 2)
            out["tile_start"] = out["tile_start"].reshape(d.value + 1, a.value)
        return out

    def colsplit_flag(self):
        flag = C.c_int()
        check(lib().smh_crs_colsplit(self._h, C.byref(flag), None, None, None, None, None))
        return bool(flag.value)

    def colsplit(self):
        flag, ml, nl = C.c_int(), C.c_uint32(), C.c_size_t()
        check(lib().smh_crs_colsplit(self._h, C.byref(flag), C.byref(ml), C.byref(nl), None, None, None))
        out = {"split": bool(flag.value), "min_long": ml.value, "n_long": nl.value}
        if out["split"]:
            rows = np.zeros(nl.value, np.uint32)
            hl, hs = C.c_void_p(), C.c_void_p()
            check(lib().smh_crs_colsplit(self._h, None, None, None, rows.ctypes.data, C.byref(hl), C.byref(hs)))
            out["long_rows"] = rows
            for name, h in (("long", hl), ("short", hs)):
                nr, nnz = lib().smh_crs_n_rows(h), lib().smh_crs_nnz(h)
                off, col, val = np.zeros(nr + 1, np.uint32), np.zeros(nnz, np.uint32), np.zeros(nnz, self._dtype)
                check(lib().smh_crs_download(h, off.ctypes.data, col.ctypes.data if nnz else None, val.ctypes.data if nnz else None))
                var, lanes = C.c_int(), C.c_int()
                check(lib().smh_crs_resolved_variant(h, C.byref(var), C.byref(lanes)))
                out[name] = (nr, off, col, val)
                out[name + "_variant"] = {1: "vector", 2: "merge", 3: "seq", 4: "stream", 5: "colblock", 6: "colfused", 7: "colsplit", 8: "tiled"}[var.value]
        return out

    def colfused(self, arrays=True):
        fits, sh, nb, rt, nt = C.c_int(), C.c_uint32(), C.c_size_t(), C.c_uint32(), C.c_size_t()
        check(lib().smh_crs_colfused(self._h, C.byref(fits), C.byref(sh), C.byref(nb), C.byref(rt), C.byref(nt), None, None, None, None, None))
        out = {"fits": bool(fits.value), "shift": sh.value, "n_blocks": nb.value, "rows_per_lane": rt.value, "n_tiles": nt.value}
        if arrays and out["fits"]:
            nnz = self.n_non_zero_entries()
            tiles = np.zeros(nt.value + 1, np.uint32)
            seg = np.zeros(nt.value * nb.value + 1, np.uint32)
            cnt = np.zeros(nt.value * nb.value * 64 * rt.value, np.uint8)
            col = np.zeros(nnz, np.uint32)
            val = np.zeros(nnz, self._dtype)
            check(lib().smh_crs_colfused(self._h, None, None, None, None, None, tiles.ctypes.data, seg.ctypes.data,
                                         cnt.ctypes.data if len(cnt) else None, col.ctypes.data if nnz else None,
                                         val.ctypes.data if nnz else None))
            out.update(tile_rows=tiles, segments=seg, counts=cnt, columns=col, values=val)
        return out

    def colblock(self, arrays=True):
        sh, nb, rpt, span = C.c_uint32(), C.c_size_t(), C.c_int(), C.c_double()
        check(lib().smh_crs_colblock(self._h, C.byref(sh), C.byref(nb), C.byref(rpt), C.byref(span), None, None, None))
        out = dict(shift=sh.value, n_blocks=nb.value, rows_per_thread=rpt.value, span_fraction=span.value)
        if arrays:
            nnz = self.n_non_zero_entries()
            off = np.zeros((nb.value, self.n_rows() + 1), dtype=np.uint32)
            col = np.zeros(nnz, dtype=np.uint32)
            val = np.zeros(nnz, dtype=self._dtype)
            check(lib().smh_crs_colblock(self._h, None, None, None, None, off.ctypes.data,
                                         col.ctypes.data if nnz else None, val.ctypes.data if nnz else None))
            out.update(offsets=off, columns=col, values=val)
        return out

    def set_vector_lanes(self, lanes):
        check(lib().smh_crs_set_vector_lanes(self._h, lanes))

    def set_stream_xs(self, mode):
        check(lib().smh_crs_set_stream_xs(self._h, mode))

    def set_stream_direct(self, mode):
        check(lib().smh_crs_set_stream_direct(self._h, mode))

    def stream_direct(self):
        a = C.c_int()
        check(lib().smh_crs_stream_direct(self._h, C.byref(a)))
        return bool(a.value)

    def stream_value_dict(self):
        n = C.c_int()
        buf = np.zeros(32, dtype=self.dtype)
        check(lib().smh_crs_stream_value_dict(self._h, C.byref(n), buf.ctypes.data))
        return buf[:n.value].copy()

    def set_stream_value_dict(self, mode):
        check(lib().smh_crs_set_stream_value_dict(self._h, int(mode)))

    def stream_layout(self):
        a, b, c, d = C.c_int(), C.c_int(), C.c_int(), C.c_int()
        check(lib().smh_crs_stream_layout(self._h, C.byref(a), C.byref(b), C.byref(c), C.byref(d)))
        return {"coded": bool(a.value), "byte_lengths": bool(b.value), "small_tiles": bool(c.value), "xs_chunks": d.value}

    def set_vector_chunks(self, chunks):
        check(lib().smh_crs_set_vector_chunks(self._h, chunks))

    def set_ring(self, mode):
        check(lib().smh_crs_set_ring(self._h, mode))

    def ring_entries(self):
        out = C.c_uint32()
        check(lib().smh_crs_ring_entries(self._h, C.byref(out)))
        return out.value

    def ring_column_form(self):
        out = C.c_int()
        check(lib().smh_crs_ring_column_form(self._h, C.byref(out)))
        return ("u32", "col16", "col12")[out.value]

    def ring_bands(self, intervals=False):
        bands = C.c_uint32()
        check(lib().smh_crs_ring_bands(self._h, C.byref(bands), None))
        if not intervals:
            return bands.value
        if bands.value != 4:
            return bands.value, None
        table = np.zeros(((self.n_rows() + 63) // 64, 4, 2), dtype=np.uint32)
        check(lib().smh_crs_ring_bands(self._h, C.byref(bands), table.ctypes.data))
        return bands.value, table

    def ring_plan(self):
        nb, nph, frac, act = C.c_uint32(), C.c_size_t(), C.c_double(), C.c_int()
        check(lib().smh_crs_ring_plan(self._h, C.byref(nb), C.byref(nph), C.byref(frac), C.byref(act), None, None))
        ptr = np.zeros(nb.value + 1, dtype=np.uint32)
        ph = np.zeros((nph.value, 11), dtype=np.uint32)
        check(lib().smh_crs_ring_plan(self._h, None, None, None, None, ptr.ctypes.data,
                                      ph.ctypes.data if nph.value else None))
        return nb.value, frac.value, bool(act.value), ptr, ph

    def max_row_len(self):
        out = C.c_uint32()
        check(lib().smh_crs_max_row_len(self._h, C.byref(out)))
        return out.value

    def col_range(self):
        lo, hi = C.c_uint32(), C.c_uint32()
        check(lib().smh_crs_col_range(self._h, C.byref(lo), C.byref(hi)))
        return lo.value, hi.value

    def merge_table(self):
        n = lib().smh_crs_merge_tiles(self._h)
        rows = np.zeros(n + 1, dtype=np.uint32)
        nz = np.zeros(n + 1, dtype=np.uint32)
        check(lib().smh_crs_merge_table(self._h, rows.ctypes.data, nz.ctypes.data))
        return rows, nz, lib().smh_crs_merge_tile_items(self._h)

    def mvp(self, rhs, variant="auto"):
        var = _lib.VARIANTS[variant]
        if isinstance(rhs, DenseVec):
            ret = DenseVec.zeros(self.n_rows(), self._dtype)
            check(lib().smh_crs_spmv_vec(self._h, rhs._h, ret._h, var))
            return ret
        x = np.ascontiguousarray(rhs, dtype=self._dtype)
        y = np.zeros(self.n_rows(), dtype=self._dtype)
        check(lib().smh_crs_spmv(self._h, x.ctypes.data if x.size else None, x.size,
                                 y.ctypes.data if y.size else None, var))
        return y

    def mvp_many(self, rhs):
        if isinstance(rhs, MultiVec):
            ret = MultiVec.zeros(self.n_rows(), rhs.count(), self._dtype)
            check(lib().smh_crs_spmv_many(self._h, rhs._h, ret._h))
            return ret
        x = pack_host(rhs, self._dtype)
        y = np.zeros((x.shape[0], self.n_rows()), dtype=self._dtype)
        check(lib().smh_crs_spmv_many_host(self._h, x.ctypes.data if x.size else None, x.shape[1], x.shape[0],
                                           y.ctypes.data if y.size else None))
        return y

    def mvp_many_dev(self, x_ptr, x_len, y_ptr, k, ld, stream=None):
        check(lib().smh_crs_spmv_many_dev(self._h, C.c_void_p(x_ptr), x_len, C.c_void_p(y_ptr), k, ld, C.c_void_p(stream or 0)))

    def __mul__(self, rhs):
        if isinstance(rhs, numbers.Real):
            ret = self.clone()
            ret.scale(rhs)
            return ret
        return self.mvp(rhs)

    def __imul__(self, rhs):
        if isinstance(rhs, numbers.Real):
            self.scale(rhs)
            return self
        return NotImplemented

    def inner_prod(self, lhs, rhs, variant="auto"):
        out = C.c_double()
        var = _lib.VARIANTS[variant]
        if isinstance(lhs, DenseVec) and isinstance(rhs, DenseVec):
            check(lib().smh_crs_inner_prod_vec(self._h, lhs._h, rhs._h, var, C.byref(out)))
            return out.value
        a = np.ascontiguousarray(lhs, dtype=self._dtype)
        b = np.ascontiguousarray(rhs, dtype=self._dtype)
        check(lib().smh_crs_inner_prod(self._h, a.ctypes.data if a.size else None, a.size,
                                       b.ctypes.data if b.size else None, b.size, var, C.byref(out)))
        return out.value

    def prepare(self, variant="auto"):
        check(lib().smh_crs_prepare(self._h, _lib.VARIANTS[variant]))

    def prepare_stats(self, variant="auto"):
        ms, nb = C.c_double(), C.c_size_t()
        check(lib().smh_crs_prepare_stats(self._h, _lib.VARIANTS[variant], C.byref(ms), C.byref(nb)))
        return ms.value, nb.value

    def mvp_dev(self, x_ptr, x_len, y_ptr, variant="auto", stream=None):
        check(lib().smh_crs_spmv_dev(self._h, C.c_void_p(x_ptr), x_len, C.c_void_p(y_ptr),
                                     _lib.VARIANTS[variant], C.c_void_p(stream or 0)))


class UpdatePlan:

    def __init__(self, handle, matrix, n_ops):
        self._h = handle
        self._m = matrix
        self._n = n_ops

    def execute(self, values, from_zero=False):
        values = np.asarray(values)
        dtype = self._m._dtype
        if values.dtype.kind == "f" and values.dtype != dtype:
            raise _lib.SparseMatPanic(_lib.SMH_ERR_INVALID, "values are %s, the matrix holds %s" % (values.dtype, dtype))
        values = np.ascontiguousarray(values, dtype=dtype)
        if len(values) != self._n:
            raise _lib.SparseMatPanic(_lib.SMH_ERR_INVALID, "the plan holds %d operations, values has %d" % (self._n, len(values)))
        check(lib().smh_update_plan_execute(self._h, self._m._h, values.ctypes.data if self._n else None, 1 if from_zero else 0))

    def execute_dev(self, vals_ptr, from_zero=False):
        check(lib().smh_update_plan_execute_dev(self._h, self._m._h, C.c_void_p(vals_ptr or 0), 1 if from_zero else 0))

    def stats(self):
        names = ("n_ops", "n_targets", "n_live_ops", "longest_run", "long_run_threshold", "device_bytes")
        out = [C.c_size_t(0) for _ in names]
        check(lib().smh_update_plan_stats(self._h, *[C.byref(o) for o in out]))
        return {k: int(o.value) for k, o in zip(names, out)}

    def __del__(self):
        h, self._h = getattr(self, "_h", None), None
        if h:
            try:
                lib().smh_update_plan_destroy(h)
            except Exception:
                pass
```

Before: 8098.

## Compute row offsets arithmetically for ring phases with uniform row length

Adds a plan-time kernel that checks, for each ring phase, whether every row has the same length, and records that length per phase. When all phases use the ring and at least one is regular, a new kernel specialization computes row start and end offsets as e0 + i*L instead of loading them from the row-offset array. This removes the per-unit offset loads and their latency from the software-pipelined loop. In exchange it adds another template instantiation, a per-phase branch, and an extra plan-time kernel with a host readback.

```diff
diff --git a/include/sparsemat_hip.h b/include/sparsemat_hip.h
--- a/include/sparsemat_hip.h
+++ b/include/sparsemat_hip.h
@@ -138,6 +138,7 @@
 int smh_crs_ring_plan(smh_crs *m, uint32_t *n_blocks_out, size_t *n_phases_out,
                       double *ring_fraction_out, int *active_out, uint32_t *phase_ptr_out,
                       uint32_t *phases_out);
+int smh_crs_ring_regular(smh_crs *m, uint32_t *len_out);
 
 int smh_crs_set_colblock_shift(smh_crs *m, uint32_t shift);
 int smh_crs_colblock(smh_crs *m, uint32_t *shift_out, size_t *n_blocks_out, int *rows_per_thread_out,
diff --git a/rust/src/ffi.rs b/rust/src/ffi.rs
--- a/rust/src/ffi.rs
+++ b/rust/src/ffi.rs
@@ -92,6 +92,7 @@
     pub fn smh_crs_permute_symmetric_dev(a: *const smh_crs, perm_dev: *const u32, n_perm: usize, out: *mut *mut smh_crs) -> c_int;
     pub fn smh_crs_bandwidth(m: *const smh_crs, lower_out: *mut u32, upper_out: *mut u32) -> c_int;
     pub fn smh_crs_span_fraction(m: *mut smh_crs, out: *mut f64) -> c_int;
+    pub fn smh_crs_ring_regular(m: *mut smh_crs, len_out: *mut u32) -> c_int;
     pub fn smh_crs_rcm(m: *const smh_crs, perm_out: *mut u32, n_components_out: *mut usize, n_levels_out: *mut usize) -> c_int;
     pub fn smh_crs_rcm_dev(m: *const smh_crs, perm_out_dev: *mut u32, n_components_out: *mut usize, n_levels_out: *mut usize) -> c_int;
     pub fn smh_crs_color(m: *const smh_crs, seed: u32, colors_out: *mut u32, perm_out: *mut u32, n_colors_out: *mut usize, n_rounds_out: *mut usize) -> c_int;
diff --git a/sparsemat_amd/_lib.py b/sparsemat_amd/_lib.py
--- a/sparsemat_amd/_lib.py
+++ b/sparsemat_amd/_lib.py
@@ -95,6 +95,7 @@
     "smh_crs_ring_entries": (_int, [_vp, _u32p]),
     "smh_crs_ring_column_form": (_int, [_vp, C.POINTER(_int)]),
     "smh_crs_ring_bands": (_int, [_vp, _u32p, _vp]),
+    "smh_crs_ring_regular": (_int, [_vp, _vp]),
     "smh_crs_ring_plan": (_int, [_vp, _u32p, C.POINTER(_sz), C.POINTER(C.c_double), C.POINTER(_int), _vp, _vp]),
     "smh_crs_set_colblock_shift": (_int, [_vp, C.c_uint32]),
     "smh_crs_tiled_layout": (_int, [_vp, _u32p, _u32p, _u32p, _u32p, C.POINTER(_sz)]),
diff --git a/sparsemat_amd/csrc/capi.hip b/sparsemat_amd/csrc/capi.hip
--- a/sparsemat_amd/csrc/capi.hip
+++ b/sparsemat_amd/csrc/capi.hip
@@ -1225,6 +1225,14 @@
     return SMH_OK;
 }
 
+int smh_crs_ring_regular(smh_crs *m, uint32_t *len_out) {
+    if (!m || !len_out) return fail(SMH_ERR_INVALID, "NULL argument");
+    SMH_TRY(ensure_ring_plan(m));
+    if (m->ring.n_phases)
+        SMH_HIP(hipMemcpy(len_out, m->ring.reg_len.get(), m->ring.n_phases * sizeof(uint32_t), hipMemcpyDeviceToHost));
+    return SMH_OK;
+}
+
 int smh_crs_ring_column_form(smh_crs *m, int *form_out) {
     if (!m || !form_out) return fail(SMH_ERR_INVALID, "NULL argument");
     bool ring = false;
diff --git a/sparsemat_amd/csrc/crs_forms.hip b/sparsemat_amd/csrc/crs_forms.hip
--- a/sparsemat_amd/csrc/crs_forms.hip
+++ b/sparsemat_amd/csrc/crs_forms.hip
@@ -123,6 +123,19 @@
     SMH_HIP(hipMemcpy(p.phase_ptr.get(), phase_ptr.data(), phase_ptr.size() * sizeof(uint32_t), hipMemcpyHostToDevice));
     if (!phases.empty())
         SMH_HIP(hipMemcpy(p.phases.get(), phases.data(), phases.size() * sizeof(RingPhase), hipMemcpyHostToDevice));
+    SMH_TRY(p.reg_len.alloc(phases.size() + 1));
+    if (!phases.empty()) {
+        std::vector<uint32_t> h_reg(phases.size());
+        SMH_TRY(read_back(p.reg_len.get(), h_reg.data(), phases.size(), m->stream, [&](uint32_t *d_reg) {
+            return launch_ring_regular(m->d_off, p.phases.get(), phases.size(), d_reg, m->stream);
+        }));
+        bool ring_only = true, any_regular = false;
+        for (size_t i = 0; i < phases.size(); ++i) {
+            ring_only = ring_only && phases[i].use_ring == 1u;
+            any_regular = any_regular || h_reg[i] != 0u;
+        }
+        p.reg_applies = ring_only && any_regular;
+    }
     p.blocks = blocks;
     p.n_phases = phases.size();
     p.state = Form::Ready;
diff --git a/sparsemat_amd/csrc/internal.hpp b/sparsemat_amd/csrc/internal.hpp
--- a/sparsemat_amd/csrc/internal.hpp
+++ b/sparsemat_amd/csrc/internal.hpp
@@ -445,7 +445,9 @@
                       const void *val, const void *x, void *y, size_t n_rows, size_t nnz, bool padded, unsigned n_blocks,
                       const uint32_t *phase_ptr, const RingPhase *phases, unsigned ring_entries, unsigned bands,
                       hipStream_t s, void *dot_partials = nullptr ,
-                      unsigned block_begin = 0, unsigned block_end = ~0u );
+                      unsigned block_begin = 0, unsigned block_end = ~0u ,
+                      const uint32_t *reg_len = nullptr );
+int launch_ring_regular(const uint32_t *off, const RingPhase *phases, size_t n_phases, uint32_t *reg_len, hipStream_t s);
 int launch_tile_intervals(const uint32_t *off, const uint32_t *col, size_t n_rows, size_t tile_rows, size_t max_width,
                           uint32_t *win, uint32_t *d_count, hipStream_t s);
 int launch_ring_band_codes(const uint32_t *off, const uint32_t *col, const uint32_t *win, size_t n_rows, uint32_t S,
@@ -565,6 +567,8 @@
     size_t n_phases = 0;
     DevArray<uint32_t> phase_ptr;
     DevArray<RingPhase> phases;
+    DevArray<uint32_t> reg_len;
+    bool reg_applies = false;
     DevArray<uint32_t> win;
     DevArray<uint16_t> col16;
     Form c12 = Form::NotTried;
diff --git a/sparsemat_amd/csrc/spmv_dispatch.hip b/sparsemat_amd/csrc/spmv_dispatch.hip
--- a/sparsemat_amd/csrc/spmv_dispatch.hip
+++ b/sparsemat_amd/csrc/spmv_dispatch.hip
@@ -1,4 +1,5 @@
 #include <cstdlib>
+#include <cstring>
 
 #include "crs_forms.hpp"
 
@@ -112,10 +113,13 @@
 }
 
 static int launch_ring(smh_crs *m, const void *x, void *y, hipStream_t s, void *dot_partials = nullptr, unsigned b0 = 0, unsigned b1 = ~0u) {
+    const char *reg_env = getenv("SMH_RING_REGULAR");
+    const bool reg_off = reg_env && strcmp(reg_env, "auto") != 0 && atoi(reg_env) == 0;
+    const uint32_t *reg_len = m->ring.reg_applies && !reg_off && (m->ring.lo8.get() || m->ring.col16.get()) ? m->ring.reg_len.get() : nullptr;
     return launch_spmv_ring2(m->dtype, auto_lanes(m), auto_chunks(m), m->d_off, m->d_col, m->ring.col16.get(),
                              RingCol12{m->ring.lo8.get(), m->ring.hdr.get(), m->ring.escapes.get()}, m->d_val, x, y, m->n_rows, m->nnz,
                              m->owns || m->nnz % 4 == 0, m->ring.blocks, m->ring.phase_ptr.get(), m->ring.phases.get(), m->ring.entries,
-                             m->ring.bands, s, dot_partials, b0, b1);
+                             m->ring.bands, s, dot_partials, b0, b1, reg_len);
 }
 
 size_t spmv_fused_dot_partials(smh_crs *m, size_t x_len, int variant, bool any_lhs) {
diff --git a/sparsemat_amd/csrc/spmv_ring2.hip b/sparsemat_amd/csrc/spmv_ring2.hip
--- a/sparsemat_amd/csrc/spmv_ring2.hip
+++ b/sparsemat_amd/csrc/spmv_ring2.hip
@@ -131,6 +131,14 @@
     u.o1 = off[r1];
 }
 
+template <typename T, int NCH>
+__device__ __forceinline__ void regular_offsets(Unit<T, NCH> &u, uint32_t e0, uint32_t L, uint64_t rb, uint64_t base, uint64_t row_end,
+                                                uint32_t lane) {
+    const uint32_t n = (uint32_t)(row_end - rb), d = base - rb < n ? (uint32_t)(base - rb) : n, left = n - d;
+    u.o0 = e0 + (d + (lane < left ? lane : left)) * L;
+    u.o1 = e0 + (d + (lane + 1u < left ? lane + 1u : left)) * L;
+}
+
 template <int LANES>
 __device__ __forceinline__ void row_bounds(uint32_t o0, uint32_t o1, int t, uint32_t lane, uint32_t nnz_lim,
                                            uint32_t &s, uint32_t &e) {
@@ -232,11 +240,11 @@
     }
 }
 
-template <typename T, int LANES, int CH, int GM, int CF, int RING, bool DOT = false>
+template <typename T, int LANES, int CH, int GM, int CF, int RING, bool DOT = false, bool REG = false>
 __device__ __forceinline__ void phase_rows(const uint32_t *__restrict__ off, const ColStream &cols,
                                            const T *__restrict__ val, const T *__restrict__ x, const T *ring,
                                            T *__restrict__ y, uint64_t rb, uint64_t re, uint32_t nnz_lim,
-                                           uint64_t last_chunk, uint32_t wave, uint32_t lane, T *dacc = nullptr) {
+                                           uint64_t last_chunk, uint32_t wave, uint32_t lane, T *dacc = nullptr, uint32_t L = 0) {
     constexpr int STEPS = LANES;
     constexpr int SBMAX = sizeof(T) == 8 ? SMH_RING2_SB64 : kRing2SB;
     constexpr int SB = STEPS < SBMAX ? STEPS : SBMAX;
@@ -244,13 +252,39 @@
     constexpr uint64_t STRIDE = (uint64_t)(Ring2Cfg<T, RING>::kThreads / kWave) * RU;
     uint64_t base = rb + (uint64_t)wave * RU;
     if (base >= re) return;
-    uint32_t kb = __builtin_amdgcn_readfirstlane(off[rb]) & ~3u;
+    const uint32_t e0 = __builtin_amdgcn_readfirstlane(off[rb]);
+    uint32_t kb = e0 & ~3u;
     kb = kb < (uint32_t)last_chunk ? kb : (uint32_t)last_chunk;
     const uint32_t last_rel = (uint32_t)last_chunk - kb;
     ColStream cs = cols;
     cs.colp = reinterpret_cast<const char *>(cols.colp) + (size_t)kb * (CF == kCol12 ? 1u : CF == kCol16 ? 2u : 4u);
     if constexpr (CF == kCol12) cs.hdrp = cols.hdrp + (kb >> 2);
     const T *valp = val + kb;
+    if constexpr (REG) {
+        Unit<T, SB * CH> A, B;
+        regular_offsets(A, e0, L, rb, base, re, lane);
+        regular_offsets(B, e0, L, rb, base + STRIDE, re, lane);
+        issue_unit<T, LANES, CH, SB, CF>(A, cs, valp, kb, nnz_lim, last_rel, lane);
+        for (;;) {
+            if (base + STRIDE >= re) {
+                consume_unit<T, LANES, CH, SB, GM, CF, RING, DOT>(A, base, re, cs, valp, x, ring, y, kb, nnz_lim, last_rel, lane, dacc);
+                break;
+            }
+            issue_unit<T, LANES, CH, SB, CF>(B, cs, valp, kb, nnz_lim, last_rel, lane);
+            consume_unit<T, LANES, CH, SB, GM, CF, RING, DOT>(A, base, re, cs, valp, x, ring, y, kb, nnz_lim, last_rel, lane, dacc);
+            regular_offsets(A, e0, L, rb, base + 2 * STRIDE, re, lane);
+            base += STRIDE;
+            if (base + STRIDE >= re) {
+                consume_unit<T, LANES, CH, SB, GM, CF, RING, DOT>(B, base, re, cs, valp, x, ring, y, kb, nnz_lim, last_rel, lane, dacc);
+                break;
+            }
+            issue_unit<T, LANES, CH, SB, CF>(A, cs, valp, kb, nnz_lim, last_rel, lane);
+            consume_unit<T, LANES, CH, SB, GM, CF, RING, DOT>(B, base, re, cs, valp, x, ring, y, kb, nnz_lim, last_rel, lane, dacc);
+            regular_offsets(B, e0, L, rb, base + 2 * STRIDE, re, lane);
+            base += STRIDE;
+        }
+        return;
+    }
     Unit<T, SB * CH> A, B, N;
     load_offsets(A, off, base, re, lane);
     load_offsets(B, off, base + STRIDE, re, lane);
@@ -279,12 +313,12 @@
 
 __device__ const col12::Table k_col12_table = col12::make_table();
 
-template <typename T, int LANES, int CH, int CF, int RING, bool DOT = false>
+template <typename T, int LANES, int CH, int CF, int RING, bool DOT = false, bool REGK = false>
 __global__ void __launch_bounds__((Ring2Cfg<T, RING>::kThreads), (Ring2Cfg<T, RING>::kWavesPerSimd))
 k_spmv_ring2(const uint32_t *__restrict__ off, const uint32_t *__restrict__ col, const uint16_t *__restrict__ col16, RingCol12 c12,
              const T *__restrict__ val, const T *__restrict__ x, T *__restrict__ y, uint32_t nnz_lim, uint64_t last_chunk,
              const uint32_t *__restrict__ phase_ptr, const RingPhase *__restrict__ phases, uint32_t bands,
-             T *__restrict__ dot_partials, uint32_t lb0, uint32_t lb_n) {
+             T *__restrict__ dot_partials, uint32_t lb0, uint32_t lb_n, const uint32_t *__restrict__ reg_len) {
     T dacc_v = T(0);
     T *dacc = DOT ? &dacc_v : nullptr;
     extern __shared__ __attribute__((aligned(16))) unsigned char ring_raw[];
@@ -322,7 +356,16 @@
             }
             __syncthreads();
         }
-        if (ph.use_ring == 1)
+        if constexpr (REGK) {
+            static_assert(CF != kColU32, "regular phases stream one of the narrow column forms");
+            const uint32_t L = reg_len[p];
+            if (L != 0)
+                phase_rows<T, LANES, CH, 1, CF, RING, DOT, true>(off, ring_cols, val, x, ring, y, ph.row_begin, ph.row_end, nnz_lim,
+                                                                 last_chunk, wave, lane, dacc, L);
+            else
+                phase_rows<T, LANES, CH, 1, CF, RING, DOT>(off, ring_cols, val, x, ring, y, ph.row_begin, ph.row_end, nnz_lim, last_chunk,
+                                                           wave, lane, dacc);
+        } else if (ph.use_ring == 1)
             phase_rows<T, LANES, CH, 1, CF, RING, DOT>(off, ring_cols, val, x, ring, y, ph.row_begin, ph.row_end, nnz_lim, last_chunk, wave,
                                                        lane, dacc);
         else if (ph.use_ring == 2)
@@ -386,6 +429,36 @@
     uint64_t blocks = (n_out + kBlock - 1) / kBlock;
     if (blocks > 8192) blocks = 8192;
     hipLaunchKernelGGL(k_narrow_columns, dim3((unsigned)blocks), dim3(kBlock), 0, s, col, (uint64_t)nnz, (uint64_t)n_out, col16);
+    SMH_HIP(hipGetLastError());
+    return SMH_OK;
+}
+
+__global__ void __launch_bounds__(kBlock)
+k_ring_regular(const uint32_t *__restrict__ off, const RingPhase *__restrict__ phases, uint32_t n_phases, uint32_t *__restrict__ reg_len) {
+    __shared__ uint32_t s_bad;
+    for (uint32_t p = blockIdx.x; p < n_phases; p += gridDim.x) {
+        const uint32_t rb = phases[p].row_begin, re = phases[p].row_end;
+        const bool ring = phases[p].use_ring == 1u && re > rb;
+        if (threadIdx.x == 0) s_bad = 0u;
+        __syncthreads();
+        uint32_t L = 0;
+        if (ring) {
+            const uint32_t e0 = off[rb];
+            L = off[rb + 1] - e0;
+            bool bad = false;
+            for (uint64_t r = (uint64_t)rb + threadIdx.x; r <= re; r += kBlock) bad |= (uint64_t)off[r] != (uint64_t)e0 + (r - rb) * (uint64_t)L;
+            if (bad) s_bad = 1u;
+        }
+        __syncthreads();
+        if (threadIdx.x == 0) reg_len[p] = s_bad ? 0u : L;
+        __syncthreads();
+    }
+}
+
+int launch_ring_regular(const uint32_t *off, const RingPhase *phases, size_t n_phases, uint32_t *reg_len, hipStream_t s) {
+    if (n_phases == 0) return SMH_OK;
+    hipLaunchKernelGGL(k_ring_regular, dim3((unsigned)(n_phases < 8192 ? n_phases : 8192)), dim3(kBlock), 0, s, off, phases, (uint32_t)n_phases,
+                       reg_len);
     SMH_HIP(hipGetLastError());
     return SMH_OK;
 }
@@ -472,7 +545,7 @@
 static int launch_ring2_t(int lanes, int chunks, const uint32_t *off, const uint32_t *col, const uint16_t *col16, const RingCol12 &c12, const T *val,
                           const T *x, T *y, size_t n_rows, size_t nnz, bool padded, unsigned n_blocks,
                           const uint32_t *phase_ptr, const RingPhase *phases, uint32_t bands, T *dot_partials, hipStream_t s,
-                          unsigned block_begin, unsigned block_end) {
+                          unsigned block_begin, unsigned block_end, const uint32_t *reg_len) {
     if (bands == 4u && !col16) return fail(SMH_ERR_INVALID, "banded ring plan without the 16-bit slot array");
     constexpr bool kHasCol12 = std::is_same<T, float>::value && RING == (int)col12::kSlots;
     if (c12.lo8 && (!kHasCol12 || bands != 1u || !c12.hdr || !c12.escapes))
@@ -489,31 +562,35 @@
         const uint64_t last_chunk = (nnz_lim - 1) & ~uint64_t(3);
         dim3 grid(((lb1 - lb0) + 7u) & ~7u), block(Ring2Cfg<T, RING>::kThreads);
         constexpr size_t ring_bytes = (size_t)RING * sizeof(T);
-#define SMH_R2_LAUNCH2(L, C, N, D)                                                                                       \
+#define SMH_R2_LAUNCH2(L, C, N, D, R)                                                                                    \
     do {                                                                                                                 \
         constexpr size_t lds_bytes = ring_bytes + ((N) == kCol12 ? sizeof(col12::Table) : 0);                            \
                   \
         static std::atomic<uint64_t> attr_mask{0};                                                                       \
         const uint64_t dev_bit = 1ull << (unsigned)(current_device() & 63);                                              \
         if (!(attr_mask.load(std::memory_order_acquire) & dev_bit)) {                                                    \
-            SMH_HIP(hipFuncSetAttribute(reinterpret_cast<const void *>(&k_spmv_ring2<T, L, C, N, RING, D>),               \
+            SMH_HIP(hipFuncSetAttribute(reinterpret_cast<const void *>(&k_spmv_ring2<T, L, C, N, RING, D, R>),            \
                                         hipFuncAttributeMaxDynamicSharedMemorySize, (int)lds_bytes));                    \
             attr_mask.fetch_or(dev_bit, std::memory_order_release);                                                      \
         }                                                                                                                \
-        hipLaunchKernelGGL((k_spmv_ring2<T, L, C, N, RING, D>), grid, block, lds_bytes, s, off, col, col16, c12, val, x, y, \
+        hipLaunchKernelGGL((k_spmv_ring2<T, L, C, N, RING, D, R>), grid, block, lds_bytes, s, off, col, col16, c12, val, x, y, \
                            (uint32_t)nnz_lim, last_chunk, phase_ptr, phases, bands, dot_partials, (uint32_t)lb0,         \
-                           (uint32_t)(lb1 - lb0));                                                                       \
+                           (uint32_t)(lb1 - lb0), reg_len);                                                              \
     } while (0)
-#define SMH_R2_LAUNCH1(L, C, N)                                                            \
-    do {                                                                                   \
-        if (dot_partials) SMH_R2_LAUNCH2(L, C, N, true); else SMH_R2_LAUNCH2(L, C, N, false); \
+#define SMH_R2_LAUNCH1(L, C, N, R)                                                               \
+    do {                                                                                         \
+        if (dot_partials) SMH_R2_LAUNCH2(L, C, N, true, R); else SMH_R2_LAUNCH2(L, C, N, false, R); \
+    } while (0)
+#define SMH_R2_LAUNCH0(L, C, N)                                                                 \
+    do {                                                                                        \
+        if (reg_len) SMH_R2_LAUNCH1(L, C, N, true); else SMH_R2_LAUNCH1(L, C, N, false);         \
     } while (0)
 #define SMH_R2_LAUNCH(L, C)                                                   \
     do {                                                                      \
         if (c12.lo8) {                                                        \
-            if constexpr (kHasCol12) SMH_R2_LAUNCH1(L, C, kCol12);            \
-        } else if (col16) SMH_R2_LAUNCH1(L, C, kCol16);                       \
-        else SMH_R2_LAUNCH1(L, C, kColU32);                                   \
+            if constexpr (kHasCol12) SMH_R2_LAUNCH0(L, C, kCol12);            \
+        } else if (col16) SMH_R2_LAUNCH0(L, C, kCol16);                       \
+        else SMH_R2_LAUNCH1(L, C, kColU32, false);                            \
     } while (0)
         switch (lanes * 16 + chunks) {
             case 1 * 16 + 1: SMH_R2_LAUNCH(1, 1); break;
@@ -530,6 +607,7 @@
                 return fail(SMH_ERR_INVALID, "ring kernel: unsupported (lanes per row, chunks per lane) = (%d, %d)", lanes, chunks);
         }
 #undef SMH_R2_LAUNCH
+#undef SMH_R2_LAUNCH0
 #undef SMH_R2_LAUNCH1
 #undef SMH_R2_LAUNCH2
         SMH_HIP(hipGetLastError());
@@ -548,22 +626,22 @@
 int launch_spmv_ring2(int dtype, int lanes, int chunks, const uint32_t *off, const uint32_t *col, const uint16_t *col16, const RingCol12 &c12,
                       const void *val, const void *x, void *y, size_t n_rows, size_t nnz, bool padded, unsigned n_blocks,
                       const uint32_t *phase_ptr, const RingPhase *phases, unsigned ring_entries, unsigned bands,
-                      hipStream_t s, void *dot_partials, unsigned block_begin, unsigned block_end) {
+                      hipStream_t s, void *dot_partials, unsigned block_begin, unsigned block_end, const uint32_t *reg_len) {
     if (n_rows == 0) return SMH_OK;
     if (bands != 1u && bands != 4u) return fail(SMH_ERR_INVALID, "ring kernel: %u bands", bands);
     if (dtype == SMH_F64) {
         if (ring_entries != (unsigned)kRingEntries) return fail(SMH_ERR_INVALID, "f64 ring kernel: ring of %u columns", ring_entries);
         return launch_ring2_t<double, kRingEntries>(lanes, chunks, off, col, col16, c12, (const double *)val, (const double *)x,
                                                     (double *)y, n_rows, nnz, padded, n_blocks, phase_ptr, phases, bands,
-                                                    (double *)dot_partials, s, block_begin, block_end);
+                                                    (double *)dot_partials, s, block_begin, block_end, reg_len);
     }
     if (ring_entries == (unsigned)kRingEntriesWide)
         return launch_ring2_t<float, kRingEntriesWide>(lanes, chunks, off, col, col16, c12, (const float *)val, (const float *)x,
                                                        (float *)y, n_rows, nnz, padded, n_blocks, phase_ptr, phases, bands,
-                                                       (float *)dot_partials, s, block_begin, block_end);
+                                                       (float *)dot_partials, s, block_begin, block_end, reg_len);
     if (ring_entries != (unsigned)kRingEntries) return fail(SMH_ERR_INVALID, "ring kernel: ring of %u columns", ring_entries);
     return launch_ring2_t<float, kRingEntries>(lanes, chunks, off, col, col16, c12, (const float *)val, (const float *)x, (float *)y,
-                                               n_rows, nnz, padded, n_blocks, phase_ptr, phases, bands, (float *)dot_partials, s, block_begin, block_end);
-}
-
-}
+                                               n_rows, nnz, padded, n_blocks, phase_ptr, phases, bands, (float *)dot_partials, s, block_begin, block_end, reg_len);
+}
+
+}
diff --git a/sparsemat_amd/sparsemat_crs.py b/sparsemat_amd/sparsemat_crs.py
--- a/sparsemat_amd/sparsemat_crs.py
+++ b/sparsemat_amd/sparsemat_crs.py
@@ -540,6 +540,14 @@
                                       ph.ctypes.data if nph.value else None))
         return nb.value, frac.value, bool(act.value), ptr, ph
 
+    def ring_regular(self):
+        nph = C.c_size_t()
+        check(lib().smh_crs_ring_plan(self._h, None, C.byref(nph), None, None, None, None))
+        out = np.zeros(nph.value, dtype=np.uint32)
+        if nph.value:
+            check(lib().smh_crs_ring_regular(self._h, out.ctypes.data))
+        return out
+
     def max_row_len(self):
         out = C.c_uint32()
         check(lib().smh_crs_max_row_len(self._h, C.byref(out)))
```

After: 8279 (median of 6 runs). 2.2% higher.
